# arangesh/Ground-Plane-Polling

Measured on AMD Instinct MI355X. Metric: images/sec end-to-end (resnet50, 1k planes, 1242x375), higher is better.
Workload: dtype f16x3

## Files before the change

### ground-plane-polling_amd/csrc/conv_igemm.hip

```cpp

#include <hip/hip_runtime.h>
#include <stdint.h>
#include <stdlib.h>

#include "conv_igemm_types.h"
#include "conv_tiles.h"
#include "gpp.h"

namespace {

inline bool is_x3(int dtype) { return dtype == GPP_BF16X3 || dtype == GPP_F16X3; }
inline bool f32_storage(int dtype) { return dtype == GPP_F32 || is_x3(dtype); }
inline int elem_size(int dtype) { return f32_storage(dtype) ? 4 : 2; }

int validate(const gpp_conv_desc& d)
{
    if (!d.in || !d.weight || !d.out) return GPP_ERR_BAD_ARG;
    if (d.dtype != GPP_BF16 && d.dtype != GPP_F16 && d.dtype != GPP_F32 && !is_x3(d.dtype)) return GPP_ERR_UNSUPPORTED;
    const int esz = elem_size(d.dtype), ck = 128 / esz, va = 16 / esz;
    if (d.batch <= 0 || d.C_in <= 0 || d.C_out <= 0 || d.KH <= 0 || d.KW <= 0) return GPP_ERR_BAD_ARG;
    constexpr int kMaxDim = 1 << 20;
    if (d.batch > kMaxDim || d.C_in > kMaxDim || d.C_out > kMaxDim || d.in_pitch > kMaxDim || d.out_pitch > kMaxDim || d.res_pitch > kMaxDim ||
        d.weight_rows > kMaxDim || d.weight_rows < 0 || d.in_pitch < 0 || d.out_pitch < 0 || d.res_pitch < 0 || d.partial_bytes < 0)
        return GPP_ERR_UNSUPPORTED;
    if (d.KH > 8 || d.KW > 8) return GPP_ERR_UNSUPPORTED;
    if (d.C_in % ck != 0 || d.C_out % 4 != 0) return GPP_ERR_UNSUPPORTED;
    if (d.stride != 1 && d.stride != 2) return GPP_ERR_UNSUPPORTED;
    if (d.n_groups < 1 || d.n_groups > GPP_MAX_GROUPS) return GPP_ERR_BAD_ARG;
    if (d.split_k < 0) return GPP_ERR_BAD_ARG;
#ifndef GPP_STAMPS
    if (d.reserved != 0) return GPP_ERR_BAD_ARG;
#endif
    if (d.reserved2 != 0 || (d.x3_split & ~(GPP_X3_IN | GPP_X3_OUT | GPP_X3_RES))) return GPP_ERR_BAD_ARG;
    if (d.reserved3 != 0 || (d.gather_rows != nullptr) != (d.gather_counts != nullptr)) return GPP_ERR_BAD_ARG;
    if (((uintptr_t)d.gather_rows | (uintptr_t)d.gather_counts | (uintptr_t)d.guard) & 3) return GPP_ERR_ALIGN;
    if (d.gather_rows && (d.stride != 1 || d.residual || !d.out_f32 || d.split_k > 1)) return GPP_ERR_UNSUPPORTED;
    if (d.x3_split && !is_x3(d.dtype)) return GPP_ERR_BAD_ARG;
    if (d.out_scale && d.dtype != GPP_F16X3) return GPP_ERR_BAD_ARG;
    if ((d.x3_split & GPP_X3_OUT) && (d.out_f32 || d.C_out % 32 != 0 || d.out_pitch % 32 != 0)) return GPP_ERR_UNSUPPORTED;
    if ((d.x3_split & GPP_X3_IN) && d.in_pitch % 32 != 0) return GPP_ERR_UNSUPPORTED;
    if ((d.x3_split & GPP_X3_RES) && (!d.residual || d.res_pitch % 32 != 0)) return GPP_ERR_UNSUPPORTED;
    const int oa = (d.out_f32 || f32_storage(d.dtype)) ? 4 : 8;
    if (d.in_pitch < d.C_in || d.in_pitch % va != 0) return GPP_ERR_ALIGN;
    if (d.out_pitch < d.C_out || d.out_pitch % oa != 0) return GPP_ERR_ALIGN;
    if (d.residual && (d.res_pitch < d.C_out || d.res_pitch % va != 0)) return GPP_ERR_ALIGN;
    if (((uintptr_t)d.in | (uintptr_t)d.weight | (uintptr_t)d.out | (uintptr_t)d.zero_page | (uintptr_t)d.residual |
         (uintptr_t)d.bias | (uintptr_t)d.partial) & 15)
        return GPP_ERR_ALIGN;
    for (int g = 0; g < d.n_groups; ++g) {
        const gpp_conv_group& G = d.groups[g];
        if (G.H_in <= 0 || G.W_in <= 0 || G.H_out <= 0 || G.W_out <= 0) return GPP_ERR_BAD_ARG;
        if (G.H_in > kMaxDim || G.W_in > kMaxDim || G.H_out > kMaxDim || G.W_out > kMaxDim || G.H_res > kMaxDim || G.W_res > kMaxDim) return GPP_ERR_UNSUPPORTED;
        constexpr int64_t kMaxOff = (int64_t)1 << 40;
        if (G.in_off < 0 || G.out_off < 0 || G.res_off < 0 || G.in_bstride < 0 || G.out_bstride < 0 || G.res_bstride < 0 || G.in_off > kMaxOff ||
            G.out_off > kMaxOff || G.res_off > kMaxOff || G.in_bstride > kMaxOff || G.out_bstride > kMaxOff || G.res_bstride > kMaxOff)
            return GPP_ERR_BAD_ARG;
        if ((G.out_off | G.out_bstride) % oa != 0) return GPP_ERR_ALIGN;
        if ((G.in_off | G.in_bstride) % va != 0) return GPP_ERR_ALIGN;
        if (d.residual && ((G.res_off | G.res_bstride) % va != 0 || G.H_res <= 0 || G.W_res <= 0)) return GPP_ERR_ALIGN;
        if ((int64_t)d.batch * G.H_out * G.W_out >= (1LL << 31)) return GPP_ERR_UNSUPPORTED;
        if ((d.x3_split & GPP_X3_OUT) && ((G.out_off | G.out_bstride) % 32 != 0)) return GPP_ERR_ALIGN;
        if ((d.x3_split & GPP_X3_IN) && ((G.in_off | G.in_bstride) % 32 != 0)) return GPP_ERR_ALIGN;
        if ((d.x3_split & GPP_X3_RES) && ((G.res_off | G.res_bstride) % 32 != 0)) return GPP_ERR_ALIGN;
    }
    return GPP_OK;
}

int split_rule(const gpp_conv_desc& d)
{
    if (!d.partial) return 1;
    int64_t pix = 0;
    for (int g = 0; g < d.n_groups; ++g) pix += (int64_t)d.groups[g].H_out * d.groups[g].W_out;
    const int64_t tiles_per_image = ((pix + 127) / 128) * ((d.C_out + 127) / 128);
    const int64_t kdepth = (int64_t)d.KH * d.KW * d.C_in;
    if (tiles_per_image > 24 || kdepth < 3072) return 1;
    int split = (int)((kdepth + 768) / 1536);
    return split < 1 ? 1 : (split > 8 ? 8 : split);
}

int fill_range_counter(gpp_conv_desc& d)
{
    if (d.dtype != GPP_F16X3) return d.range_counter ? GPP_ERR_BAD_ARG : GPP_OK;
    if (!d.range_counter) d.range_counter = (uint64_t*)gpp_x3_range_counter_f16x3();
    if (!d.range_counter) return GPP_ERR_UNSUPPORTED;
    return ((uintptr_t)d.range_counter & 7) ? GPP_ERR_ALIGN : GPP_OK;
}

int dispatch_any(gpp_conv_desc& d, hipStream_t st)
{
    const int rc = fill_range_counter(d);
    if (rc != GPP_OK) return rc;
    if (d.split_k == 0) d.split_k = split_rule(d);
    if (d.gather_rows) {
        if (d.split_k > 1) return GPP_ERR_UNSUPPORTED;
        return gpp_conv_gather_dispatch(d, st);
    }
    switch (d.dtype) {
        case GPP_BF16: return gpp_conv_dispatch_bf16(d, st);
        case GPP_F16: return gpp_conv_dispatch_f16(d, st);
        case GPP_BF16X3: return gpp_conv_dispatch_bf16x3(d, st);
        case GPP_F16X3: return gpp_conv_dispatch_f16x3(d, st);
        default: return gpp_conv_dispatch_f32(d, st);
    }
}

int tail_entry(const gpp_conv_desc* conv3x3, const gpp_conv_desc* conv1x1, int tile_rows, void* stream)
{
    if (!conv3x3 || !conv1x1) return GPP_ERR_BAD_ARG;
    gpp_conv_desc d1 = *conv3x3, d2 = *conv1x1;
    int rc = validate(d1);
    if (rc == GPP_OK) rc = validate(d2);
    if (rc != GPP_OK) return rc;
    if (d1.gather_rows || d2.gather_rows || d1.guard || d2.guard) return GPP_ERR_UNSUPPORTED;
    const gpp_conv_group &G1 = d1.groups[0], &G2 = d2.groups[0];
    if (d1.dtype == GPP_F32) return GPP_ERR_UNSUPPORTED;
    if (is_x3(d1.dtype) && (!(d1.x3_split & GPP_X3_IN) || (d2.x3_split & (GPP_X3_OUT | GPP_X3_RES)) != (GPP_X3_OUT | GPP_X3_RES) || !d2.residual))
        return GPP_ERR_UNSUPPORTED;
    if (d1.dtype != d2.dtype || d1.n_groups != 1 || d2.n_groups != 1 || d1.batch != d2.batch) return GPP_ERR_UNSUPPORTED;
    if (d1.KH != 3 || d1.KW != 3 || d1.stride != 1 || d1.pad_top != 1 || d1.pad_left != 1 || d1.residual || d1.out_f32) return GPP_ERR_UNSUPPORTED;
// ... 71 lines not shown
{
    return gpp_x3_range_snapshot_of(nullptr, device_count, stream);
}

extern "C" int gpp_x3_range_snapshot_of(const uint64_t* counter, uint64_t* device_count, void* stream)
{
    if (!device_count) return GPP_ERR_BAD_ARG;
    if (((uintptr_t)counter | (uintptr_t)device_count) & 7) return GPP_ERR_ALIGN;
    return gpp_x3_range_snapshot_f16x3((const unsigned long long*)counter, (unsigned long long*)device_count, (hipStream_t)stream);
}

extern "C" int gpp_conv2d_flops(const gpp_conv_desc* host_desc, double* flops)
{
    if (!host_desc || !flops) return GPP_ERR_BAD_ARG;
    if (host_desc->n_groups < 1 || host_desc->n_groups > GPP_MAX_GROUPS) return GPP_ERR_BAD_ARG;
    double f = 0.0;
    for (int g = 0; g < host_desc->n_groups; ++g)
        f += 2.0 * host_desc->batch * (double)host_desc->groups[g].H_out * host_desc->groups[g].W_out *
             host_desc->KH * host_desc->KW * (double)host_desc->C_in * host_desc->C_out;
    *flops = f;
    return GPP_OK;
}

extern "C" int gpp_conv2d_split_rule(const gpp_conv_desc* host_desc, int* split_k)
{
    if (!host_desc || !split_k) return GPP_ERR_BAD_ARG;
    gpp_conv_desc d = *host_desc;
    int rc = validate(d);
    if (rc != GPP_OK) return rc;
    *split_k = d.split_k > 0 ? d.split_k : split_rule(d);
    return GPP_OK;
}

extern "C" int gpp_conv2d_workspace_bytes(const gpp_conv_desc* host_desc, size_t* bytes)
{
    if (!host_desc || !bytes) return GPP_ERR_BAD_ARG;
    gpp_conv_desc d = *host_desc;
    char probe[16] __attribute__((aligned(16)));
    if (!d.partial) { d.partial = probe; d.partial_bytes = 0; }
    int rc = validate(d);
    if (rc != GPP_OK) return rc;
    const int split = d.split_k > 0 ? d.split_k : split_rule(d);
    *bytes = 0;
    if (split <= 1) return GPP_OK;
    int64_t rows = 0;
    for (int g = 0; g < d.n_groups; ++g) rows += (int64_t)d.batch * d.groups[g].H_out * d.groups[g].W_out + 256;
    const int64_t npad = (d.C_out + 255) / 256 * 256;
    *bytes = (size_t)(split * rows * npad * 4);
    return GPP_OK;
}

extern "C" int gpp_conv2d_igemm(const gpp_conv_desc* host_desc, void* stream)
{
    if (!host_desc) return GPP_ERR_BAD_ARG;
    gpp_conv_desc d = *host_desc;
    for (int g = 0; g < GPP_MAX_GROUPS; ++g) d.groups[g].row_begin = 0;
    int rc = validate(d);
    if (rc != GPP_OK) return rc;
    return dispatch_any(d, (hipStream_t)stream);
}

static const gpp_tiles::Entry kTiles[] = {{0, gpp_tiles::PLAIN, gpp_tiles::ALL, 0, 128, 0, 0, 0}, GPP_CONV_TILES(GPP_TILE_ENTRY, GPP_TILE_NONE, GPP_TILE_NONE)};

static bool env_is_1(const char* name) { const char* e = getenv(name); return e && e[0] == '1'; }

static bool tile_is_candidate(const gpp_conv_desc* desc, const gpp_tiles::Entry& t)
{
    using namespace gpp_tiles;
    const gpp_conv_desc& d = *desc;
    if ((d.gather_rows != nullptr) != (t.form == GATHER)) return t.code == 0;
    const bool x3_in = is_x3(d.dtype) && (d.x3_split & GPP_X3_IN);
    if (!owner_has(t.owner, f32_storage(d.dtype), is_x3(d.dtype))) return false;
    if (is_x3(d.dtype) && x3_wants_split_input(t.form, t.owner) && !x3_in && t.owner != ALL_X3IN) return false;
    const int nk = d.KH * d.KW * (d.C_in / (128 / elem_size(d.dtype)));
    if (t.form == DUAL && !dual_can_run(d, nk)) return false;
    if (t.form == MIX && !mix_can_run(d, nk)) return false;
    if (t.form == WS && !ws_can_run(d, t.bm, t.bn)) return false;
    static const bool no_deep = env_is_1("GPP_NO_DEEP_TILES"), no_ws = env_is_1("GPP_NO_WS_TILES"), no_mix = env_is_1("GPP_NO_MIX_TILES");
    int64_t rows = 0;
    for (int g = 0; g < d.n_groups; ++g) rows += (int64_t)d.batch * d.groups[g].H_out * d.groups[g].W_out;
    const int bn = t.bn;
    const auto pads_less_than = [&](int other) { return (d.C_out + bn - 1) / bn * bn < (d.C_out + other - 1) / other * other; };
    switch (t.form) {
        case GATHER: return bn != 160 || pads_less_than(64);
        case DEEP: {
            int64_t tiles_m = 0;
            for (int g = 0; g < d.n_groups; ++g) tiles_m += ((int64_t)d.batch * d.groups[g].H_out * d.groups[g].W_out + t.bm - 1) / t.bm;
            const int64_t wgs = tiles_m * ((d.C_out + bn - 1) / bn) * (d.split_k > 1 ? d.split_k : 1);
            return !(bn == 64 && d.C_out > 256) && !no_deep && nk >= 12 && wgs <= 320;
        }
        case WS: return !no_ws && rows >= 256 * 16;
        case MIX: return !no_mix && nk >= 4 && rows * (d.C_out / 256) >= 256 * 256;
        default: break;
    }
    if (t.code == 0) return true;
    if (bn == 64 && d.C_out > 256 && !(d.KH == 1 && d.KW == 1 && d.C_in <= 256)) return false;
    if (bn == 256 && (d.C_out < 192 || rows < 256 * 16)) return false;
    if ((t.form == PIPE || t.form == DUAL) && nk < 4) return false;
    if ((bn == 160 || bn == 96) && !pads_less_than(128)) return false;
    return true;
}

extern "C" int gpp_conv2d_tile_candidates(const gpp_conv_desc* desc, int* tiles, int capacity, int* count)
{
    if (!desc || !count || capacity < 0 || (capacity > 0 && !tiles)) return GPP_ERR_BAD_ARG;
    {
        gpp_conv_desc d = *desc;
        for (int g = 0; g < GPP_MAX_GROUPS; ++g) d.groups[g].row_begin = 0;
        const int rc = validate(d);
        if (rc != GPP_OK) return rc;
    }
    int n = 0;
    for (const gpp_tiles::Entry& t : kTiles) {
        if (!tile_is_candidate(desc, t)) continue;
        if (n < capacity) tiles[n] = t.code;
        ++n;
    }
    *count = n;
    return GPP_OK;
}

extern "C" int gpp_conv2d_autotune(gpp_conv_desc* desc, int iters, void* stream, float* best_us)
{
    if (!desc || iters < 1) return GPP_ERR_BAD_ARG;
    {
        gpp_conv_desc d = *desc;
        for (int g = 0; g < GPP_MAX_GROUPS; ++g) d.groups[g].row_begin = 0;
        const int rc = validate(d);
        if (rc != GPP_OK) return rc;
    }
    hipStream_t st = (hipStream_t)stream;
    hipEvent_t e0, e1;
    hipError_t e = hipEventCreate(&e0);
    if (e != hipSuccess) return (int)e;
    e = hipEventCreate(&e1);
    if (e != hipSuccess) { (void)hipEventDestroy(e0); return (int)e; }
    const int tile_in = desc->tile_hint;
    float best = 1e30f;
    int best_tile = tile_in, rc = GPP_OK;
    auto time_one = [&](int tile, float* us, int reps = 2) -> int {
        desc->tile_hint = tile;
        int r = gpp_conv2d_igemm(desc, stream);
        if (r != GPP_OK) return r;
        float t_best = 1e30f;
        for (int rep = 0; rep < reps; ++rep) {
            (void)hipEventRecord(e0, st);
            for (int i = 0; i < iters; ++i) (void)gpp_conv2d_igemm(desc, stream);
            (void)hipEventRecord(e1, st);
            hipError_t s = hipEventSynchronize(e1);
            if (s != hipSuccess) return (int)s;
            float ms = 0.0f;
            (void)hipEventElapsedTime(&ms, e0, e1);
            t_best = ms < t_best ? ms : t_best;
        }
        *us = t_best * 1000.0f / iters;
        return GPP_OK;
    };
    float second = 1e30f;
    int second_tile = -1;
    for (const gpp_tiles::Entry& t : kTiles) {
        if (!tile_is_candidate(desc, t)) continue;
        const int tile = t.code;
        float us = 0.0f;
        int r = time_one(tile, &us);
        if (r != GPP_OK) { if (tile == 0) { rc = r; break; } continue; }
        if (us < best) { second = best; second_tile = best_tile; best = us; best_tile = tile; }
        else if (us < second) { second = us; second_tile = tile; }
// ... 124 lines not shown
```

### ground-plane-polling_amd/csrc/conv_igemm_impl.h

```cpp
#ifndef GPP_CONV_IGEMM_IMPL_H_
#define GPP_CONV_IGEMM_IMPL_H_

#include <hip/hip_runtime.h>
#include <stdint.h>

#include <atomic>
#include <type_traits>

#include "conv_tiles.h"
#include "gpp.h"

namespace {

typedef __attribute__((ext_vector_type(8))) __bf16 bf16x8;
typedef __attribute__((ext_vector_type(8))) _Float16 f16x8;
typedef __attribute__((ext_vector_type(4))) float f32x4;

struct f32x8 {
    f32x4 lo, hi;
    __device__ __forceinline__ float operator[](int e) const { return e < 4 ? lo[e] : hi[e - 4]; }
};

template <int DT> struct Elem;
template <> struct Elem<GPP_BF16> {
    using scalar = __bf16;
    using vec8 = bf16x8;
    using frag = bf16x8;
    static constexpr int ESZ = 2;
    static __device__ __forceinline__ f32x4 mfma(frag a, frag b, f32x4 c)
    {
        return __builtin_amdgcn_mfma_f32_16x16x32_bf16(a, b, c, 0, 0, 0);
    }
    static __device__ __forceinline__ vec8 pack(const float (&v)[8])
    {
        vec8 o;
#pragma unroll
        for (int e = 0; e < 8; ++e) o[e] = (scalar)v[e];
        return o;
    }
};
template <> struct Elem<GPP_F16> {
    using scalar = _Float16;
    using vec8 = f16x8;
    using frag = f16x8;
    static constexpr int ESZ = 2;
    static __device__ __forceinline__ f32x4 mfma(frag a, frag b, f32x4 c)
    {
        return __builtin_amdgcn_mfma_f32_16x16x32_f16(a, b, c, 0, 0, 0);
    }
    static __device__ __forceinline__ vec8 pack(const float (&v)[8])
    {
        vec8 o;
#pragma unroll
        for (int e = 0; e < 8; ++e) o[e] = (scalar)v[e];
        return o;
    }
};
template <> struct Elem<GPP_F32> {
    using scalar = float;
    using vec8 = f32x8;
    using frag = f32x4;
    static constexpr int ESZ = 4;
    static __device__ __forceinline__ f32x4 mfma(frag a, frag b, f32x4 c)
    {
        c = __builtin_amdgcn_mfma_f32_16x16x4f32(a[0], b[0], c, 0, 0, 0);
        c = __builtin_amdgcn_mfma_f32_16x16x4f32(a[1], b[1], c, 0, 0, 0);
        c = __builtin_amdgcn_mfma_f32_16x16x4f32(a[2], b[2], c, 0, 0, 0);
        c = __builtin_amdgcn_mfma_f32_16x16x4f32(a[3], b[3], c, 0, 0, 0);
        return c;
    }
    static __device__ __forceinline__ vec8 pack(const float (&v)[8])
    {
        vec8 o;
        o.lo = (f32x4){v[0], v[1], v[2], v[3]};
        o.hi = (f32x4){v[4], v[5], v[6], v[7]};
        return o;
    }
};

constexpr int kRowBytes = 128;

__device__ __forceinline__ void glds16(__amdgpu_buffer_rsrc_t rsrc, int voffset, int soffset, void* lds_dst_wave_base)
{
    __builtin_amdgcn_raw_ptr_buffer_load_lds(rsrc, (__attribute__((address_space(3))) void*)lds_dst_wave_base, 16,
                                             voffset, soffset, 0, 0);
}

constexpr int kOutOfRange = (int)0x80000000;

#ifndef GPP_DMA_SPREAD
#define GPP_DMA_SPREAD 1
#endif
#ifndef GPP_X3_PRIO
#define GPP_X3_PRIO 1
#endif
constexpr bool kSpreadDma = GPP_DMA_SPREAD != 0;

#ifndef GPP_X3_SERPENTINE
#define GPP_X3_SERPENTINE 2
#endif
#define GPP_SERP(g, j, n) ((GPP_X3_SERPENTINE && ((g) & 1)) ? (n) - 1 - (j) : (j))
#define GPP_SERP2(g, j, n) ((GPP_X3_SERPENTINE > 1 && ((g) & 1)) ? (n) - 1 - (j) : (j))

#ifdef GPP_STAMPS
#define GPP_STAMP(k)                                                                                          \
    do {                                                                                                      \
        if ((d.reserved & 16) && wave == 0 && lane == 0)                                                      \
            ((unsigned long long*)d.zero_page)[((int64_t)blockIdx.y * gridDim.x + blockIdx.x) * 8 + (k)] = __builtin_amdgcn_s_memrealtime(); \
    } while (0)
#define GPP_STAMP_END()                                                                                       \
    do {                                                                                                      \
        GPP_STAMP(3);                                                                                         \
        asm volatile("s_waitcnt vmcnt(0)" ::: "memory");                                                      \
        GPP_STAMP(4);                                                                                         \
    } while (0)
#define GPP_ABL(flag) if (!(flag))
#else
#define GPP_ABL(flag)
#define GPP_STAMP(k) do { } while (0)
#define GPP_STAMP_END() do { } while (0)
#endif

__device__ __forceinline__ int xcd_remap(int bid, int nwg)
{
    const int xcd = bid & 7, local = bid >> 3;
    const int q = nwg >> 3, r = nwg & 7;
    return (xcd < r ? xcd * (q + 1) : r * (q + 1) + (xcd - r) * q) + local;
}

template <int DT> constexpr bool kX3 = (DT == GPP_BF16X3 || DT == GPP_F16X3);
template <int DT> struct X3Half {
    using half = __bf16;
    using vec = bf16x8;
    static __device__ __forceinline__ f32x4 mfma(vec, vec, f32x4 c) { return c; }
    static __device__ __forceinline__ float clamp(float x) { return x; }
};

template <> struct X3Half<GPP_BF16X3> {
    using half = __bf16;
    using vec = bf16x8;
    static __device__ __forceinline__ f32x4 mfma(vec a, vec b, f32x4 c) { return __builtin_amdgcn_mfma_f32_16x16x32_bf16(a, b, c, 0, 0, 0); }
    static __device__ __forceinline__ float clamp(float x) { return x; }
};
template <> struct X3Half<GPP_F16X3> {
    using half = _Float16;
    using vec = f16x8;
    static __device__ __forceinline__ f32x4 mfma(vec a, vec b, f32x4 c) { return __builtin_amdgcn_mfma_f32_16x16x32_f16(a, b, c, 0, 0, 0); }
    static __device__ __forceinline__ float clamp(float x) { return fminf(fmaxf(x, -65504.0f), 65504.0f); }
};
template <int DT>
__device__ __forceinline__ void x3_range(float (&v)[8], unsigned long long* counter)
{
    if constexpr (DT == GPP_F16X3) {
        float c[8];
        bool changed = false;
#pragma unroll
        for (int e = 0; e < 8; ++e) {
            c[e] = X3Half<DT>::clamp(v[e]);
            changed |= (c[e] != v[e]);
        }
        if (__builtin_expect(changed, 0)) {
            atomicAdd(counter, 1ull);
#pragma unroll
            for (int e = 0; e < 8; ++e) c[e] = (fabsf(v[e]) <= 3.402823466e38f) ? c[e] : v[e];
        }
#pragma unroll
        for (int e = 0; e < 8; ++e) v[e] = c[e];
    }
}
__device__ __forceinline__ const char* x3_addr(const void* buf, int64_t base, int n)
{
    return (const char*)buf + ((base + (n & ~31)) << 2) + ((n & 31) << 1);
}
template <int DT>
__device__ __forceinline__ void x3_unpack(const f32x4 hi_bits, const f32x4 lo_bits, float (&r)[8])
{
    union { f32x4 f; typename X3Half<DT>::vec b; } h, l;
    h.f = hi_bits;
    l.f = lo_bits;
// ... 120 lines not shown
                                            int64_t out_off, int64_t out_bs, int64_t res_off, int64_t res_bs)
{
    const int b = m / HoWo, p = m - b * HoWo;
    int64_t rp = p;
    if (d.residual && (H_res != H_out || W_res != W_out)) {
        const float sy = (float)H_res / (float)H_out, sx = (float)W_res / (float)W_out;
        const int oy = p / W_out, ox = p - oy * W_out;
        const int ry = min((int)floorf((float)oy * sy), H_res - 1);
        const int rx = min((int)floorf((float)ox * sx), W_res - 1);
        rp = (int64_t)ry * W_res + rx;
    }
    RowAddr a;
    a.obase = out_off + (int64_t)b * out_bs + (int64_t)p * d.out_pitch;
    a.rbase = res_off + (int64_t)b * res_bs + rp * d.res_pitch;
    return a;
}

struct PixWalk {
    int b, oy, ox;
    __device__ __forceinline__ void init(int m, int HoWo, int W_out)
    {
        b = m / HoWo;
        const int p = m - b * HoWo;
        oy = p / W_out;
        ox = p - oy * W_out;
    }
    __device__ __forceinline__ void advance(int n, int H_out, int W_out)
    {
        ox += n;
        while (ox >= W_out) { ox -= W_out; ++oy; }
        while (oy >= H_out) { oy -= H_out; ++b; }
    }
};

__device__ __forceinline__ RowAddr row_addr_at(const gpp_conv_desc& d, const PixWalk& w, int W_out, int H_out, int H_res, int W_res,
                                               int64_t out_off, int64_t out_bs, int64_t res_off, int64_t res_bs)
{
    const int p = w.oy * W_out + w.ox;
    int64_t rp = p;
    if (d.residual && (H_res != H_out || W_res != W_out)) {
        const float sy = (float)H_res / (float)H_out, sx = (float)W_res / (float)W_out;
        const int ry = min((int)floorf((float)w.oy * sy), H_res - 1);
        const int rx = min((int)floorf((float)w.ox * sx), W_res - 1);
        rp = (int64_t)ry * W_res + rx;
    }
    RowAddr a;
    a.obase = out_off + (int64_t)w.b * out_bs + (int64_t)p * d.out_pitch;
    a.rbase = res_off + (int64_t)w.b * res_bs + rp * d.res_pitch;
    return a;
}

template <int DT> struct ElemX3 {
    using scalar = float;
    using vec8 = f32x8;
    using frag = f32x4;
    static constexpr int ESZ = 4;
    static __device__ __forceinline__ vec8 pack(const float (&v)[8]) { return Elem<GPP_F32>::pack(v); }
    static __device__ __forceinline__ f32x4 mfma(frag, frag, f32x4 c) { return c; }
    static __device__ __forceinline__ void split(const f32x4 x0, const f32x4 x1, typename X3Half<DT>::vec& hi, typename X3Half<DT>::vec& lo)
    {
        using half = typename X3Half<DT>::half;
#pragma unroll
        for (int e = 0; e < 8; ++e) {
            const float x = X3Half<DT>::clamp(e < 4 ? x0[e] : x1[e - 4]);
            const half h = (half)x;
            hi[e] = h;
            lo[e] = (half)(x - (float)h);
        }
    }
};
template <> struct Elem<GPP_BF16X3> : ElemX3<GPP_BF16X3> {};
template <> struct Elem<GPP_F16X3> : ElemX3<GPP_F16X3> {};

template <int DT> constexpr bool kF32Storage = (DT == GPP_F32 || DT == GPP_BF16X3 || DT == GPP_F16X3);

constexpr int stage_rows(int BM, int NW) { return (BM + 8 * NW - 1) / (8 * NW) * (8 * NW); }

template <int DT, int BM, int BN, int WM, int WN, int STAGES, bool PIPE, bool XIN = false, bool PRE = false, bool GATHER = false>
__device__ __forceinline__ void conv_igemm_body(const gpp_conv_desc& d, const int block_x, const int grid_x, const float* pre_s = nullptr,
                                                const float* pre_t = nullptr)
{
    static_assert(!XIN || kX3<DT>, "pre-split input maps: GPP_BF16X3 / GPP_F16X3");
    static_assert(!PRE || (!PIPE && !XIN && kF32Storage<DT>), "pre-activation: float32-sized input maps, plain loop");
    static_assert(!GATHER || (!PIPE && !PRE), "gathered rows: plain loop");
    if (d.guard != nullptr && *(const volatile int32_t*)d.guard != d.guard_value) return;
    using E = Elem<DT>;
    using vec8 = typename E::vec8;
    using frag = typename E::frag;
    using scalar = typename E::scalar;
    using xh8 = typename X3Half<DT>::vec;
    constexpr int ESZ = E::ESZ, CK = kRowBytes / ESZ;
    constexpr int NW = WM * WN;
    constexpr int MF = BM / WM / 16, NF = BN / WN / 16;
    constexpr int BMS = stage_rows(BM, NW);
    constexpr int A_BYTES = BMS * kRowBytes, B_BYTES = BN * kRowBytes, STAGE = A_BYTES + B_BYTES;
    constexpr int A_IT = BMS / 8 / NW, B_IT = BN / 8 / NW;
    constexpr int PER_STAGE = A_IT + B_IT;
    constexpr int PF = STAGES - 1;
    static_assert(MF >= 1 && NF >= 1 && A_IT >= 1 && B_IT >= 1 && BMS % (8 * NW) == 0 && BN % (8 * NW) == 0 && BM % (16 * WM) == 0, "tile / wave shape");

    extern __shared__ __attribute__((aligned(16))) unsigned char smem[];

    const int tid = threadIdx.x, lane = tid & 63;
    const int wave = __builtin_amdgcn_readfirstlane(tid >> 6);
    const int wm = wave / WN, wn = wave % WN;
    GPP_STAMP(0);

    const int bid = GATHER ? block_x : xcd_remap(block_x, grid_x);
    const int n_tiles = (d.C_out + BN - 1) / BN;
    const int nt = bid % n_tiles, mt = bid / n_tiles;
    int tile_start = 0, row_begin = 0, H_in = 0, W_in = 0, H_out = 0, W_out = 0, H_res = 0, W_res = 0;
    int64_t in_off = 0, in_bs = 0, out_off = 0, out_bs = 0, res_off = 0, res_bs = 0;
    int list_begin = 0, list_next = 0, group = 0;
#pragma unroll
    for (int q = 0; q < GPP_MAX_GROUPS; ++q) {
        if constexpr (GATHER) {
            if (q < d.n_groups && mt >= d.groups[q].tile_start) { list_begin = list_next; group = q; }
            if (q < d.n_groups) list_next += d.batch * d.groups[q].H_out * d.groups[q].W_out;
        }
        if (q < d.n_groups && mt >= d.groups[q].tile_start) {
            tile_start = d.groups[q].tile_start;
            row_begin = d.groups[q].row_begin;
            H_in = d.groups[q].H_in; W_in = d.groups[q].W_in;
            H_out = d.groups[q].H_out; W_out = d.groups[q].W_out;
            H_res = d.groups[q].H_res; W_res = d.groups[q].W_res;
            in_off = d.groups[q].in_off; in_bs = d.groups[q].in_bstride;
            out_off = d.groups[q].out_off; out_bs = d.groups[q].out_bstride;
            res_off = d.groups[q].res_off; res_bs = d.groups[q].res_bstride;
        }
    }
    const int HoWo = H_out * W_out;
    const int Mpix = d.batch * HoWo;
    const int32_t* const glist = GATHER ? d.gather_rows + list_begin : nullptr;
    const int Mg = GATHER ? min(max(d.gather_counts[group], 0), Mpix) : Mpix;
    const int m0 = row_begin + (mt - tile_start) * BM, n0 = nt * BN;
    if constexpr (GATHER) {
        if (m0 >= Mg) return;
    }
    auto pixel_of = [&](int m) { return min(max(glist[m], 0), Mpix - 1); };
    const int Ktot = d.KH * d.KW * d.C_in;
    const int cpt = d.C_in / CK;
    const int nk_total = d.KH * d.KW * cpt;
    const int nsplit = gridDim.y, split = blockIdx.y;
    int ks0 = 0, nk = nk_total;
    if (nsplit > 1) {
        ks0 = (int)((unsigned)(nk_total * split) / (unsigned)nsplit);
        nk = (int)((unsigned)(nk_total * (split + 1)) / (unsigned)nsplit) - ks0;
    }

    const int srow = lane >> 3;
    const int gchunk = (lane & 7) ^ srow;
    const __amdgpu_buffer_rsrc_t in_rsrc = __builtin_amdgcn_make_buffer_rsrc((void*)d.in, 0, d.in_bytes, 0x00020000);
    const __amdgpu_buffer_rsrc_t w_rsrc = __builtin_amdgcn_make_buffer_rsrc((void*)d.weight, 0, d.weight_bytes, 0x00020000);
    constexpr bool VOFF_INLINE = PIPE && A_IT >= 8;
    int a_base[A_IT], a_mask[A_IT], a_voff[VOFF_INLINE ? 1 : A_IT];
    int tap_delta = 0, tap_need = 0;
    const int pitch2 = d.in_pitch * ESZ;
    {
        PixWalk pw;
        if constexpr (!GATHER) pw.init(m0 + wave * A_IT * 8 + srow, HoWo, W_out);
#pragma unroll
        for (int i = 0; i < A_IT; ++i) {
            const int m = m0 + (wave * A_IT + i) * 8 + srow;
            a_mask[i] = 0;
            a_base[i] = 0;
            if (m < Mg) {
                if constexpr (GATHER) pw.init(pixel_of(m), HoWo, W_out);
                const int iy0 = pw.oy * d.stride - d.pad_top, ix0 = pw.ox * d.stride - d.pad_left;
                const int rlo = max(0, -iy0), rhi = min(d.KH, max(0, H_in - iy0));
                const int clo = max(0, -ix0), chi = min(d.KW, max(0, W_in - ix0));
                const int rmask = rhi > rlo ? ((1 << rhi) - 1) & ~((1 << rlo) - 1) : 0;
                const int cmask = chi > clo ? ((1 << chi) - 1) & ~((1 << clo) - 1) : 0;
                a_mask[i] = rmask | (cmask << 8);
                a_base[i] = (int)((in_off + (int64_t)pw.b * in_bs) * ESZ) + gchunk * 16 + (iy0 * W_in + ix0) * pitch2;
            }
            if (!GATHER && i + 1 < A_IT) pw.advance(8, H_out, W_out);
        }
    }
    int w_voff[B_IT];
#pragma unroll
    for (int i = 0; i < B_IT; ++i) w_voff[i] = (n0 + (wave * B_IT + i) * 8 + srow) * Ktot * ESZ + gchunk * 16;

    auto set_tap = [&](int kh, int kw) {
        const int delta = (kh * W_in + kw) * pitch2;
        const int need = (1 << kh) | (1 << (8 + kw));
        if constexpr (VOFF_INLINE) {
            tap_delta = delta; tap_need = need;
        } else {
#pragma unroll
            for (int i = 0; i < A_IT; ++i) a_voff[i] = ((a_mask[i] & need) == need) ? a_base[i] + delta : kOutOfRange;
        }
    };
    auto voff_of = [&](int i) {
        if constexpr (VOFF_INLINE) return ((a_mask[i] & tap_need) == tap_need) ? a_base[i] + tap_delta : kOutOfRange;
        else return a_voff[i];
    };
    auto stage = [&](int buf, int cc, int ks) {
        unsigned char* sa = smem + buf * STAGE + wave * A_IT * 8 * kRowBytes;
        unsigned char* sb = smem + buf * STAGE + A_BYTES + wave * B_IT * 8 * kRowBytes;
#pragma unroll
        for (int i = 0; i < A_IT; ++i) glds16(in_rsrc, voff_of(i), cc * kRowBytes, sa + i * 8 * kRowBytes);
#pragma unroll
        for (int i = 0; i < B_IT; ++i) glds16(w_rsrc, w_voff[i], ks * kRowBytes, sb + i * 8 * kRowBytes);
    };
// ... 456 lines not shown
        }
        if (use_pre) {
#pragma unroll
            for (int i = 0; i < MF; ++i) {
                const int m = m0 + wm * (BM / WM) + i * 16 + frow;
                if (m >= Mg) continue;
#pragma unroll
                for (int jj = 0; jj < NF / 2; ++jj) {
                    const int n = n0 + wn * COLS + jj * 32 + fq * 8;
                    if (n >= d.C_out) continue;
                    float v[8];
#pragma unroll
                    for (int e = 0; e < 4; ++e) {
                        v[e] = comb(acc[i][2 * jj][e], jj, e);
                        v[4 + e] = comb(acc[i][2 * jj + 1][e], jj, 4 + e);
                    }
                    finish8_pre<DT>(d, v, n, ra_pre[i].obase, true, rpre[i][jj]);
                }
            }
            GPP_STAMP_END();
            return;
        }
    }
    if (interior && !res) {
        const int mfirst = m0 + wm * (BM / WM) + frow;
        int b = mfirst / HoWo, p = mfirst - b * HoWo;
#pragma unroll
        for (int i = 0; i < MF; ++i) {
            const int64_t obase = out_off + (int64_t)b * out_bs + (int64_t)p * d.out_pitch;
#pragma unroll
            for (int jj = 0; jj < NF / 2; ++jj) {
                float v[8];
#pragma unroll
                for (int e = 0; e < 4; ++e) {
                    v[e] = comb(acc[i][2 * jj][e], jj, e);
                    v[4 + e] = comb(acc[i][2 * jj + 1][e], jj, 4 + e);
                }
                finish8_pre<DT>(d, v, n0 + wn * COLS + jj * 32 + fq * 8, obase, false, typename E::vec8());
            }
            p += 16;
            while (p >= HoWo) { p -= HoWo; ++b; }
        }
        GPP_STAMP_END();
        return;
    }
    PixWalk pwe;
    if constexpr (!GATHER) pwe.init(m0 + wm * (BM / WM) + frow, HoWo, W_out);
#pragma unroll
    for (int i = 0; i < MF; ++i) {
        const int m = m0 + wm * (BM / WM) + i * 16 + frow;
        if (m >= Mg) break;
        if constexpr (GATHER) pwe.init(pixel_of(m), HoWo, W_out);
        const RowAddr ra = row_addr_at(d, pwe, W_out, H_out, H_res, W_res, out_off, out_bs, res_off, res_bs);
        if constexpr (!GATHER) pwe.advance(16, H_out, W_out);
        const scalar* rrow = res ? res + ra.rbase : nullptr;
#pragma unroll
        for (int jj = 0; jj < NF / 2; ++jj) {
            const int n = n0 + wn * COLS + jj * 32 + fq * 8;
            if (n >= d.C_out) continue;
            float v[8];
#pragma unroll
            for (int e = 0; e < 4; ++e) {
                v[e] = comb(acc[i][2 * jj][e], jj, e);
                v[4 + e] = comb(acc[i][2 * jj + 1][e], jj, 4 + e);
            }
            finish8<DT>(d, v, n, ra.obase, rrow);
        }
    }
    GPP_STAMP_END();
}

template <int DT, int BM, int BN, int WM, int WN, int STAGES, bool PIPE, bool XIN = false>
__global__ __launch_bounds__(64 * WM * WN, 2) void conv_igemm_kernel(const gpp_conv_desc d)
{
    conv_igemm_body<DT, BM, BN, WM, WN, STAGES, PIPE, XIN>(d, blockIdx.x, gridDim.x);
}

template <int DT, int BM, int BN, int WM, int WN, int STAGES, bool XIN>
__global__ __launch_bounds__(64 * WM * WN, 2) void conv_gather_kernel(const gpp_conv_desc d)
{
    conv_igemm_body<DT, BM, BN, WM, WN, STAGES, false, XIN, false, true>(d, blockIdx.x, gridDim.x);
}

template <int DT, int BM, int BN, int WM, int WN>
__global__ __launch_bounds__(64 * WM * WN, 2) void conv_preact_kernel(const gpp_conv_desc d, const float* in_scale, const float* in_shift)
{
    conv_igemm_body<DT, BM, BN, WM, WN, 2, false, false, true>(d, blockIdx.x, gridDim.x, in_scale, in_shift);
}

template <int DT, bool XIN = false>
__global__ __launch_bounds__(512, 2) void conv_igemm_dual_kernel(const gpp_conv_desc d0, const gpp_conv_desc d1, const int n0,
                                                                 const int split0, const int n1)
{
    if ((int)blockIdx.x < split0) {
        if ((int)blockIdx.x < n0) conv_igemm_body<DT, 256, 256, 2, 4, 2, true, XIN>(d0, blockIdx.x, n0);
    } else {
        conv_igemm_body<DT, 512, 128, 4, 2, 2, true, XIN>(d1, (int)blockIdx.x - split0, n1);
    }
}

template <int DT, int BMA, int BMB, int BN, bool XIN>
__global__ __launch_bounds__(512, 2) void conv_igemm_mix_kernel(const gpp_conv_desc da, const gpp_conv_desc db, const int na,
                                                                const int splita, const int nb)
{
    if ((int)blockIdx.x < splita) {
        if ((int)blockIdx.x < na) conv_igemm_body<DT, BMA, BN, 2, 4, 2, true, XIN>(da, blockIdx.x, na);
    } else {
        conv_igemm_body<DT, BMB, BN, 2, 4, 2, true, XIN>(db, (int)blockIdx.x - splita, nb);
    }
}

template <int DT>
__global__ __launch_bounds__(256) void splitk_reduce_kernel(const gpp_conv_desc d, int BM, int npad, int nsplit)
{
    if (d.guard != nullptr && *(const volatile int32_t*)d.guard != d.guard_value) return;
    using scalar = typename Elem<DT>::scalar;
    const int n8 = (d.C_out + 7) / 8;
    const int64_t total = (int64_t)d.partial_rows * n8;
    const int64_t e = (int64_t)blockIdx.x * 256 + threadIdx.x;
    if (e >= total) return;
    const int r = (int)(e / n8), n = (int)(e - (int64_t)r * n8) * 8;
    const int mt = r / BM;
    int tile_start = 0, H_out = 0, W_out = 0, H_res = 0, W_res = 0;
    int64_t out_off = 0, out_bs = 0, res_off = 0, res_bs = 0;
#pragma unroll
    for (int q = 0; q < GPP_MAX_GROUPS; ++q) {
        if (q < d.n_groups && mt >= d.groups[q].tile_start) {
            tile_start = d.groups[q].tile_start;
            H_out = d.groups[q].H_out; W_out = d.groups[q].W_out;
            H_res = d.groups[q].H_res; W_res = d.groups[q].W_res;
            out_off = d.groups[q].out_off; out_bs = d.groups[q].out_bstride;
            res_off = d.groups[q].res_off; res_bs = d.groups[q].res_bstride;
        }
    }
    const int HoWo = H_out * W_out;
    const int m = r - tile_start * BM;
    if (m >= d.batch * HoWo) return;
    float v[8];
#pragma unroll
    for (int k = 0; k < 8; ++k) v[k] = 0.0f;
    const float* src = (const float*)d.partial + (int64_t)r * npad + n;
    for (int s = 0; s < nsplit; ++s) {
        const f32x4 a = *(const f32x4*)(src + (int64_t)s * d.partial_rows * npad);
        const f32x4 b = *(const f32x4*)(src + (int64_t)s * d.partial_rows * npad + 4);
#pragma unroll
        for (int k = 0; k < 4; ++k) { v[k] += a[k]; v[4 + k] += b[k]; }
    }
    if constexpr (DT == GPP_F16X3) {
        if (d.out_scale) {
#pragma unroll
            for (int k = 0; k < 8; ++k) if (n + k < d.C_out) v[k] *= d.out_scale[n + k];
        }
    }
    if (d.bias) {
#pragma unroll
        for (int k = 0; k < 8; ++k) if (n + k < d.C_out) v[k] += d.bias[n + k];
    }
    const RowAddr ra = row_addr(d, m, HoWo, W_out, H_out, H_res, W_res, out_off, out_bs, res_off, res_bs);
    finish8<DT>(d, v, n, ra.obase, d.residual ? (const scalar*)d.residual + ra.rbase : nullptr);
}

template <int DT, int BM, int CMID>
__global__ __launch_bounds__(256, 2) void bottleneck_tail_kernel(const gpp_conv_desc d1, const gpp_conv_desc d2)
{
    using E = Elem<DT>;
    using vec8 = typename E::vec8;
// ... 896 lines not shown
    d1.weight_rows = d.weight_rows - head;
    if (d.bias) d1.bias = d.bias + head;
    if (d.out_scale) d1.out_scale = d.out_scale + head;
    for (int g = 0; g < d.n_groups; ++g) {
        d1.groups[g].out_off += head;
        d1.groups[g].res_off += head;
    }
    const int t0 = prepare<256, 256>(d0), t1 = prepare<512, 128>(d1);
    if (t0 < 0) return t0;
    if (t1 < 0) return t1;
    const int n0 = t0 * (head / 256), n1 = t1;
    const int split0 = (n0 + 7) / 8 * 8;
    kernel<<<dim3((unsigned)(split0 + n1)), dim3(512), lds, st>>>(d0, d1, n0, split0, n1);
    return last_launch_rc();
}

template <int DT, int BMA, int BMB>
int launch_mix(const gpp_conv_desc& d, hipStream_t st)
{
    constexpr int BN = 256, CUS = 256;
    constexpr int ESZ = Elem<DT>::ESZ, CK = kRowBytes / ESZ;
    static_assert(kX3<DT>, "mixed grids exist for the x3 types");
    if (!gpp_tiles::mix_can_run(d, d.KH * d.KW * (d.C_in / CK))) return GPP_ERR_UNSUPPORTED;
    const int n_tiles = d.C_out / BN;
    const int64_t rows0 = (int64_t)d.batch * d.groups[0].H_out * d.groups[0].W_out;
    auto tiles_b = [&](int64_t begin, int bm) {
        int64_t t = (rows0 - begin + bm - 1) / bm;
        for (int g = 1; g < d.n_groups; ++g) t += ((int64_t)d.batch * d.groups[g].H_out * d.groups[g].W_out + bm - 1) / bm;
        return t * n_tiles;
    };
    int64_t best_cost = (tiles_b(0, BMA) + CUS - 1) / CUS * BMA;
    int best_ra = 0;
    for (int ra = 1; ra <= 64; ++ra) {
        if ((ra * CUS) % n_tiles != 0) continue;
        const int64_t ma = (int64_t)ra * CUS / n_tiles;
        if (ma * BMA > rows0) break;
        const int64_t cost = (int64_t)ra * BMA + (tiles_b(ma * BMA, BMB) + CUS - 1) / CUS * BMB;
        if (cost < best_cost) { best_cost = cost; best_ra = ra; }
    }
    if (best_ra == 0) return GPP_ERR_UNSUPPORTED;
    constexpr int lds = 2 * (stage_rows(BMA > BMB ? BMA : BMB, 8) + BN) * kRowBytes;
    constexpr auto kernel = conv_igemm_mix_kernel<DT, BMA, BMB, BN, true>;
    const int rc = allow_lds<kernel>(lds);
    if (rc != GPP_OK) return rc;
    const int ma = best_ra * CUS / n_tiles;
    gpp_conv_desc da = d, db = d;
    da.n_groups = 1;
    const int ta = prepare<BMA, BN>(da);
    if (ta < 0) return ta;
    db.groups[0].row_begin = ma * BMA;
    const int tb = prepare<BMB, BN>(db);
    if (tb < 0) return tb;
    da.in_bytes = db.in_bytes;
    const int na = ma * n_tiles, nb = tb * n_tiles;
    const int splita = (na + 7) / 8 * 8;
    kernel<<<dim3((unsigned)(splita + nb)), dim3(512), lds, st>>>(da, db, na, splita, nb);
    return last_launch_rc();
}

template <int DT, int BM, int BN>
int launch_ws(gpp_conv_desc& d, hipStream_t st)
{
    constexpr int R = 4;
    static_assert(kX3<DT>, "weight-stationary 1 x 1: x3 types");
    if (!gpp_tiles::ws_can_run(d, BM, BN)) return GPP_ERR_UNSUPPORTED;
    const gpp_conv_group& G = d.groups[0];
    const int lds = (d.C_in / 32) * BN * kRowBytes + R * BM * kRowBytes;
    const int tiles = prepare<BM, BN>(d);
    if (tiles < 0) return tiles;
    const int n_mtiles = (int)(((int64_t)d.batch * G.H_out * G.W_out + BM - 1) / BM);
    const auto go = [&](auto has_res) {
        constexpr auto kernel = conv1x1_ws_kernel<DT, BM, BN, decltype(has_res)::value>;
        const int rc = allow_lds<kernel>(160 * 1024);
        if (rc != GPP_OK) return rc;
        kernel<<<dim3(256), dim3(512), lds, st>>>(d, n_mtiles);
        return last_launch_rc();
    };
    return d.residual ? go(std::true_type()) : go(std::false_type());
}

template <int DT, int BM, int BN, int WM, int WN, int STAGES, bool XIN = false>
int launch_gather(gpp_conv_desc& d, hipStream_t st)
{
    if constexpr (kX3<DT> && !XIN) {
        if (d.x3_split & GPP_X3_IN) return launch_gather<DT, BM, BN, WM, WN, STAGES, true>(d, st);
    }
    constexpr int BMS = stage_rows(BM, WM * WN);
    constexpr int lds = STAGES * (BMS + BN) * kRowBytes;
    constexpr auto kernel = conv_gather_kernel<DT, BM, BN, WM, WN, STAGES, XIN>;
    const int rc = allow_lds<kernel>(lds);
    if (rc != GPP_OK) return rc;
    const int tiles = prepare<BM, BN>(d);
    if (tiles < 0) return tiles;
    const int n_tiles = (d.C_out + BN - 1) / BN;
    kernel<<<dim3((unsigned)(tiles * n_tiles)), dim3(64 * WM * WN), lds, st>>>(d);
    return last_launch_rc();
}

template <int DT, int FORM, int OWNER, int BM, int BN, int WM, int WN, int STAGES>
int run_tile(gpp_conv_desc& d, hipStream_t st)
{
    if constexpr (FORM == gpp_tiles::GATHER) {
        return GPP_ERR_BAD_ARG;
    } else if constexpr (!gpp_tiles::owner_has(OWNER, kF32Storage<DT>, kX3<DT>)) {
        return kF32Storage<DT> ? GPP_ERR_UNSUPPORTED : GPP_ERR_BAD_ARG;
    } else {
        constexpr bool XIN = kX3<DT> && gpp_tiles::x3_wants_split_input(FORM, OWNER);
        if (XIN && !(d.x3_split & GPP_X3_IN)) return GPP_ERR_UNSUPPORTED;
        if constexpr (FORM == gpp_tiles::DUAL) return launch_dual<DT>(d, st);
        else if constexpr (FORM == gpp_tiles::MIX) return launch_mix<DT, BM, BN>(d, st);
        else if constexpr (FORM == gpp_tiles::WS) return d.guard ? GPP_ERR_UNSUPPORTED : launch_ws<DT, BM, BN>(d, st);
        else return launch<DT, BM, BN, WM, WN, STAGES, gpp_tiles::tile_pipelined(FORM, BM, BN, kF32Storage<DT>), XIN>(d, st);
    }
}

#define GPP_RUN_TILE(code, form, owner, bm, bn, wm, wn, stages) \
    case code: return run_tile<DT, gpp_tiles::form, gpp_tiles::owner, bm, bn, wm, wn, stages>(d, st);
#define GPP_RUN_GATHER(code, form, owner, bm, bn, wm, wn, stages) \
    case code: if constexpr (gpp_tiles::form == gpp_tiles::GATHER) return launch_gather<DT, bm, bn, wm, wn, stages>(d, st); else break;
#define GPP_RUN_PREACT(code, form, owner, bm, bn, wm, wn, stages) \
    case code: return launch_preact<DT, bm, bn, wm, wn>(d, in_scale, in_shift, st);

template <int DT>
int dispatch_preact(gpp_conv_desc& d, const float* in_scale, const float* in_shift, hipStream_t st)
{
    switch (d.tile_hint) {
        case 0: return d.C_out <= 64 ? launch_preact<DT, 128, 64, 2, 2>(d, in_scale, in_shift, st)
                                     : launch_preact<DT, 128, 128, 2, 2>(d, in_scale, in_shift, st);
        GPP_CONV_TILES(GPP_TILE_NONE, GPP_TILE_NONE, GPP_RUN_PREACT)
        default: return GPP_ERR_BAD_ARG;
    }
}

template <int DT>
int dispatch_gather(gpp_conv_desc& d, hipStream_t st)
{
    switch (d.tile_hint) {
        case 0: return launch_gather<DT, 64, 64, 2, 2, 2>(d, st);
        GPP_CONV_TILES(GPP_RUN_GATHER, GPP_RUN_GATHER, GPP_TILE_NONE)
        default: break;
    }
    return GPP_ERR_BAD_ARG;
}

template <int DT>
int dispatch(gpp_conv_desc& d, hipStream_t st)
{
#ifdef GPP_STAMPS
    if constexpr (!kF32Storage<DT>) {
        if ((d.reserved & 4) && (d.tile_hint == 128 || d.tile_hint == 128128)) return launch<DT, 128, 128, 2, 2, 2, true>(d, st);
        if ((d.reserved & 8) && (d.tile_hint == 512 || d.tile_hint == 256256)) return launch<DT, 256, 256, 2, 4, 2, false>(d, st);
    }
#endif
    switch (d.tile_hint) {
        GPP_CONV_TILES(GPP_RUN_TILE, GPP_RUN_TILE, GPP_TILE_NONE)
        case 0: break;
        default: return GPP_ERR_BAD_ARG;
    }
    if (d.C_out <= 64 || (d.C_out % 128 != 0 && d.C_out % 128 <= 64)) return launch<DT, 128, 64, 2, 2, 2, false>(d, st);
    if constexpr (!kF32Storage<DT>) {
        int64_t rows = 0;
        for (int g = 0; g < d.n_groups; ++g) rows += (int64_t)d.batch * d.groups[g].H_out * d.groups[g].W_out;
        const int nk = d.KH * d.KW * (d.C_in / 64);
        const int n256 = (d.C_out + 255) / 256;
        const int64_t big_blocks = ((rows + 255) / 256) * n256;
        const bool n_fits = d.C_out >= 256 && n256 * 256 * 7 <= d.C_out * 8;
        if (n_fits && big_blocks >= 512 && nk >= 8 && d.split_k <= 1) return launch<DT, 256, 256, 2, 4, 2, true>(d, st);
    }
    return launch<DT, 128, 128, 2, 2, 2, false>(d, st);
}

template <auto KERNEL, int BM, int CMID, int ESZ, int LDS>
int launch_tail_as(gpp_conv_desc& d1, gpp_conv_desc& d2, hipStream_t st)
{
    int rc = allow_lds<KERNEL>(LDS);
    if (rc == GPP_OK) rc = set_input_extent(d1, ESZ);
    if (rc == GPP_OK) rc = set_weight_extent(d1, 9 * CMID, ESZ);
    if (rc == GPP_OK) rc = set_weight_extent(d2, CMID, ESZ);
    if (rc != GPP_OK) return rc;
    const gpp_conv_group& G = d1.groups[0];
    const int64_t rows = (int64_t)d1.batch * G.H_out * G.W_out;
    KERNEL<<<dim3((unsigned)((rows + BM - 1) / BM)), dim3(256), LDS, st>>>(d1, d2);
    return last_launch_rc();
}

template <int DT, int BM, int CMID>
int launch_tail(gpp_conv_desc& d1, gpp_conv_desc& d2, hipStream_t st)
{
    return launch_tail_as<bottleneck_tail_kernel<DT, BM, CMID>, BM, CMID, 2, 2 * (BM + CMID) * kRowBytes>(d1, d2, st);
}

template <int DT, int BM, int CMID>
int launch_tail_x3(gpp_conv_desc& d1, gpp_conv_desc& d2, hipStream_t st)
{
    constexpr int KC = CMID / 32;
    constexpr int ring = 2 * (BM + CMID) * kRowBytes, phase2 = KC * BM * kRowBytes + KC * 128 * kRowBytes;
    return launch_tail_as<bottleneck_tail_x3_kernel<DT, BM, CMID>, BM, CMID, 4, (ring > phase2 ? ring : phase2)>(d1, d2, st);
}

template <int DT>
int dispatch_tail_x3(gpp_conv_desc& d1, gpp_conv_desc& d2, int tile_rows, hipStream_t st)
{
    if (d1.C_in != 64) return GPP_ERR_UNSUPPORTED;
    switch (tile_rows) {
        case 64: return launch_tail_x3<DT, 64, 64>(d1, d2, st);
        case 96: return launch_tail_x3<DT, 96, 64>(d1, d2, st);
        case 0:
        case 128: return launch_tail_x3<DT, 128, 64>(d1, d2, st);
        case 160: return launch_tail_x3<DT, 160, 64>(d1, d2, st);
        default: return GPP_ERR_BAD_ARG;
    }
}

template <int DT>
int dispatch_tail(gpp_conv_desc& d1, gpp_conv_desc& d2, int tile_rows, hipStream_t st)
{
    const bool c64 = d1.C_in == 64;
    switch (tile_rows) {
        case 96: return c64 ? launch_tail<DT, 96, 64>(d1, d2, st) : launch_tail<DT, 96, 128>(d1, d2, st);
        case 0:
        case 128: return c64 ? launch_tail<DT, 128, 64>(d1, d2, st) : launch_tail<DT, 128, 128>(d1, d2, st);
// ... 9 lines not shown
```

### ground-plane-polling_amd/csrc/conv_tiles.h

```cpp
#ifndef GPP_CONV_TILES_H_
#define GPP_CONV_TILES_H_

#include <stdint.h>

#include "gpp.h"

namespace gpp_tiles {

enum Form {
    PLAIN,
    PIPE,
    DUAL,
    MIX,
    WS,
    DEEP,
    GATHER,
    PREACT,
};

enum Owner {
    ALL,
    ALL_X3IN,
    B16,
    NOT_F32,
    X3,
    X3IN,
};

struct Entry {
    int code, form, owner;
    int bm, bn;
    int wm, wn, stages;
};

#define GPP_CONV_TILES(T, X, P)                                                                                                          \
    T(64064, PLAIN, ALL, 64, 64, 2, 2, 2)                                                                                                \
    T(96064, PLAIN, ALL, 96, 64, 2, 2, 2)                                                                                                \
    T(128064, PLAIN, ALL, 128, 64, 2, 2, 2)                                                                                              \
    T(160064, PLAIN, ALL, 160, 64, 2, 2, 2)                                                                                              \
    T(192064, PLAIN, ALL, 192, 64, 2, 2, 2)                                                                                              \
    T(64128, PLAIN, ALL, 64, 128, 2, 2, 2)                                                                                               \
    T(96128, PLAIN, ALL, 96, 128, 2, 2, 2)                                                                                               \
    T(128128, PLAIN, ALL, 128, 128, 2, 2, 2)                                                                                             \
    T(160128, PLAIN, ALL, 160, 128, 2, 2, 2)                                                                                             \
    T(192128, PLAIN, ALL, 192, 128, 2, 2, 2)                                                                                             \
    T(224128, PLAIN, ALL, 224, 128, 2, 2, 2)                                                                                             \
    T(1128128, PIPE, NOT_F32, 128, 128, 2, 2, 2)                                                                                         \
    T(1192128, PIPE, NOT_F32, 192, 128, 2, 2, 2)                                                                                         \
    T(1128256, PIPE, NOT_F32, 128, 256, 2, 4, 2)                                                                                         \
    T(1160256, PIPE, X3IN, 160, 256, 2, 4, 2)                                 \
    T(1192256, PIPE, NOT_F32, 192, 256, 2, 4, 2)                                                                                         \
    T(1224256, PIPE, X3IN, 224, 256, 2, 4, 2)                                                                                            \
                                \
    T(256256, PLAIN, NOT_F32, 256, 256, 2, 4, 2)                                                                                         \
    T(1256256, PIPE, X3IN, 256, 256, 2, 4, 2)                                                                                            \
                     \
    T(128160, PLAIN, ALL, 128, 160, 4, 1, 2)                                                                                             \
    T(192160, PLAIN, ALL_X3IN, 192, 160, 4, 1, 2)                  \
    T(1192160, PIPE, B16, 192, 160, 4, 1, 2)                                                                                             \
    T(1128160, PIPE, NOT_F32, 128, 160, 4, 1, 2)                                                                                         \
    T(2256256, DUAL, NOT_F32, 256, 256, 2, 4, 2)                                                                                         \
    T(1192096, PIPE, NOT_F32, 192, 96, 4, 1, 2)                                                                                          \
    T(3256224, MIX, X3IN, 256, 224, 2, 4, 2)                                                                                             \
    T(3192160, MIX, X3IN, 192, 160, 2, 4, 2)                                                                                             \
    T(4128064, WS, X3IN, 128, 64, 2, 4, 4)                                                                                               \
    T(4064064, WS, X3IN, 64, 64, 2, 4, 4)                                                                                                \
    T(4128128, WS, X3IN, 128, 128, 2, 4, 4)                                                                                              \
    T(4064128, WS, X3IN, 64, 128, 2, 4, 4)                                                                                               \
              \
    T(5064064, DEEP, X3IN, 64, 64, 2, 2, 4)                                                                                              \
    T(5096064, DEEP, X3IN, 96, 64, 2, 2, 4)                                                                                              \
    T(5064128, DEEP, X3IN, 64, 128, 2, 2, 4)                                                                                             \
    T(5096128, DEEP, X3IN, 96, 128, 2, 2, 4)                                                                                             \
    T(5128128, DEEP, X3IN, 128, 128, 2, 2, 4)                                                                                            \
                                                 \
    T(128256, PLAIN, X3, 128, 256, 2, 4, 2)                                                                                              \
    T(192256, PLAIN, X3, 192, 256, 2, 4, 2)                                                                                              \
           \
    T(6064064, GATHER, ALL, 64, 64, 2, 2, 2)                                                                                             \
    T(6032064, GATHER, ALL, 32, 64, 2, 2, 2)                                                                                             \
    T(6064160, GATHER, ALL, 64, 160, 4, 1, 2)                                                                                            \
    T(7064064, GATHER, ALL, 64, 64, 2, 2, 4)                                                                                             \
    T(7032064, GATHER, ALL, 32, 64, 2, 2, 4)                                                                                             \
    T(7064160, GATHER, ALL, 64, 160, 4, 1, 4)                                                                                            \
    X(64, PLAIN, ALL, 128, 64, 2, 2, 2)                                                                                                  \
    X(128, PLAIN, ALL, 128, 128, 2, 2, 2)                                                                                                \
    X(256, PLAIN, B16, 256, 128, 4, 2, 3)                                                             \
    X(512, PLAIN, B16, 256, 256, 2, 4, 2)                                                                                                \
    P(64064, PREACT, ALL, 64, 64, 2, 2, 2)                                                                                               \
    P(128064, PREACT, ALL, 128, 64, 2, 2, 2)                                                                                             \
    P(64128, PREACT, ALL, 64, 128, 2, 2, 2)                                                                                              \
    P(128128, PREACT, ALL, 128, 128, 2, 2, 2)                                                                                            \
    P(192128, PREACT, ALL, 192, 128, 2, 2, 2)

#define GPP_TILE_ENTRY(code, form, owner, bm, bn, wm, wn, stages) {code, gpp_tiles::form, gpp_tiles::owner, bm, bn, wm, wn, stages},
#define GPP_TILE_NONE(...)

constexpr bool owner_has(int owner, bool f32_storage, bool x3)
{
    return owner == ALL || owner == ALL_X3IN || (owner == B16 && !f32_storage) || (owner == NOT_F32 && (!f32_storage || x3)) ||
           ((owner == X3 || owner == X3IN) && x3);
}

constexpr bool x3_wants_split_input(int form, int owner)
{
    return owner == X3IN || owner == ALL_X3IN || (form != PLAIN && form != GATHER && form != PREACT);
}

constexpr bool tile_pipelined(int form, int bm, int bn, bool f32_storage) { return form == PIPE || (!f32_storage && form == PLAIN && bm == 256 && bn == 256); }


inline bool dual_can_run(const gpp_conv_desc& d, int nk) { return d.C_out >= 384 && d.C_out % 256 == 128 && nk >= 2 && d.split_k <= 1; }

inline bool mix_can_run(const gpp_conv_desc& d, int nk) { return d.C_out % 256 == 0 && nk >= 2 && d.split_k <= 1; }

inline bool ws_can_run(const gpp_conv_desc& d, int bm, int bn)
{
    const gpp_conv_group& G = d.groups[0];
    return (d.x3_split & GPP_X3_IN) && d.KH == 1 && d.KW == 1 && d.stride == 1 && d.pad_top == 0 && d.pad_left == 0 && d.n_groups == 1 && d.split_k <= 1 &&
           d.C_out % bn == 0 && 32 % (d.C_out / bn) == 0 && d.C_in % 32 == 0 && G.H_in == G.H_out && G.W_in == G.W_out &&
           (!d.residual || ((d.x3_split & GPP_X3_RES) && G.H_res == G.H_out && G.W_res == G.W_out)) &&
           (d.C_in / 32) * bn * 128 + 4 * bm * 128 <= 160 * 1024;
}

}

#endif
```

### ground-plane-polling_amd/csrc/decode.hip

```cpp

#include <hip/hip_runtime.h>
#include <stdint.h>
#include <limits.h>

#include <atomic>

#include "gpp.h"

namespace {

constexpr int kCounterStride = 4096;
constexpr int kHeaderBytes = 64 * kCounterStride;
constexpr int kKeptCountWord = 1;
constexpr int kKeptKeysOffset = 1024;

__device__ __forceinline__ float cephes_expf(float x)
{
    x = fminf(fmaxf(x, -88.3762626647949f), 88.3762626647949f);
    float fx = floorf(x * 1.44269504088896341f + 0.5f);
    x = (x - fx * 0.693359375f) - fx * -2.12194440e-4f;
    const float z = x * x;
    float y = 1.9875691500e-4f;
    y = y * x + 1.3981999507e-3f;
    y = y * x + 8.3334519073e-3f;
// ... 567 lines not shown
    if (stages & GPP_DETECT_CANDIDATES) {
        clear_counters_kernel<<<1, 64, 0, st>>>(cnt, lists);
        const dim3 grid((unsigned)((n_anchors + 255) / 256), (unsigned)B);
        if (osf) candidates_osf_kernel<<<grid, 256, 0, st>>>(cls_logits, n_anchors, kstride, score_thr, keys, cnt);
        else candidates_kernel<<<grid, 256, 0, st>>>(cls_logits, n_anchors, kstride, score_thr, keys, cnt);
    }
    if (stages & GPP_DETECT_SELECT) {
        static std::atomic<uint64_t> configured{0};
        int dev = 0;
        e = hipGetDevice(&dev);
        if (e != hipSuccess) return (int)e;
        if (!(configured.load(std::memory_order_acquire) & (1ull << (dev & 63)))) {
            e = hipFuncSetAttribute((const void*)nms_kernel, hipFuncAttributeMaxDynamicSharedMemorySize, kLdsKeys * 16 + kHistBins * 4);
            if (e != hipSuccess) return (int)e;
            configured.fetch_or(1ull << (dev & 63), std::memory_order_release);
        }
        nms_kernel<<<dim3((unsigned)lists), kNmsThreads, kLdsKeys * 16 + kHistBins * 4, st>>>(
            keys, cnt, kstride, cls_logits, regression, regression_dim, (const float4*)anchors, n_anchors, L, iou_thr, max_det,
            counts, wboxes, alive, ws, lists_per_image);
    }
    if (stages & GPP_DETECT_EMIT) {
        if (osf)
            emit_osf_kernel<<<dim3((unsigned)B), 512, 0, st>>>(ws, cls_logits, regression, regression_dim, (const float4*)anchors,
                                                               n_anchors, L, max_det, boxes, dims, scores, labels, orientations,
                                                               anchor_index, counts);
        else
            emit_kernel<<<dim3((unsigned)B), 128, 0, st>>>(ws, cls_logits, regression, regression_dim, (const float4*)anchors,
                                                           n_anchors, L, max_det, boxes, dims, scores, labels, orientations, anchor_index);
    }
    e = hipGetLastError();
    return e == hipSuccess ? GPP_OK : (int)e;
}

}

namespace {

__global__ __launch_bounds__(256) void pack_kernel(const float* __restrict__ boxes, const float* __restrict__ dims,
                                                   const float* __restrict__ scores, const int32_t* __restrict__ labels,
                                                   const int32_t* __restrict__ orient, const float* __restrict__ keypoints,
                                                   const float* __restrict__ keyplanes, const float* __restrict__ residuals,
                                                   float* __restrict__ out, int64_t rows)
{
    const int64_t e = (int64_t)blockIdx.x * 256 + threadIdx.x;
    if (e >= rows * 35) return;
    const int64_t r = e / 35;
    const int c = (int)(e - r * 35);
    float v;
    if (c < 12) v = boxes[r * 12 + c];
    else if (c < 15) v = dims[r * 3 + (c - 12)];
    else if (c == 15) v = scores[r];
    else if (c == 16) v = (float)labels[r];
    else if (c == 17) v = (float)orient[r];
    else if (c < 30) v = keypoints[r * 12 + (c - 18)];
    else if (c < 34) v = keyplanes[r * 4 + (c - 30)];
    else v = residuals[r];
    out[e] = v;
}

}

extern "C" int gpp_pack_detections(const float* boxes, const float* dims, const float* scores, const int32_t* labels,
                                   const int32_t* orientations, const float* keypoints, const float* keyplanes,
                                   const float* residuals, int B, int D, float* packed, void* stream)
{
    if (B < 0 || D < 0) return GPP_ERR_BAD_ARG;
    if (B == 0 || D == 0) return GPP_OK;
    if (!boxes || !dims || !scores || !labels || !orientations || !keypoints || !keyplanes || !residuals || !packed) return GPP_ERR_BAD_ARG;
    const int64_t rows = (int64_t)B * D;
    pack_kernel<<<dim3((unsigned)((rows * 35 + 255) / 256)), 256, 0, (hipStream_t)stream>>>(
        boxes, dims, scores, labels, orientations, keypoints, keyplanes, residuals, packed, rows);
    hipError_t e = hipGetLastError();
    return e == hipSuccess ? GPP_OK : (int)e;
}

namespace {

struct LevelTable {
    int n_levels;
    int pix[GPP_MAX_GROUPS];
    int pix_begin[GPP_MAX_GROUPS];
    int word_begin[GPP_MAX_GROUPS];
    int list_begin[GPP_MAX_GROUPS];
};

__global__ __launch_bounds__(256) void mark_pixels_kernel(const unsigned long long* __restrict__ keys, const int32_t* __restrict__ cnt,
                                                          int64_t key_stride, int64_t n_anchors, int nba, int lists_per_image,
                                                          const LevelTable T, uint32_t* __restrict__ bitmap)
{
    const int list = blockIdx.y, b = list / lists_per_image;
    const int64_t n = min((int64_t)max(cnt[list * (kCounterStride / 4)], 0), n_anchors);
    for (int64_t i = (int64_t)blockIdx.x * 256 + threadIdx.x; i < n; i += (int64_t)gridDim.x * 256) {
        const uint32_t a = 0xFFFFFFFFu - (uint32_t)keys[(int64_t)list * key_stride + i];
        if ((int64_t)a >= n_anchors) continue;
        const int pixel = (int)(a / (uint32_t)nba);
        int l = 0;
        for (int q = 1; q < T.n_levels; ++q) l = pixel >= T.pix_begin[q] ? q : l;
        const int bit = b * T.pix[l] + (pixel - T.pix_begin[l]);
        atomicOr(&bitmap[T.word_begin[l] + (bit >> 5)], 1u << (bit & 31));
    }
}

constexpr int kCompactThreads = 1024;
__global__ __launch_bounds__(kCompactThreads) void compact_pixels_kernel(uint32_t* __restrict__ bitmap, const LevelTable T, int B, int max_rows,
                                                                         int32_t* __restrict__ rows, int32_t* __restrict__ counts,
                                                                         int32_t* __restrict__ flag)
{
    __shared__ int wave_sum[kCompactThreads / 64];
    const int tid = threadIdx.x, lane = tid & 63, wave = tid >> 6;
    int total = 0;
    for (int l = 0; l < GPP_MAX_GROUPS; ++l) {
        int running = 0;
        if (l < T.n_levels) {
            const int n_words = (B * T.pix[l] + 31) >> 5;
            for (int w0 = 0; w0 < n_words; w0 += kCompactThreads) {
                const int w = w0 + tid;
                uint32_t word = 0;
                if (w < n_words) {
                    word = bitmap[T.word_begin[l] + w];
                    if (word) bitmap[T.word_begin[l] + w] = 0;
                }
                const int c = __popc(word);
                int incl = c;
#pragma unroll
                for (int s = 1; s < 64; s <<= 1) {
                    const int up = __shfl_up(incl, s, 64);
                    if (lane >= s) incl += up;
                }
                if (lane == 63) wave_sum[wave] = incl;
                __syncthreads();
                int before = 0, all = 0;
#pragma unroll
                for (int q = 0; q < kCompactThreads / 64; ++q) {
                    const int v = wave_sum[q];
                    before += q < wave ? v : 0;
                    all += v;
                }
                __syncthreads();
                int pos = running + before + incl - c;
                while (word) {
                    const int bit = __ffs((int)word) - 1;
                    word &= word - 1;
                    rows[T.list_begin[l] + pos++] = w * 32 + bit;
                }
                running += all;
            }
        }
        if (tid == 0) counts[l] = running;
        total += running;
    }
    if (tid == 0) {
        counts[GPP_MAX_GROUPS] = total;
        flag[0] = total > max_rows ? 1 : 0;
    }
}

}

extern "C" int gpp_detect_pixel_lists(const gpp_pixel_list_desc* host_desc, void* stream)
{
    if (!host_desc) return GPP_ERR_BAD_ARG;
    const gpp_pixel_list_desc& d = *host_desc;
    if (d.B < 0 || d.B > kMaxBatch || d.n_anchors <= 0 || d.n_anchors > kMaxAnchors || d.num_base_anchors <= 0 || d.max_rows < 0 ||
        d.n_levels < 1 || d.n_levels > GPP_MAX_GROUPS || (d.lists_per_image != 1 && d.lists_per_image != 4) || d.reserved != 0 || d.reserved2 != 0)
        return GPP_ERR_BAD_ARG;
    if (d.B == 0) return GPP_OK;
    if (!d.workspace || !d.bitmap || !d.rows || !d.counts || !d.flag) return GPP_ERR_BAD_ARG;
    if (((uintptr_t)d.workspace & 15) || (((uintptr_t)d.bitmap | (uintptr_t)d.rows | (uintptr_t)d.counts | (uintptr_t)d.flag) & 3)) return GPP_ERR_ALIGN;
    const int lists = d.B * d.lists_per_image;
    if (lists > 64) return GPP_ERR_UNSUPPORTED;
    LevelTable T;
    T.n_levels = d.n_levels;
    int64_t pixels = 0, words = 0;
    for (int l = 0; l < GPP_MAX_GROUPS; ++l) {
        const int pix = l < d.n_levels ? d.level_pixels[l] : 0;
        if (l < d.n_levels && pix <= 0) return GPP_ERR_BAD_ARG;
        if ((int64_t)d.B * (pixels + pix) >= (1LL << 31)) return GPP_ERR_UNSUPPORTED;
        T.pix[l] = pix;
        T.pix_begin[l] = (int)pixels;
        T.word_begin[l] = (int)words;
        T.list_begin[l] = (int)((int64_t)d.B * pixels);
        pixels += pix;
        words += ((int64_t)d.B * pix + 31) / 32;
    }
    if (pixels * d.num_base_anchors != d.n_anchors) return GPP_ERR_BAD_ARG;
    hipStream_t st = (hipStream_t)stream;
    const unsigned char* ws = (const unsigned char*)d.workspace;
    const int32_t* cnt = (const int32_t*)ws;
    const unsigned long long* keys = (const unsigned long long*)(ws + kHeaderBytes);
    mark_pixels_kernel<<<dim3(16, (unsigned)lists), 256, 0, st>>>(keys, cnt, pow2_ceil(d.n_anchors), d.n_anchors, d.num_base_anchors,
                                                                   d.lists_per_image, T, d.bitmap);
    compact_pixels_kernel<<<1, kCompactThreads, 0, st>>>(d.bitmap, T, d.B, d.max_rows, d.rows, d.counts, d.flag);
    const hipError_t e = hipGetLastError();
    return e == hipSuccess ? GPP_OK : (int)e;
}

extern "C" int gpp_detect_workspace_bytes(int B, int64_t n_anchors, size_t* bytes)
{
    if (!bytes || B < 0 || B > kMaxBatch || n_anchors <= 0 || n_anchors > kMaxAnchors) return GPP_ERR_BAD_ARG;
    *bytes = detect_bytes(B, n_anchors, 1);
    return GPP_OK;
}

extern "C" int gpp_detect_osf_workspace_bytes(int B, int64_t n_anchors, size_t* bytes)
{
    if (!bytes || B < 0 || B > kMaxBatch || n_anchors <= 0 || n_anchors > kMaxAnchors) return GPP_ERR_BAD_ARG;
    *bytes = detect_bytes(B, n_anchors, 4);
    return GPP_OK;
}

extern "C" int gpp_detect_stages_f32(int stages, const float* cls_logits, const float* regression,
                                     const float* regression_dim, const float* anchors, int B, int64_t n_anchors,
                                     int num_base_anchors, int fused_layout, float score_thr, float iou_thr, int max_det,
                                     float* boxes, float* dims, float* scores, int32_t* labels, int32_t* orientations,
                                     int32_t* anchor_index, int32_t* counts,
                                     void* workspace, size_t workspace_bytes, void* stream)
{
    return detect_impl(stages, 1, cls_logits, regression, regression_dim, anchors, B, n_anchors, num_base_anchors, fused_layout, score_thr,
                       iou_thr, max_det, boxes, dims, scores, labels, orientations, anchor_index, counts, workspace, workspace_bytes, stream);
}

extern "C" int gpp_detect_osf_f32(const float* cls_logits, const float* regression, const float* regression_dim,
                                  const float* anchors, int B, int64_t n_anchors, int num_base_anchors, int fused_layout,
                                  float score_thr, float iou_thr, int max_det,
                                  float* boxes, float* dims, float* scores, int32_t* labels, int32_t* orientations,
                                  int32_t* anchor_index, int32_t* counts,
                                  void* workspace, size_t workspace_bytes, void* stream)
{
    return detect_impl(GPP_DETECT_CANDIDATES | GPP_DETECT_SELECT | GPP_DETECT_EMIT, 4, cls_logits, regression, regression_dim, anchors, B,
                       n_anchors, num_base_anchors, fused_layout, score_thr, iou_thr, max_det, boxes, dims, scores, labels, orientations,
                       anchor_index, counts, workspace, workspace_bytes, stream);
}

extern "C" int gpp_detect_f32(const float* cls_logits, const float* regression, const float* regression_dim,
                              const float* anchors, int B, int64_t n_anchors, int num_base_anchors, int fused_layout,
                              float score_thr, float iou_thr, int max_det,
                              float* boxes, float* dims, float* scores, int32_t* labels, int32_t* orientations,
                              int32_t* anchor_index, int32_t* counts,
                              void* workspace, size_t workspace_bytes, void* stream)
{
    return gpp_detect_stages_f32(GPP_DETECT_CANDIDATES | GPP_DETECT_SELECT | GPP_DETECT_EMIT, cls_logits, regression, regression_dim,
                                 anchors, B, n_anchors, num_base_anchors, fused_layout, score_thr, iou_thr, max_det, boxes, dims,
                                 scores, labels, orientations, anchor_index, counts, workspace, workspace_bytes, stream);
}
```

### ground-plane-polling_amd/csrc/stem.hip

```cpp

#include <hip/hip_runtime.h>
#include <stdlib.h>
#include <stdint.h>

#include <atomic>

#include "gpp.h"
#include "conv_igemm_types.h"

namespace {

typedef __attribute__((ext_vector_type(8))) __bf16 bf16x8;
typedef __attribute__((ext_vector_type(8))) _Float16 f16x8;
typedef __attribute__((ext_vector_type(8))) float f32x8_natural;
typedef f32x8_natural f32x8 __attribute__((aligned(16)));

constexpr int TW = 64, TH = 4;
constexpr int PW = TW * 2 + 5, PH = TH * 2 + 5;
constexpr int PPITCH = PW * 3 + 1;

__device__ __forceinline__ int ragged_height(const int* __restrict__ heights, int b, int H)
{
    const int h = __builtin_amdgcn_readfirstlane(heights[b]);
    return h < 1 ? 1 : (h > H ? H : h);
// ... 291 lines not shown
        else stem_pool_mfma_ragged_kernel<_Float16, f16x8, 4><<<grid, 256, lds, st>>>(in, wp, bias, (_Float16*)out, B, H, W, Ho, Wo, Hp, Wp, pt, pl, heights);
        return result();
    }
    if (which == 0) stem_pool_mfma_kernel<__bf16, bf16x8, 8><<<grid, 512, lds, st>>>(in, wp, bias, (__bf16*)out, B, H, W, Ho, Wo, Hp, Wp, pt, pl);
    else if (which == 1) stem_pool_mfma_kernel<_Float16, f16x8, 8><<<grid, 512, lds, st>>>(in, wp, bias, (_Float16*)out, B, H, W, Ho, Wo, Hp, Wp, pt, pl);
    else if (which == 2) stem_pool_mfma_kernel<__bf16, bf16x8, 4><<<grid, 256, lds, st>>>(in, wp, bias, (__bf16*)out, B, H, W, Ho, Wo, Hp, Wp, pt, pl);
    else stem_pool_mfma_kernel<_Float16, f16x8, 4><<<grid, 256, lds, st>>>(in, wp, bias, (_Float16*)out, B, H, W, Ho, Wo, Hp, Wp, pt, pl);
    return result();
}

extern "C" int gpp_stem_pool_fused_mfma(const float* in, const void* packed_weight_f16, const float* bias, void* out,
                                        int dtype, int B, int H, int W, void* stream)
{
    return stem_pool_mfma_run(in, packed_weight_f16, bias, out, dtype, B, H, W, nullptr, stream);
}

extern "C" int gpp_stem_pool_fused_mfma_ragged(const float* in, const void* packed_weight_f16, const float* bias, void* out,
                                               int dtype, int B, int H, int W, int Hp, const int32_t* heights, void* stream)
{
    const int rc = ragged_check(heights, H, Hp, 4);
    return rc != GPP_OK ? rc : stem_pool_mfma_run(in, packed_weight_f16, bias, out, dtype, B, H, W, heights, stream);
}

static int stem_pool_x3_run(const float* in, const void* packed_weight_x3, const float* bias, float* out,
                            int B, int H, int W, uint64_t* range_counter, const int32_t* heights, void* stream)
{
    if (!in || !packed_weight_x3 || !bias || !out || B <= 0 || H <= 0 || W <= 0) return GPP_ERR_BAD_ARG;
    if ((uintptr_t)range_counter & 7) return GPP_ERR_ALIGN;
    if (((uintptr_t)out | (uintptr_t)packed_weight_x3) & 15) return GPP_ERR_ALIGN;
    const int Ho = (H + 6 - 7) / 2 + 1, Wo = (W + 6 - 7) / 2 + 1;
    const int Hp = (Ho + 1) / 2, Wp = (Wo + 1) / 2;
    const int pt = ((Hp - 1) * 2 + 3 - Ho > 0 ? (Hp - 1) * 2 + 3 - Ho : 0) / 2;
    const int pl = ((Wp - 1) * 2 + 3 - Wo > 0 ? (Wp - 1) * 2 + 3 - Wo : 0) / 2;
    static const int env_rows = [] { const char* e = getenv("GPP_STEM_POOL_X3_ROWS"); return (e && atoi(e) == 4) ? 4 : 6; }();
    const int rows = heights ? 4 : env_rows;
    const int pr = rows / 2;
    const int64_t total = (int64_t)B * ((Wp + FP_PCOLS - 1) / FP_PCOLS) * ((Hp + pr - 1) / pr);
    if (total >= (1LL << 30)) return GPP_ERR_UNSUPPORTED;
    int dev = 0, cus = 0;
    if (hipGetDevice(&dev) != hipSuccess || hipDeviceGetAttribute(&cus, hipDeviceAttributeMultiprocessorCount, dev) != hipSuccess || cus <= 0)
        return GPP_ERR_UNSUPPORTED;
    const unsigned grid = (unsigned)(total < cus ? total : cus);
    hipStream_t st = (hipStream_t)stream;
    static std::atomic<uint64_t> done[4];
    const int which = rows == 6 ? 0 : 1;
    const void* fns[4] = {(const void*)stem_pool_mfma_x3_kernel<6>, (const void*)stem_pool_mfma_x3_kernel<4>,
                          nullptr, (const void*)stem_pool_mfma_x3_ragged_kernel<4>};
    const int lds = xp_lds(rows);
    const int fn = which + (heights ? 2 : 0);
    if (!(done[fn].load(std::memory_order_acquire) & (1ull << (dev & 63)))) {
        const hipError_t e = hipFuncSetAttribute(fns[fn], hipFuncAttributeMaxDynamicSharedMemorySize, lds);
        if (e != hipSuccess) return (int)e;
        done[fn].fetch_or(1ull << (dev & 63), std::memory_order_release);
    }
    unsigned long long* counter = range_counter ? (unsigned long long*)range_counter : gpp_x3_range_counter_f16x3();
    if (!counter) return GPP_ERR_UNSUPPORTED;
    const _Float16* wp = (const _Float16*)packed_weight_x3;
    if (heights) stem_pool_mfma_x3_ragged_kernel<4><<<grid, 256, lds, st>>>(in, wp, bias, out, B, H, W, Ho, Wo, Hp, Wp, pt, pl, counter, heights);
    else if (which == 0) stem_pool_mfma_x3_kernel<6><<<grid, 384, lds, st>>>(in, wp, bias, out, B, H, W, Ho, Wo, Hp, Wp, pt, pl, counter);
    else stem_pool_mfma_x3_kernel<4><<<grid, 256, lds, st>>>(in, wp, bias, out, B, H, W, Ho, Wo, Hp, Wp, pt, pl, counter);
    return result();
}

extern "C" int gpp_stem_pool_fused_x3(const float* in, const void* packed_weight_x3, const float* bias, float* out,
                                      int B, int H, int W, uint64_t* range_counter, void* stream)
{
    return stem_pool_x3_run(in, packed_weight_x3, bias, out, B, H, W, range_counter, nullptr, stream);
}

extern "C" int gpp_stem_pool_fused_x3_ragged(const float* in, const void* packed_weight_x3, const float* bias, float* out,
                                             int B, int H, int W, int Hp, const int32_t* heights, uint64_t* range_counter, void* stream)
{
    const int rc = ragged_check(heights, H, Hp, 4);
    return rc != GPP_OK ? rc : stem_pool_x3_run(in, packed_weight_x3, bias, out, B, H, W, range_counter, heights, stream);
}

static int maxpool_run(const void* in, void* out, int dtype, int B, int H, int W, int C, const int32_t* heights, void* stream)
{
    if (!in || !out || B <= 0 || H <= 0 || W <= 0 || C <= 0 || C % 8 != 0) return GPP_ERR_BAD_ARG;
    if (((uintptr_t)in | (uintptr_t)out) & 15) return GPP_ERR_ALIGN;
    const int Ho = (H + 1) / 2, Wo = (W + 1) / 2;
    const int pt = ((Ho - 1) * 2 + 3 - H > 0 ? (Ho - 1) * 2 + 3 - H : 0) / 2;
    const int pl = ((Wo - 1) * 2 + 3 - W > 0 ? (Wo - 1) * 2 + 3 - W : 0) / 2;
    const int64_t total = (int64_t)B * Ho * Wo * (C / 8);
    const unsigned blocks = (unsigned)((total + 255) / 256 < 8192 ? (total + 255) / 256 : 8192);
    hipStream_t st = (hipStream_t)stream;
    if (dtype != GPP_BF16 && dtype != GPP_F16 && dtype != GPP_F32) return GPP_ERR_UNSUPPORTED;
    if (heights) {
        if (dtype == GPP_BF16)
            maxpool_ragged_kernel<__bf16, bf16x8><<<blocks, 256, 0, st>>>((const __bf16*)in, (__bf16*)out, B, H, W, C, Ho, Wo, pt, pl, heights);
        else if (dtype == GPP_F16)
            maxpool_ragged_kernel<_Float16, f16x8><<<blocks, 256, 0, st>>>((const _Float16*)in, (_Float16*)out, B, H, W, C, Ho, Wo, pt, pl, heights);
        else
            maxpool_ragged_kernel<float, f32x8><<<blocks, 256, 0, st>>>((const float*)in, (float*)out, B, H, W, C, Ho, Wo, pt, pl, heights);
        return result();
    }
    if (dtype == GPP_BF16)
        maxpool_kernel<__bf16, bf16x8><<<blocks, 256, 0, st>>>((const __bf16*)in, (__bf16*)out, B, H, W, C, Ho, Wo, pt, pl);
    else if (dtype == GPP_F16)
        maxpool_kernel<_Float16, f16x8><<<blocks, 256, 0, st>>>((const _Float16*)in, (_Float16*)out, B, H, W, C, Ho, Wo, pt, pl);
    else if (dtype == GPP_F32)
        maxpool_kernel<float, f32x8><<<blocks, 256, 0, st>>>((const float*)in, (float*)out, B, H, W, C, Ho, Wo, pt, pl);
    else
        return GPP_ERR_UNSUPPORTED;
    return result();
}

extern "C" int gpp_maxpool3x3s2_same(const void* in, void* out, int dtype, int B, int H, int W, int C, void* stream)
{
    return maxpool_run(in, out, dtype, B, H, W, C, nullptr, stream);
}

extern "C" int gpp_maxpool3x3s2_same_ragged(const void* in, void* out, int dtype, int B, int H, int W, int C, int Hp,
                                            const int32_t* heights, void* stream)
{
    const int rc = ragged_check(heights, H, Hp, 2);
    return rc != GPP_OK ? rc : maxpool_run(in, out, dtype, B, H, W, C, heights, stream);
}

extern "C" int gpp_relu_strided(const void* in, int64_t in_bstride, void* out, int64_t out_bstride, int dtype, int B,
                                int64_t count, void* stream)
{
    if (!in || !out || B <= 0 || count <= 0 || count % 8 != 0 || in_bstride % 8 != 0 || out_bstride % 8 != 0)
        return GPP_ERR_BAD_ARG;
    if (((uintptr_t)in | (uintptr_t)out) & 15) return GPP_ERR_ALIGN;
    const int64_t n8 = count / 8;
    const dim3 grid((unsigned)((n8 + 255) / 256 < 4096 ? (n8 + 255) / 256 : 4096), (unsigned)B);
    hipStream_t st = (hipStream_t)stream;
    if (dtype == GPP_BF16X3 || dtype == GPP_F16X3) {
        if (count % 32 != 0 || in_bstride % 32 != 0 || out_bstride % 32 != 0) return GPP_ERR_BAD_ARG;
        relu_x3_kernel<<<grid, 256, 0, st>>>((const char*)in, in_bstride * 4, (char*)out, out_bstride * 4, count / 8);
        return result();
    }
    if (dtype == GPP_BF16)
        relu_kernel<__bf16, bf16x8><<<grid, 256, 0, st>>>((const __bf16*)in, in_bstride, (__bf16*)out, out_bstride, n8);
    else if (dtype == GPP_F16)
        relu_kernel<_Float16, f16x8><<<grid, 256, 0, st>>>((const _Float16*)in, in_bstride, (_Float16*)out, out_bstride, n8);
    else if (dtype == GPP_F32)
        relu_kernel<float, f32x8><<<grid, 256, 0, st>>>((const float*)in, in_bstride, (float*)out, out_bstride, n8);
    else
        return GPP_ERR_UNSUPPORTED;
    return result();
}

extern "C" int gpp_relu(const void* in, void* out, int dtype, int64_t count, void* stream)
{
    return gpp_relu_strided(in, 0, out, 0, dtype, 1, count, stream);
}
```

### ground-plane-polling_amd/keras_retinanet_3D/backend/hip.py

```python

import ctypes
import os

_LIB = None
_HERE = os.path.dirname(os.path.abspath(__file__))
LIB_PATH = os.environ.get('GPP_LIB') or os.path.normpath(os.path.join(_HERE, '..', '..', 'lib', 'libgpp_hip.so'))
CSRC_DIR = os.path.normpath(os.path.join(_HERE, '..', '..', 'csrc'))

GPP_OK = 0
_ERRORS = {
    -1: 'GPP_ERR_BAD_ARG',
    -2: 'GPP_ERR_WORKSPACE',
    -3: 'GPP_ERR_ALIGN',
    -4: 'GPP_ERR_UNSUPPORTED',
}

c_void_p = ctypes.c_void_p
c_int = ctypes.c_int
c_float = ctypes.c_float
c_size_t = ctypes.c_size_t
c_int64 = ctypes.c_int64


GPP_BF16 = 1
GPP_F16 = 2
GPP_F32 = 3
GPP_BF16X3 = 4
GPP_F16X3 = 5
GPP_MAX_GROUPS = 5
GPP_DRAW_PRIM_WORDS = 16
GPP_DRAW_PRIMS_PER_DET = 26
GPP_DRAW_COUNT_WORDS = 4
GPP_POSE_COLS = 36
GPP_EVAL_MAX_DETECTIONS, GPP_EVAL_MAX_ANNOTATIONS = 1024, 1024
GPP_EVAL_ANN_COLS, GPP_EVAL_ERR_COLS = 17, 11
GPP_KITTI_MAX_DETECTIONS, GPP_KITTI_MAX_LABELS = 128, 128
GPP_KITTI_MAX_THRESHOLDS, GPP_KITTI_LABEL_COLS = 41, 16
GPP_LABEL_MOD_COLS = 20
GPP_ABSMAX_F32, GPP_ABSMAX_SPLIT_F16, GPP_ABSMAX_SPLIT_BF16 = 1, 2, 3


class GppError(RuntimeError):
    pass


class ConvGroup(ctypes.Structure):
    _fields_ = [('in_off', c_int64), ('in_bstride', c_int64), ('out_off', c_int64), ('out_bstride', c_int64),
                ('res_off', c_int64), ('res_bstride', c_int64),
                ('H_in', ctypes.c_int32), ('W_in', ctypes.c_int32), ('H_out', ctypes.c_int32), ('W_out', ctypes.c_int32),
                ('H_res', ctypes.c_int32), ('W_res', ctypes.c_int32), ('tile_start', ctypes.c_int32),
                ('row_begin', ctypes.c_int32)]


class ConvDesc(ctypes.Structure):
    _fields_ = [('inp', c_void_p), ('weight', c_void_p), ('bias', c_void_p), ('residual', c_void_p),
                ('out', c_void_p), ('zero_page', c_void_p),
                ('dtype', ctypes.c_int32), ('out_f32', ctypes.c_int32),
                ('batch', ctypes.c_int32), ('C_in', ctypes.c_int32), ('C_out', ctypes.c_int32),
                ('KH', ctypes.c_int32), ('KW', ctypes.c_int32), ('stride', ctypes.c_int32),
                ('pad_top', ctypes.c_int32), ('pad_left', ctypes.c_int32),
                ('in_pitch', ctypes.c_int32), ('out_pitch', ctypes.c_int32), ('res_pitch', ctypes.c_int32),
                ('weight_rows', ctypes.c_int32), ('relu', ctypes.c_int32), ('n_groups', ctypes.c_int32),
                ('tile_hint', ctypes.c_int32), ('reserved', ctypes.c_int32),
                ('in_bytes', ctypes.c_int32), ('weight_bytes', ctypes.c_int32),
                ('partial', c_void_p), ('partial_bytes', c_int64), ('split_k', ctypes.c_int32), ('partial_rows', ctypes.c_int32),
                ('groups', ConvGroup * GPP_MAX_GROUPS),
                ('x3_split', ctypes.c_int32), ('reserved2', ctypes.c_int32), ('out_scale', c_void_p), ('range_counter', c_void_p),
                ('gather_rows', c_void_p), ('gather_counts', c_void_p), ('guard', c_void_p),
                ('guard_value', ctypes.c_int32), ('reserved3', ctypes.c_int32)]


class PixelListDesc(ctypes.Structure):
    _fields_ = [('workspace', c_void_p), ('bitmap', c_void_p), ('rows', c_void_p), ('counts', c_void_p), ('flag', c_void_p),
                ('n_anchors', c_int64)] + \
               [(n, ctypes.c_int32) for n in ('B', 'num_base_anchors', 'lists_per_image', 'n_levels', 'max_rows', 'reserved')] + \
               [('level_pixels', ctypes.c_int32 * GPP_MAX_GROUPS), ('reserved2', ctypes.c_int32)]


class MobileNetBlockDesc(ctypes.Structure):
    _fields_ = [('inp', c_void_p), ('dw_weight', c_void_p), ('dw_bias', c_void_p), ('pw_weight', c_void_p), ('pw_bias', c_void_p),
                ('out_scale', c_void_p), ('out', c_void_p)] + \
               [(n, ctypes.c_int32) for n in ('dtype', 'B', 'H', 'W', 'C_in', 'C_out', 'stride', 'in_pitch', 'out_pitch', 'weight_rows',
                                              'tile_hint', 'reserved')]


class MobileNetStemDesc(ctypes.Structure):
    _fields_ = [('inp', c_void_p), ('weight', c_void_p), ('bias', c_void_p), ('out', c_void_p)] + \
               [(n, ctypes.c_int32) for n in ('B', 'H', 'W', 'C_out', 'out_pitch', 'reserved')]


class AbsmaxDesc(ctypes.Structure):
    _fields_ = [('inp', c_void_p), ('out', c_void_p), ('M', c_int64), ('pitch', c_int64)] + \
               [(n, ctypes.c_int32) for n in ('C', 'c_off', 'layout', 'reserved')]


class AbsmaxClearDesc(ctypes.Structure):
    _fields_ = [('table', c_void_p), ('n', c_int64)]


def _declare(lib):
    lib.gpp_version.restype = ctypes.c_char_p
    lib.gpp_version.argtypes = []
    lib.gpp_poll_workspace_bytes.restype = c_int
    lib.gpp_poll_workspace_bytes.argtypes = [c_int, c_int, c_int, ctypes.POINTER(c_size_t)]
    lib.gpp_poll_f32.restype = c_int
    lib.gpp_poll_f32.argtypes = [c_void_p] * 5 + [c_int, c_int, c_int, c_int, c_float] + [c_void_p] * 4 + \
        [c_void_p, c_size_t, c_void_p]
    lib.gpp_pose_f32.restype = c_int
    lib.gpp_pose_f32.argtypes = [c_void_p] * 8 + [c_int, c_int, c_float] + [c_void_p] * 3
    if hasattr(lib, 'gpp_draw_build'):
        lib.gpp_draw_workspace_bytes.restype = c_int
        lib.gpp_draw_workspace_bytes.argtypes = [c_int, c_int, ctypes.POINTER(c_size_t), ctypes.POINTER(c_size_t)]
        lib.gpp_draw_build.restype = c_int
        lib.gpp_draw_build.argtypes = [c_void_p, c_void_p, c_int, c_int, c_float, c_void_p, c_void_p, c_void_p]
        lib.gpp_draw_raster.restype = c_int
        lib.gpp_draw_raster.argtypes = [c_void_p, c_void_p, c_int, c_int, c_void_p, c_void_p, c_int, c_void_p, c_void_p, c_void_p]
    if hasattr(lib, 'gpp_eval_match_f32'):
        lib.gpp_eval_match_f32.restype = c_int
        lib.gpp_eval_match_f32.argtypes = [c_void_p] * 8 + [c_int] * 4 + [c_float, c_int, ctypes.c_double] + [c_void_p] * 4
    if hasattr(lib, 'gpp_kitti_overlaps_f64'):
        lib.gpp_kitti_overlaps_f64.restype = c_int
        lib.gpp_kitti_overlaps_f64.argtypes = [c_void_p] * 3 + [c_int] * 3 + [c_void_p] * 2
        lib.gpp_kitti_stats_f64.restype = c_int
        lib.gpp_kitti_stats_f64.argtypes = [c_void_p] * 4 + [ctypes.POINTER(ctypes.c_double)] + [c_void_p] * 2 + [c_int] * 4 + [c_void_p] * 5
    if hasattr(lib, 'gpp_label_prep_f64'):
        lib.gpp_label_prep_f64.restype = c_int
        lib.gpp_label_prep_f64.argtypes = [c_void_p] * 4 + [c_int, c_int, ctypes.c_uint, c_int] + [c_void_p] * 7
    if hasattr(lib, 'gpp_detect_pixel_lists'):
        lib.gpp_detect_pixel_lists.restype = c_int
        lib.gpp_detect_pixel_lists.argtypes = [ctypes.POINTER(PixelListDesc), c_void_p]
    lib.gpp_conv2d_igemm.restype = c_int
    lib.gpp_conv2d_igemm.argtypes = [ctypes.POINTER(ConvDesc), c_void_p]
    lib.gpp_stem_conv7x7_bn_relu.restype = c_int
    lib.gpp_stem_conv7x7_bn_relu.argtypes = [c_void_p, c_void_p, c_void_p, c_void_p, c_int, c_int, c_int, c_int, c_void_p]
    lib.gpp_stem_conv7x7_bn_relu_mfma.restype = c_int
    lib.gpp_stem_conv7x7_bn_relu_mfma.argtypes = [c_void_p, c_void_p, c_void_p, c_void_p, c_int, c_int, c_int, c_int, c_void_p]
    lib.gpp_stem_pack_weights_f16.restype = c_int
    lib.gpp_stem_pack_weights_f16.argtypes = [c_void_p, c_void_p, c_size_t]
    lib.gpp_stem_pack_weights_f16x3.restype = c_int
    lib.gpp_stem_pack_weights_f16x3.argtypes = [c_void_p, c_void_p, c_size_t]
    lib.gpp_stem_conv7x7_bn_relu_x3.restype = c_int
    lib.gpp_stem_conv7x7_bn_relu_x3.argtypes = [c_void_p, c_void_p, c_void_p, c_void_p, c_int, c_int, c_int, c_void_p]
    lib.gpp_stem_pool_fused_mfma.restype = c_int
    lib.gpp_stem_pool_fused_mfma.argtypes = [c_void_p, c_void_p, c_void_p, c_void_p, c_int, c_int, c_int, c_int, c_void_p]
    lib.gpp_maxpool3x3s2_same.restype = c_int
    lib.gpp_maxpool3x3s2_same.argtypes = [c_void_p, c_void_p, c_int, c_int, c_int, c_int, c_int, c_void_p]
    lib.gpp_conv2d_preact.restype = c_int
    lib.gpp_conv2d_preact.argtypes = [ctypes.POINTER(ConvDesc), c_void_p, c_void_p, c_void_p]
    lib.gpp_conv2d_preact_tile_candidates.restype = c_int
    lib.gpp_conv2d_preact_tile_candidates.argtypes = [ctypes.POINTER(ConvDesc), ctypes.POINTER(c_int), c_int, ctypes.POINTER(c_int)]
    lib.gpp_conv2d_preact_autotune.restype = c_int
    lib.gpp_conv2d_preact_autotune.argtypes = [ctypes.POINTER(ConvDesc), c_void_p, c_void_p, c_int, c_void_p, ctypes.POINTER(c_float)]
    lib.gpp_maxpool3x3s2_pad_f32.restype = c_int
    lib.gpp_maxpool3x3s2_pad_f32.argtypes = [c_void_p, c_void_p, c_int, c_int, c_int, c_int, c_int, c_int, c_void_p]
    lib.gpp_avgpool2x2_f32.restype = c_int
    lib.gpp_avgpool2x2_f32.argtypes = [c_void_p, c_void_p, c_int, c_int, c_int, c_int, c_int, c_void_p]
    lib.gpp_mobilenet_block.restype = c_int
    lib.gpp_mobilenet_block.argtypes = [ctypes.POINTER(MobileNetBlockDesc), c_void_p]
    lib.gpp_mobilenet_block_tile_candidates.restype = c_int
# ... 261 lines not shown
```

### ground-plane-polling_amd/keras_retinanet_3D/models/plan.py

```python

import collections
import ctypes

import numpy as np

from ..backend import hip
from ..layers import conv as C


class StemDesc(ctypes.Structure):
    _fields_ = [('inp', ctypes.c_void_p), ('weight', ctypes.c_void_p), ('bias', ctypes.c_void_p), ('out', ctypes.c_void_p),
                ('dtype', ctypes.c_int32), ('B', ctypes.c_int32), ('H', ctypes.c_int32), ('W', ctypes.c_int32), ('range_counter', ctypes.c_void_p)]


class PoolDesc(ctypes.Structure):
    _fields_ = [('inp', ctypes.c_void_p), ('out', ctypes.c_void_p), ('dtype', ctypes.c_int32), ('B', ctypes.c_int32),
                ('H', ctypes.c_int32), ('W', ctypes.c_int32), ('C', ctypes.c_int32), ('reserved', ctypes.c_int32)]


class RaggedStemDesc(ctypes.Structure):
    _fields_ = [('stem', StemDesc), ('heights', ctypes.c_void_p), ('Hp', ctypes.c_int32), ('reserved', ctypes.c_int32)]


class RaggedPoolDesc(ctypes.Structure):
    _fields_ = [('pool', PoolDesc), ('heights', ctypes.c_void_p), ('Hp', ctypes.c_int32), ('reserved', ctypes.c_int32)]


class ReluDesc(ctypes.Structure):
    _fields_ = [('inp', ctypes.c_void_p), ('out', ctypes.c_void_p), ('in_bstride', ctypes.c_int64),
                ('out_bstride', ctypes.c_int64), ('count', ctypes.c_int64), ('dtype', ctypes.c_int32), ('B', ctypes.c_int32)]


class DetectDesc(ctypes.Structure):
    _fields_ = [(n, ctypes.c_void_p) for n in ('cls_logits', 'regression', 'regression_dim', 'anchors', 'boxes', 'dims',
                                               'scores', 'labels', 'orientations', 'anchor_index', 'counts', 'workspace')] + \
               [('workspace_bytes', ctypes.c_size_t), ('n_anchors', ctypes.c_int64),
                ('B', ctypes.c_int32), ('num_base_anchors', ctypes.c_int32), ('fused_layout', ctypes.c_int32),
                ('max_det', ctypes.c_int32), ('score_thr', ctypes.c_float), ('iou_thr', ctypes.c_float)]


class CandidatePixelsDesc(ctypes.Structure):
    _fields_ = [('detect', ctypes.c_void_p), ('lists', hip.PixelListDesc)]


class PollDesc(ctypes.Structure):
    _fields_ = [(n, ctypes.c_void_p) for n in ('boxes', 'dims', 'orient', 'P_inv', 'planes', 'keypoints', 'keyplanes',
                                               'residuals', 'best_idx', 'workspace')] + \
               [('workspace_bytes', ctypes.c_size_t), ('B', ctypes.c_int32), ('D', ctypes.c_int32), ('N', ctypes.c_int32),
                ('planes_batched', ctypes.c_int32), ('thr', ctypes.c_float), ('reserved', ctypes.c_int32)]


class PoseDesc(ctypes.Structure):
    _fields_ = [(n, ctypes.c_void_p) for n in ('boxes', 'dims', 'scores', 'labels', 'orientations', 'keypoints', 'residuals',
                                               'frame_info', 'rows', 'counts')] + \
               [('B', ctypes.c_int32), ('D', ctypes.c_int32), ('score_thr', ctypes.c_float), ('reserved', ctypes.c_int32)]


class PreactDesc(ctypes.Structure):
    _fields_ = [('conv', ctypes.c_void_p), ('in_scale', ctypes.c_void_p), ('in_shift', ctypes.c_void_p)]


class DensePoolDesc(ctypes.Structure):
    _fields_ = [('inp', ctypes.c_void_p), ('out', ctypes.c_void_p), ('B', ctypes.c_int32), ('H', ctypes.c_int32), ('W', ctypes.c_int32),
                ('C', ctypes.c_int32), ('pad', ctypes.c_int32), ('out_pitch', ctypes.c_int32)]


class PlanOp(ctypes.Structure):
    _fields_ = [('kind', ctypes.c_int32), ('tag', ctypes.c_int32), ('desc', ctypes.c_void_p)]


class TailDesc(ctypes.Structure):
    _fields_ = [('conv3x3', ctypes.c_void_p), ('conv1x1', ctypes.c_void_p), ('tile_rows', ctypes.c_int32), ('reserved', ctypes.c_int32)]


class BlockDesc(ctypes.Structure):
    _fields_ = [('conv1x1_a', ctypes.c_void_p), ('conv3x3_b', ctypes.c_void_p), ('conv1x1_c', ctypes.c_void_p), ('tile', ctypes.c_int32), ('reserved', ctypes.c_int32)]


OP_STEM, OP_MAXPOOL, OP_CONV, OP_RELU, OP_DETECT, OP_POLL, OP_TAIL = 1, 2, 3, 4, 5, 6, 7
OP_BLOCK = 16
OP_DETECT_CANDIDATES, OP_DETECT_SELECT, OP_DETECT_EMIT = 8, 9, 10
OP_DETECT_OSF = 12
OP_STEM_POOL = 13
OP_MAXPOOL_PAD, OP_AVGPOOL, OP_CONV_PREACT = 17, 18, 32
OP_MOBILENET_STEM, OP_MOBILENET_BLOCK = 33, 34
OP_POSE = 19
OP_ABSMAX, OP_ABSMAX_CLEAR = 35, 36
OP_STEM_RAGGED, OP_STEM_POOL_RAGGED, OP_MAXPOOL_RAGGED = 37, 38, 39
OP_DETECT_CANDIDATE_PIXELS = 40
DETECT_OPS = (OP_DETECT, OP_DETECT_CANDIDATES, OP_DETECT_SELECT, OP_DETECT_EMIT, 12, OP_DETECT_CANDIDATE_PIXELS)
OP_JOIN, OP_SYNC = 0x10000, 0x20000


PlanOptions = collections.namedtuple('PlanOptions', 'x3_level fuse_stem_pool stage_chunks half_stages fuse_tail fuse_block fuse_block_proj '
                                                    'br1_lane fpn_lanes p4_lane head_lanes decode_overlap cls_lane autotune tune_key sparse_heads')


def block_form(opts, width, projection, split_input, halves, join):
    if width in opts.fuse_block and (not projection or opts.fuse_block_proj) and split_input:
        launch = 'block'
    else:
        launch = 'tail' if width in opts.fuse_tail else 'convs'
    if not projection:
        return launch, 'identity'
    return launch, 'side' if opts.br1_lane and not halves and not join else 'inline'


def part_of(fm, c0, nb):
    return C.FMap(fm.buf, nb, fm.H, fm.W, fm.C, off=fm.off + c0 * fm.bstride, bstride=fm.bstride, pitch=fm.pitch, split=fm.split, half=fm.half)


TOWER_SLICES = {('pyramid_towers_0', 0): 'pyramid_regression_0', ('pyramid_towers_0', 512): 'pyramid_classification_0',
                ('pyramid_towers_0', 768): 'pyramid_regression_dim_0'}
RANGE_AUDIT_THRESHOLD = 2.0 ** -9
X3_QUANTUM = 2.0 ** -24
SPARSE_HEADS_MAX_SHARE = '0.5'


def audit_report(maps, table, threshold=RANGE_AUDIT_THRESHOLD):
    table = np.ascontiguousarray(table).view(np.uint32).reshape(-1)
    out = []
    for m in maps:
        first, n = m['row']
        bits = table[first:first + n]
        vals = bits.view(np.float32).astype(np.float64)
        live = vals[bits != 0]
        finite = live[~np.isnan(live)]
        absmax = float('nan') if len(finite) < len(live) else float(finite.max()) if len(finite) else 0.0
        rec = {k: m[k] for k in ('name', 'consumers', 'channels') if k in m}
        rec.update({'live': int(len(live)), 'absmax': absmax,
                    'absmax_min_live': float(finite.min()) if len(finite) else None,
                    'absmax_median_live': float(np.median(finite)) if len(finite) else None,
                    'small_channels': int((finite < threshold).sum()),
                    'bits': None if not absmax > 0 else int(min(22, max(0, np.floor(np.log2(absmax / X3_QUANTUM))))) if np.isfinite(absmax) else 22,
                    'flagged': bool(0 < absmax < threshold)})
        out.append(rec)
    return out


class SparseHeads(object):

    def __init__(self, torch, device, B, level_pixels, max_share):
        i32 = torch.int32
        self.B, self.level_pixels = B, [int(p) for p in level_pixels]
        total = B * sum(self.level_pixels)
        self.max_rows = max(0, min(total, int(max_share * total)))
        self.bitmap = torch.zeros((sum((B * p + 31) // 32 for p in self.level_pixels),), dtype=i32, device=device)
        self.rows = torch.zeros((total,), dtype=i32, device=device)
        self.counts = torch.zeros((hip.GPP_MAX_GROUPS + 1,), dtype=i32, device=device)
        self.flag = torch.ones((1,), dtype=i32, device=device)
        self.dense, self.gathered = [], []
        self.lists_joined = False

    def tensors(self):
        return [self.bitmap, self.rows, self.counts, self.flag]

    def put_every_nth(self, torch, n=8):
        begin, counts = 0, []
        for p in self.level_pixels:
            idx = torch.arange(0, self.B * p, n, dtype=torch.int32, device=self.rows.device)
            self.rows[begin:begin + idx.numel()] = idx
            counts.append(int(idx.numel()))
            begin += self.B * p
        counts += [0] * (hip.GPP_MAX_GROUPS - len(counts)) + [sum(counts)]
        self.counts.copy_(torch.as_tensor(counts, dtype=torch.int32))

    def reset(self, torch):
        self.counts.zero_()
        self.flag.fill_(1)


class Plan(object):

    def __init__(self):
        self.keep = []
        self.io = {}
        self.io_parts = {}
        self.tuning_parts = {}
        self.ops = []
        self.oracle_names = {}
        self.lanes = []
        self.access = []
        self.atomic = []
        self.wrote = []
        self.op_io = []
        self.audit_table = None
        self.audit_maps = []
        self.audit_unobserved = []
        self.inner = {}
        self.open_lanes = set()
        self.conv_descs = []
        self.ws_need = {}
        self.array = None
        self.flops = 0.0
        self.ragged = False
        self.heights = None
        self.sparse = None
        self.heads_stale = False

    @property
    def regression(self):
        self.complete_heads()
        return self._regression

    @regression.setter
    def regression(self, tensor):
        self._regression = tensor

    @property
    def regression_dim(self):
        self.complete_heads()
        return self._regression_dim

    @regression_dim.setter
    def regression_dim(self, tensor):
        self._regression_dim = tensor

    def complete_heads(self):
        if self.sparse is None or not self.heads_stale:
            return
        self.heads_stale = False
        for guarded in self.sparse.dense:
            d = type(guarded).from_buffer_copy(guarded)
            d.guard, d.guard_value = None, 0
            hip.check(hip.lib().gpp_conv2d_igemm(ctypes.byref(d), hip.stream_ptr()), 'gpp_conv2d_igemm (head tensors completed)')

    def emit(self, kind, desc, name, reads=(), writes=(), tag=0, flops=0.0, lane=0, join=False, sync=False, io=None, inner=(), atomic=()):
        self.keep += list(inner) + [desc]
        if inner:
            self.inner[id(desc)] = tuple(inner)
        self.ops.append((kind, tag, desc, name, flops))
        self.lanes.append((int(lane) << 8) | (OP_JOIN if join else 0) | (OP_SYNC if sync else 0))
        self.access.append((self.spans(reads), self.spans(writes)))
        self.atomic.append(self.spans(atomic))
        self.wrote.append([x for x in writes if isinstance(x, C.FMap)])
        self.op_io.append(io)
        self.flops += flops
        if lane:
            self.open_lanes.add(lane)
        elif join:
            self.open_lanes.clear()
        if io is not None:
            self.io[name] = io
            self.io_parts.setdefault(name, []).append(io)

    @staticmethod
    def span(fm):
        e = fm.buf.element_size()
        base = fm.buf.data_ptr() + fm.off * e
        size = ((fm.H * fm.W - 1) * fm.pitch + fm.C) * e
        return [(base + b * fm.bstride * e, base + b * fm.bstride * e + size) for b in range(fm.B)]

    @staticmethod
    def span_of(tensor):
        return [(tensor.data_ptr(), tensor.data_ptr() + tensor.numel() * tensor.element_size())]

    @staticmethod
    def spans(items):
        return [iv for x in items for iv in (Plan.span(x) if isinstance(x, C.FMap) else Plan.span_of(x))]

    def insert_behind(self, extra):
        old = (self.ops, self.lanes, self.access, self.atomic, self.wrote, self.op_io)
        self.ops, self.lanes, self.access, self.atomic, self.wrote, self.op_io = [], [], [], [], [], []
        for pos, row in enumerate(zip(*old)):
            for dst, item in zip((self.ops, self.lanes, self.access, self.atomic, self.wrote, self.op_io), row):
                dst.append(item)
            for kind, desc, name, reads, atomic in extra.get(pos, ()):
                self.keep.append(desc)
                self.ops.append((kind, 0, desc, name, 0.0))
                self.lanes.append(row[1] & 0xff00)
                self.access.append((self.spans(reads), []))
                self.atomic.append(self.spans(atomic))
                self.wrote.append([])
                self.op_io.append(None)

    def check_stream_ordering(self):
        def overlap(a, b):
            return any(x0 < y1 and y0 < x1 for x0, x1 in a for y0, y1 in b)
        bad, seen = [], []
        active = {}
        forks, joins = {}, []
        for pos, (kind, _, desc, name, _) in enumerate(self.ops):
            flags = self.lanes[pos]
            lane, join, sync = (flags >> 8) & 0xff, bool(flags & OP_JOIN), bool(flags & OP_SYNC)
            if lane > 0:
                if not active.get(lane) or sync:
                    forks.setdefault(lane, []).append(pos)
                    active[lane] = True
            elif join:
                joins.append(pos)
                active = {}
            reads, writes = self.access[pos]
            atomic = self.atomic[pos]
            for p0, l0, n0, r0, w0, a0 in seen:
                if l0 == lane or not (overlap(w0, reads) or overlap(w0, writes) or overlap(r0, writes) or overlap(a0, reads) or
                                      overlap(a0, writes) or overlap(w0, atomic) or overlap(r0, atomic)):
                    continue
                j = [q for q in joins if p0 < q <= pos]
                if l0 == 0:
                    ok = any(p0 < f <= pos for f in forks.get(lane, []))
                elif lane == 0:
                    ok = bool(j)
                else:
                    ok = bool(j) and any(min(j) <= f <= pos for f in forks.get(lane, []))
                if not ok:
                    bad.append((n0, name))
            seen.append((pos, lane, name, reads, writes, atomic))
# ... 26 lines not shown
```

### ground-plane-polling_amd/keras_retinanet_3D/models/retinanet.py

```python

import ctypes
import json
import os

import numpy as np

from ..backend import hip
from ..layers import conv as C
from ..layers import mobilenet as M
from ..layers.filter_detections import MAX_DETECTIONS, NMS_THRESHOLD, SCORE_THRESHOLD
from ..utils import anchors as anchor_utils
from ..utils.gpp_utils import POLL_THRESHOLD, POSE_SCORE_THRESHOLD
from . import weights as W
from .plan import (BlockDesc, CandidatePixelsDesc, DensePoolDesc, DetectDesc, PlanOp, PollDesc, PoolDesc, PoseDesc,
                   PreactDesc, RaggedPoolDesc, RaggedStemDesc, ReluDesc, StemDesc, TailDesc,
                   OP_STEM, OP_MAXPOOL, OP_CONV, OP_RELU, OP_DETECT, OP_POLL, OP_TAIL, OP_BLOCK,
                   OP_DETECT_CANDIDATES, OP_DETECT_SELECT, OP_DETECT_EMIT, OP_DETECT_OSF, OP_STEM_POOL,
                   OP_MAXPOOL_PAD, OP_AVGPOOL, OP_CONV_PREACT, OP_MOBILENET_STEM, OP_MOBILENET_BLOCK, OP_POSE,
                   OP_ABSMAX, OP_ABSMAX_CLEAR, OP_STEM_RAGGED, OP_STEM_POOL_RAGGED, OP_MAXPOOL_RAGGED,
                   OP_DETECT_CANDIDATE_PIXELS, DETECT_OPS, OP_JOIN, OP_SYNC,
                   PlanOptions, block_form, part_of, TOWER_SLICES, RANGE_AUDIT_THRESHOLD, X3_QUANTUM,
                   SPARSE_HEADS_MAX_SHARE, audit_report, SparseHeads, Plan)


class RetinaNet3D(object):

    def __init__(self, weights, backbone_name='resnet50', dtype='f16x3', nms=True, class_specific_filter=True,
                 orientation_specific_filter=False, name='retinanet-bbox', on_range_event=None, plan=None, pose=False, range_audit=False):
        import torch
        self.audit = bool(range_audit)
        if self.audit and dtype != 'f16x3':
            raise ValueError("range_audit=True watches the lower range of dtype='f16x3', got dtype={!r}: the IEEE-half pair is a fixed-point "
                             "number with a quantum of 2^-24 below 2^-14; bf16 halves keep float32's exponent and have no such regime, "
                             "and the other types store no split halves".format(dtype))
        self.small_magnitude_events = 0
        self.last_range_audit = None
        self._last_plan = None
        self.pose = bool(pose)
        self.plan_mode = plan or os.environ.get('GPP_PLAN', 'throughput')
        if self.plan_mode not in ('throughput', 'latency'):
            raise ValueError("plan must be 'throughput' or 'latency', got {!r}".format(self.plan_mode))
        self.on_range_event = on_range_event or os.environ.get('GPP_ON_RANGE_EVENT', 'f32')
        if self.on_range_event not in ('f32', 'raise', 'ignore'):
            raise ValueError("on_range_event must be 'f32', 'raise' or 'ignore', got {!r}".format(self.on_range_event))
        self.range_fallbacks = 0
        self._twin = None
        self._weights = weights if (dtype == 'f16x3' and self.on_range_event == 'f32') else None
        self.class_specific_filter = class_specific_filter
        self.osf = bool(orientation_specific_filter)
        self.nms = bool(nms)
        self.name = name
        self.mobilenet = W.is_mobilenet(backbone_name)
        self.backbone_name = backbone_name if self.mobilenet else backbone_name.split('_')[0]
        self.densenet = W.is_densenet(self.backbone_name)
        if self.backbone_name not in W.BLOCKS and not self.densenet and not self.mobilenet:
            raise ValueError('Backbone (\'{}\') not in allowed backbones ({}).'.format(
                backbone_name, sorted(W.BLOCKS) + sorted(W.DENSENET_BLOCKS) + ['{}_<{}>'.format(r, '|'.join(str(a) for a in W.MOBILENET_ALPHAS))
                                                                              for r in W.MOBILENET_ROWS]))
        if dtype not in ('bf16', 'f16', 'f32', 'bf16x3', 'f16x3'):
            raise ValueError("dtype must be 'bf16', 'f16', 'f32', 'bf16x3' or 'f16x3', got {!r}".format(dtype))
        if self.densenet and dtype not in ('f32', 'f16x3', 'bf16x3'):
            raise ValueError("a DenseNet backbone runs with dtype 'f32', 'f16x3' or 'bf16x3', got {!r}".format(dtype))
        if self.mobilenet and dtype not in ('f32', 'f16x3', 'bf16x3'):
            raise ValueError("a MobileNet backbone runs with dtype 'f32', 'f16x3' or 'bf16x3', got {!r}".format(dtype))
        self.dtype = dtype
        self.esz = C.elem_size(dtype)
        self.tdtype = C.torch_dtype(dtype)
        self.device = hip.require_device()
        hip.lib()
        self.torch = torch
        self._plans = {}
        self._anchors = {}
        self._taps, self._ragged_taps = {}, {}
        self._tuned = {}
        self.stem_x3 = False
        self._load_tune_cache()
        self._upload(weights)
        self.tag_names = []

    def _upload(self, weights):
        torch, dev = self.torch, self.device
        W.validate_weights(weights, self.backbone_name)
        self.conv_w = {}
        self.conv_scale = {}

        def put(name, kernel, bias):
            self.conv_w[name] = (C.pack_weight(kernel, self.dtype, dev), torch.as_tensor(bias).to(dev).contiguous(),
                                 kernel.shape)
            if self.dtype == 'f16x3':
                self.conv_scale[name] = C.out_scale_of(kernel, dev)

        if self.densenet:
            self._upload_densenet(weights, put)
        if self.mobilenet:
            self._upload_mobilenet(weights)
        for conv, bn, kh, kw, cin, cout, _ in (() if self.densenet or self.mobilenet else W.backbone_layers(self.backbone_name)):
            k, b = W.folded_conv(weights, conv, bn)
            if k.shape != (kh, kw, cin, cout):
                raise ValueError('weight {} has shape {}, expected {}'.format(conv, k.shape, (kh, kw, cin, cout)))
            if conv == 'conv1':
                if self.dtype in C.X3_TYPES and os.environ.get('GPP_X3_STEM', 'mfma') != 'valu':
                    self.stem_w = hip.pack_stem_weights_x3(k.reshape(147, 64), dev)
                    self.stem_x3 = True
                elif self.esz == 4:
                    self.stem_w = torch.as_tensor(np.ascontiguousarray(k.reshape(147, 64), dtype=np.float32)).to(dev).contiguous()
# ... 227 lines not shown
            d = M.block_desc(x, y, dw_w, dw_b, pw_w, pw_b, scale, stride, self.dtype)
            plan.emit(OP_MOBILENET_BLOCK, d, 'conv_pw_{}'.format(i), [x], [y], flops=M.block_flops(d), io=([x], [y], None))
            x = y
            if i in W.MOBILENET_TAPS:
                feats.append(x)
        return feats

    def _pyramid(self, plan, opts, B, H, Wd, C3, C4, C5):
        got = [(C3.H, C3.W), (C4.H, C4.W), (C5.H, C5.W)]
        shapes = anchor_utils.pyramid_shapes_of_features(got) if self.densenet else anchor_utils.pyramid_shapes((H, Wd))
        if got != [tuple(s) for s in shapes[:3]]:
            raise RuntimeError('backbone / pyramid shape mismatch: {} vs {}'.format(got, shapes))
        pix = [h * w for h, w in shapes]
        total = sum(pix)
        plan.n_anchors = total * anchor_utils.NUM_BASE_ANCHORS
        x3s = opts.x3_level >= 1

        def pyramid(c, dtype=None):
            buf = self.torch.empty((B, total, c), dtype=dtype or self.tdtype, device=self.device)
            plan.keep.append(buf)
            sp = x3s and dtype is None
            return buf, [C.FMap(buf, B, h, w, c, off=sum(pix[:i]) * c, bstride=total * c, split=sp, half=self.dtype if sp else 'bf16x3')
                         for i, (h, w) in enumerate(shapes)]
        return shapes, pyramid

    def _fpn(self, plan, opts, C3, C4, C5, pyramid, smap):
        _, P = pyramid(512)
        l_p5, l_p6 = (1, 2) if opts.fpn_lanes else (0, 0)
        T5 = smap(C5.H, C5.W, 512)
        self._conv(plan, 'C5_reduced', [C5], [T5], 1, join=bool(plan.open_lanes))
        self._conv(plan, 'P5', [T5], [P[2]], 3, pad=(1, 1), lane=l_p5)
        self._conv(plan, 'P6', [C5], [P[3]], 3, stride=2, pad=(C.same_pad(C5.H, 3, 2)[1], C.same_pad(C5.W, 3, 2)[1]), lane=l_p6)
        R6 = smap(P[3].H, P[3].W, 512)
        relu_d = ReluDesc(P[3].buf.data_ptr() + P[3].off * self.esz, R6.buf.data_ptr(), P[3].bstride, R6.bstride, P[3].H * P[3].W * 512,
                          C.gpp_dtype(self.dtype) if opts.x3_level >= 1 else C.gpp_storage_dtype(self.dtype), P[3].B)
        plan.emit(OP_RELU, relu_d, 'C6_relu', [P[3]], [R6], lane=l_p6)
        plan.relu_io = (P[3], R6)
        self._conv(plan, 'P7', [R6], [P[4]], 3, stride=2, pad=(C.same_pad(P[3].H, 3, 2)[1], C.same_pad(P[3].W, 3, 2)[1]), lane=l_p6)
        T4 = smap(C4.H, C4.W, 512)
        self._conv(plan, 'C4_reduced', [C4], [T4], 1, residuals=[T5])
        self._conv(plan, 'P4', [T4], [P[1]], 3, pad=(1, 1), lane=opts.p4_lane, sync=bool(opts.p4_lane))
        T3 = smap(C3.H, C3.W, 512)
        self._conv(plan, 'C3_reduced', [C3], [T3], 1, residuals=[T4])
        self._conv(plan, 'P3', [T3], [P[0]], 3, pad=(1, 1))
        return P

    def _detect(self, plan, B, anchors, pyramid):
        torch, dev, D = self.torch, self.device, MAX_DETECTIONS
        f32, i32 = torch.float32, torch.int32
        plan.cls_logits, cls_o = pyramid(96, f32)
        plan.regression, reg_o = pyramid(144, f32)
        plan.regression_dim, dim_o = pyramid(36, f32)
        plan.boxes = torch.empty((B, D, 12), dtype=f32, device=dev)
        plan.dimensions = torch.empty((B, D, 3), dtype=f32, device=dev)
        plan.scores = torch.empty((B, D), dtype=f32, device=dev)
        plan.labels = torch.empty((B, D), dtype=i32, device=dev)
        plan.orientations = torch.empty((B, D), dtype=i32, device=dev)
        plan.anchor_index = torch.empty((B, D), dtype=i32, device=dev)
        plan.counts = torch.zeros((B,), dtype=i32, device=dev)
        need = hip.c_size_t(0)
        if self.osf and B > 16:
            raise ValueError('orientation_specific_filter=True handles at most 16 images per batch')
        size_fn = hip.lib().gpp_detect_osf_workspace_bytes if self.osf else hip.lib().gpp_detect_workspace_bytes
        hip.check(size_fn(B, plan.n_anchors, need), 'gpp_detect_workspace_bytes')
        plan.detect_ws = ws = torch.empty((int(need.value),), dtype=torch.uint8, device=dev)
        plan.anchors = anchors
        dd = DetectDesc(plan.cls_logits.data_ptr(), plan.regression.data_ptr(), plan.regression_dim.data_ptr(),
                        anchors.data_ptr(), plan.boxes.data_ptr(), plan.dimensions.data_ptr(), plan.scores.data_ptr(),
                        plan.labels.data_ptr(), plan.orientations.data_ptr(), plan.anchor_index.data_ptr(),
                        plan.counts.data_ptr(), ws.data_ptr(), ws.numel(), plan.n_anchors,
                        B, anchor_utils.NUM_BASE_ANCHORS, 1, D, SCORE_THRESHOLD, NMS_THRESHOLD if self.nms else 2.0)
        heads = [plan.cls_logits, plan.regression, plan.regression_dim]
        dets = [plan.boxes, plan.dimensions, plan.scores, plan.labels, plan.orientations, plan.anchor_index]
        access = {OP_DETECT_CANDIDATES: ([plan.cls_logits], [ws, plan.counts]), OP_DETECT_SELECT: ([ws, plan.regression], [ws]),
                  OP_DETECT_EMIT: (heads + [ws], dets)}

        def decode(kind, name='filtered_detections', **flags):
            reads, writes = access.get(kind, (heads, dets + [ws, plan.counts]))
            if kind == OP_DETECT_CANDIDATE_PIXELS:
                sp = plan.sparse
                lists = hip.PixelListDesc(ws.data_ptr(), sp.bitmap.data_ptr(), sp.rows.data_ptr(), sp.counts.data_ptr(), sp.flag.data_ptr(),
                                          plan.n_anchors, B, anchor_utils.NUM_BASE_ANCHORS, 4 if self.osf else 1, len(sp.level_pixels),
                                          sp.max_rows, 0, (ctypes.c_int32 * hip.GPP_MAX_GROUPS)(*sp.level_pixels), 0)
                reads, writes = access[OP_DETECT_CANDIDATES]
                plan.emit(kind, CandidatePixelsDesc(ctypes.addressof(dd), lists), name, reads, writes + sp.tensors(), inner=(dd,), **flags)
                return
            plan.emit(kind, dd, name, reads, writes, **flags)
        return (cls_o, reg_o, dim_o), decode

    def _heads(self, plan, opts, P, pyramid, outs, decode):
        cls_o, reg_o, dim_o = outs
        _, wide = pyramid(896)
        self._conv(plan, 'pyramid_towers_0', P, wide, 3, pad=(1, 1), relu=True, join=True)

        def tower(prefix, width, c0, out_name, out, tag=0, lane=0, join=False):
            src = [C.FMap(m.buf, m.B, m.H, m.W, width, off=m.off + c0, bstride=m.bstride, pitch=m.pitch, split=m.split, half=m.half)
                   for m in wide]
            for i in range(1, 4):
                _, dst = pyramid(width)
                self._conv(plan, '{}_{}'.format(prefix, i), src, dst, 3, pad=(1, 1), relu=True, tag=tag, lane=lane)
                src = dst
            out_layer(out_name, src, out, lane, join)

        def out_layer(name, src, out, lane, join):
            sp = plan.sparse
            kh, kw, cin, cout = self.conv_w[name][2]
            pixels = sum(f.H * f.W for f in out)
            split = (C.latency_split if self.plan_mode == 'latency' else C.default_split)(kh, kw, cin, cout, pixels)
            if sp is None or name == 'pyramid_classification' or lane or split > 1:
                self._conv(plan, name, src, out, 3, pad=(1, 1), out_f32=True, lane=lane, join=join)
                if sp is not None and join and not lane:
                    sp.lists_joined = True
                return
            dense = self._desc(plan, name, src, out, 3, pad=(1, 1), out_f32=True, lane=lane)
            dense.guard, dense.guard_value = sp.flag.data_ptr(), 1
            plan.emit(OP_CONV, dense, name, list(src) + [sp.flag], out, flops=C.conv_flops(dense), lane=lane, join=join or not sp.lists_joined,
                      io=(src, out, None))
            sp.lists_joined = True
            rows = self._desc(plan, name, src, out, 3, pad=(1, 1), out_f32=True, lane=lane)
            rows.gather_rows, rows.gather_counts, rows.split_k = sp.rows.data_ptr(), sp.counts.data_ptr(), 1
            rows.guard, rows.guard_value = sp.flag.data_ptr(), 0
            plan.emit(OP_CONV, rows, name, list(src) + [sp.rows, sp.counts, sp.flag], out, lane=lane, io=(src, out, None))
            sp.dense.append(dense)
            sp.gathered.append(rows)

        l_dim, l_cls = (1, 2) if opts.head_lanes else (0, 0)
        towers = {'cls': ('pyramid_classification', 256, 512, 'pyramid_classification', cls_o, 0, l_cls or opts.cls_lane),
                  'reg': ('pyramid_regression', 512, 0, 'pyramid_regression_ops', reg_o, 1, 0, bool(opts.cls_lane)),
                  'dim': ('pyramid_regression_dim', 128, 768, 'pyramid_regression_dim', dim_o, 0, l_dim)}
        if opts.sparse_heads:
            plan.sparse = SparseHeads(self.torch, self.device, P[0].B, [m.H * m.W for m in P], opts.sparse_heads)
            plan.keep += plan.sparse.tensors()
        if opts.decode_overlap:
            tower(*towers['cls'])
            decode(OP_DETECT_CANDIDATE_PIXELS if plan.sparse else OP_DETECT_CANDIDATES, 'filtered_detections/candidates',
                   lane=opts.cls_lane or 1)
            tower(*towers['reg'])
            decode(OP_DETECT_SELECT, 'filtered_detections/select', lane=1, sync=True)
            tower(*towers['dim'])
            decode(OP_DETECT_EMIT, join=True)
        else:
            for t in ('dim', 'cls', 'reg'):
                tower(*towers[t])
            decode(OP_DETECT_OSF if self.osf else OP_DETECT, join=True)

    def _poll(self, plan, B, n_planes, planes_batched):
        torch, dev, D = self.torch, self.device, MAX_DETECTIONS
        plan.keypoints = torch.empty((B, D, 4, 3), dtype=torch.float32, device=dev)
        plan.keyplanes = torch.empty((B, D, 1, 4), dtype=torch.float32, device=dev)
        plan.residuals = torch.empty((B, D), dtype=torch.float32, device=dev)
        plan.best_index = torch.empty((B, D), dtype=torch.int32, device=dev)
        need = hip.c_size_t(0)
        hip.check(hip.lib().gpp_poll_workspace_bytes(B, n_planes, int(planes_batched), need), 'gpp_poll_workspace_bytes')
        plan.poll_ws = torch.empty((max(int(need.value), 16),), dtype=torch.uint8, device=dev)
        pd = PollDesc(plan.boxes.data_ptr(), plan.dimensions.data_ptr(), plan.orientations.data_ptr(), plan.P_inv.data_ptr(),
                      plan.planes.data_ptr(), plan.keypoints.data_ptr(), plan.keyplanes.data_ptr(), plan.residuals.data_ptr(),
                      plan.best_index.data_ptr(), plan.poll_ws.data_ptr(), plan.poll_ws.numel(), B, D, n_planes,
                      int(planes_batched), POLL_THRESHOLD, 0)
        plan.emit(OP_POLL, pd, 'fit_road_planes', [plan.boxes, plan.dimensions, plan.orientations, plan.P_inv, plan.planes],
                  [plan.keypoints, plan.keyplanes, plan.residuals, plan.best_index, plan.poll_ws], tag=2,
                  flops=162.0 * B * D * n_planes)

    def _pose(self, plan, B):
        torch, dev, D = self.torch, self.device, MAX_DETECTIONS
        n = B * D * hip.GPP_POSE_COLS
        plan.pose_out = torch.zeros((n + 2 + B,), dtype=torch.float32, device=dev)
        plan.pose_rows = plan.pose_out[:n].view(B, D, hip.GPP_POSE_COLS)
        plan.pose_counts = plan.pose_out[n + 2:].view(torch.int32)
        plan.frame_info = torch.tensor([[1.0, plan.shape[1], plan.shape[2]]] * B, dtype=torch.float32, device=dev)
        pd = PoseDesc(plan.boxes.data_ptr(), plan.dimensions.data_ptr(), plan.scores.data_ptr(), plan.labels.data_ptr(),
                      plan.orientations.data_ptr(), plan.keypoints.data_ptr(), plan.residuals.data_ptr(), plan.frame_info.data_ptr(),
                      plan.pose_rows.data_ptr(), plan.pose_counts.data_ptr(), B, D, POSE_SCORE_THRESHOLD, 0)
        plan.emit(OP_POSE, pd, 'recover_pose', [plan.boxes, plan.dimensions, plan.scores, plan.labels, plan.orientations, plan.keypoints,
                                                plan.residuals, plan.frame_info], [plan.pose_rows, plan.pose_counts])

    def _audit(self, plan):
        torch, esz = self.torch, self.esz
        views, order = {}, []

        def key_of(f):
            return (f.buf.data_ptr(), f.pitch, f.off % f.pitch, f.C)

        for pos, (kind, _, desc, name, _) in enumerate(plan.ops):
            io = plan.op_io[pos]
            if kind == OP_CONV_PREACT:
                lo, hi = min(a for a, _ in Plan.spans(io[0])), max(b for _, b in Plan.spans(io[0]))
                plan.audit_unobserved.append({'name': name + '/operand', 'consumers': [name], 'extent': (lo, hi),
                                              'reason': 'max(x * scale + shift, 0) is formed after the load (gpp_conv2d_preact)'})
            elif kind == OP_MOBILENET_BLOCK:
                plan.audit_unobserved.append({'name': name.replace('conv_pw_', 'conv_dw_'), 'consumers': [name], 'extent': None,
                                              'reason': 'the depthwise result lives in LDS (gpp_mobilenet_block); bounded by ReLU6'})
            elif kind == OP_CONV:
                for f in list(io[0]) + list(io[2] or []):
                    k = key_of(f)
                    if k not in views:
                        views[k] = {'consumers': [], 'producers': [], 'channels': f.C, 'spans': [], 'fmaps': [], 'split': f.split,
                                    'layout': 'split_f16' if f.split else 'f32'}
                        order.append(k)
                    if name not in views[k]['consumers']:
                        views[k]['consumers'].append(name)
                    views[k]['spans'] += Plan.span(f)
                    if not any((g.off, g.B, g.H, g.W) == (f.off, f.B, f.H, f.W) for g in views[k]['fmaps']):
                        views[k]['fmaps'].append(f)
        offset = 0
        for k in order:
            views[k]['row'] = (offset, k[3])
            offset += k[3]
        plan.audit_table = table = torch.zeros((max(offset, 1),), dtype=torch.int32, device=self.device)
        extra = {}
        for pos, (kind, _, desc, name, _) in enumerate(plan.ops):
            for k in order:
                ptr, pitch, c0, c = k
                outs = [o for o in plan.wrote[pos] if o.buf.data_ptr() == ptr and o.pitch == pitch]
                if not outs:
                    continue
                oc0, oc = outs[0].off % pitch, outs[0].C
                lo, hi = max(c0, oc0), min(c0 + c, oc0 + oc)
                if lo >= hi:
                    continue
                v = views[k]
                if name not in v['producers']:
                    v['producers'].append(name)
                runs = []
                for start, n in sorted(((o.off - oc0 + b * o.bstride) // pitch, o.H * o.W) for o in outs for b in range(o.B)):
                    if runs and runs[-1][0] + runs[-1][1] == start:
                        runs[-1][1] += n
                    else:
                        runs.append([start, n])
                row = table[v['row'][0] + lo - c0:v['row'][0] + hi - c0]
                for start, n in runs:
                    d = hip.AbsmaxDesc(ptr + start * pitch * esz, row.data_ptr(), n, pitch, hi - lo, lo,
                                       hip.GPP_ABSMAX_SPLIT_F16 if v['split'] else hip.GPP_ABSMAX_F32, 0)
                    extra.setdefault(pos, []).append((OP_ABSMAX, d, 'absmax:' + name, outs, [row]))
        plan.insert_behind(extra)
        plan.keep.append(table)
        clear = hip.AbsmaxClearDesc(table.data_ptr(), table.numel())
        plan.emit(OP_ABSMAX_CLEAR, clear, 'absmax:clear', [], [table])
        for lst in (plan.ops, plan.lanes, plan.access, plan.atomic, plan.wrote, plan.op_io):
            lst.insert(0, lst.pop())
        for k in order:
            v = views[k]
            names = v['producers']
            if not names:
                raise RuntimeError('range audit: no launch of the plan writes the operand of {}'.format(v['consumers']))
            name = TOWER_SLICES.get((names[0], k[2]), names[0]) if len(names) == 1 else \
                '+'.join(sorted(names)) if len(names) <= 5 else '{}..{}'.format(names[0], names[-1])
            plan.audit_maps.append({'name': name, 'producers': names, 'consumers': v['consumers'], 'channels': v['channels'],
                                    'layout': v['layout'], 'row': v['row'], 'fmaps': v['fmaps'],
                                    'extent': (min(a for a, _ in v['spans']), max(b for _, b in v['spans']))})

    def _bind_workspaces(self, plan):
        plan.workspaces = {lane: self.torch.empty((max(need, 16),), dtype=self.torch.uint8, device=self.device)
                           for lane, need in plan.ws_need.items()}
        for d, lane in plan.conv_descs:
            d.partial = plan.workspaces[lane].data_ptr()
            d.partial_bytes = plan.workspaces[lane].numel()

    def _plan_options(self, B):
        env = os.environ.get
        x3 = self.dtype in C.X3_TYPES
        x3_level = int(env('GPP_X3_SPLIT', '2')) if x3 else 0
        chunks = env('GPP_STAGE_CHUNKS')
        fuse_tail = [int(v) for v in env('GPP_FUSE_TAIL', '64,128').split(',') if v.strip() and int(v) > 0]
        if x3:
            fuse_tail = [v for v in fuse_tail if v == 64] if x3_level >= 2 else []
        elif self.esz == 4:
            fuse_tail = []
        fuse_block = [int(v) for v in env('GPP_FUSE_BLOCK', '64,128').split(',') if v.strip()] if (x3 and x3_level >= 2) else []
        if self.audit:
            fuse_tail, fuse_block = [], []
        head_lanes = env('GPP_HEAD_LANES', '0') != '0'
        fpn_lanes = head_lanes or env('GPP_FPN_LANES', '1') != '0'
        overlap = env('GPP_DECODE_OVERLAP', '1') != '0' and not head_lanes and not self.osf
        return PlanOptions(
            x3_level=x3_level,
            fuse_stem_pool=not self.densenet and not self.mobilenet and (self.esz == 2 or self.stem_x3) and env('GPP_FUSE_STEM_POOL', '1') != '0',
            stage_chunks=tuple(max(1, min(B, int(v))) for v in chunks.split(',')) if chunks else (B,) * 4,
            half_stages=frozenset(int(v) for v in env('GPP_HALF_LANES', '0,1,2,3').split(',') if v.strip()) if B >= 2 else frozenset(),
            fuse_tail=tuple(v for v in fuse_tail if v in (64, 128)),
            fuse_block=tuple(v for v in fuse_block if v in (64, 128)),
            fuse_block_proj=env('GPP_FUSE_BLOCK_PROJ', '0') != '0',
            br1_lane=env('GPP_BR1_LANE', '1') != '0',
            fpn_lanes=fpn_lanes,
            p4_lane=1 if (fpn_lanes and env('GPP_P4_LANE', '1') != '0') else 0,
            head_lanes=head_lanes,
            decode_overlap=overlap,
            cls_lane=2 if (overlap and env('GPP_CLS_LANE', '1' if B <= 2 else '0') != '0') else 0,
            autotune=env('GPP_AUTOTUNE', '1') != '0',
            sparse_heads=(max(1e-9, float(env('GPP_SPARSE_HEADS_MAX_SHARE', SPARSE_HEADS_MAX_SHARE)))
                          if (overlap and not self.audit and env('GPP_SPARSE_HEADS', '1') != '0') else 0.0),
            tune_key='x3split={};fuse={}/{};plan={}{}'.format(env('GPP_X3_SPLIT', '2'), env('GPP_FUSE_TAIL', '64,128'), env('GPP_FUSE_BLOCK', '64,128'),
                                                              self.plan_mode, C.latency_split_config() if self.plan_mode == 'latency' else '') +
                     (';audit' if self.audit else ''))

    def _build(self, B, H, Wd, n_planes, planes_batched, ragged=False):
        torch, dev = self.torch, self.device
        if ragged:
            if self.mobilenet or self.densenet:
                raise ValueError('{} has no ragged form: {}; run its images grouped by shape'.format(
                    self.backbone_name, 'its first block runs at conv1\'s resolution, which differs inside a height class' if self.mobilenet
                    else 'its zero-padded pool1 (gpp_maxpool3x3s2_pad_f32) has no per-image form'))
            if self.audit:
                raise ValueError('range_audit=True has no ragged form: the audit of the conv1 map reads rows that a shorter image does not have')
            if H % 4:
                raise ValueError('the canvas of a ragged plan has 4 Hp rows, got {}'.format(H))
        opts = self._plan_options(B)
        plan = Plan()
        plan.shape = (B, H, Wd, n_planes, planes_batched)
        plan.ragged = bool(ragged)
        if ragged:
            plan.heights = torch.full((B,), H, dtype=torch.int32, device=dev)
            plan.heights_host = [H] * B
        plan.side_lanes = {'fpn': opts.fpn_lanes, 'branch1': opts.br1_lane, 'p4': bool(opts.p4_lane),
                           'half_batch_stages': sorted(opts.half_stages), 'cls_tower': bool(opts.cls_lane)}
        plan.decode_overlap = opts.decode_overlap
        plan.range_slot = torch.zeros((1,), dtype=torch.int64, device=dev)
        plan.range_seen = 0
        plan.images = torch.empty((B, H, Wd, 3), dtype=torch.float32, device=dev)
        plan.P_inv = torch.empty((B, 4, 3), dtype=torch.float32, device=dev)
        plan.planes = torch.empty((B, n_planes, 4) if planes_batched else (n_planes, 4), dtype=torch.float32, device=dev)

        def fmap(h, w, c, split=False):
            f = C.FMap.empty(B, h, w, c, self.tdtype, dev, half=self.dtype if self.dtype in C.X3_TYPES else 'bf16x3')
            plan.keep.append(f.buf)
            return f.mark_split() if split else f

        backbone = self._densenet_backbone if self.densenet else self._mobilenet_backbone if self.mobilenet else self._resnet_backbone
        C2, C3, C4, C5 = backbone(plan, opts, B, H, Wd, fmap, lambda h, w, c: fmap(h, w, c, opts.x3_level >= 2))
        plan.features = {'stem': plan.stem_out, 'C2': C2, 'C3': C3, 'C4': C4, 'C5': C5}
        shapes, pyramid = self._pyramid(plan, opts, B, H, Wd, C3, C4, C5)
        P = self._fpn(plan, opts, C3, C4, C5, pyramid, lambda h, w, c: fmap(h, w, c, opts.x3_level >= 1))
        plan.features.update({'P{}'.format(i + 3): P[i] for i in range(5)})
        outs, decode = self._detect(plan, B, self._anchor_table((H, Wd), shapes if self.densenet else None), pyramid)
        self._heads(plan, opts, P, pyramid, outs, decode)
        self._poll(plan, B, n_planes, planes_batched)
        if self.pose:
            self._pose(plan, B)
        if self.audit:
            self._audit(plan)
        self._bind_workspaces(plan)
        plan.finalize()
        plan.tagged = [name for _, tag, _, name, _ in plan.ops if tag]
        if opts.autotune:
            self._autotune(plan)
        return plan

    def _tune_cache_path(self):
        return os.environ.get('GPP_TUNE_CACHE')

    def _tune_config(self):
        ver = hip.lib().gpp_version().decode().split('src:')[-1]
        return 'v2;{};{}'.format(ver, self._plan_options(1).tune_key)

    def _load_tune_cache(self):
        path = self._tune_cache_path()
        if path and os.path.exists(path):
            with open(path) as f:
                for key, val in json.load(f).items():
                    parts = key.split('|')
                    if len(parts) != 7:
                        continue
                    cfg, bb, dt, name, b, h, w = parts
                    if cfg == self._tune_config() and bb == self.backbone_name and dt == self.dtype:
                        self._tuned[(name, int(b), int(h), int(w))] = (int(val[0]), float(val[-1]))

    def _save_tune_cache(self):
        path = self._tune_cache_path()
        if not path or int(os.environ.get('RANK', '0')) != 0:
            return
        data = {}
        if os.path.exists(path):
            try:
                with open(path) as f:
                    data = json.load(f)
            except ValueError:
                data = {}
        for (name, b, h, w), val in self._tuned.items():
            data['|'.join([self._tune_config(), self.backbone_name, self.dtype, name, str(b), str(h), str(w)])] = list(val)
        tmp = '{}.tmp.{}'.format(path, os.getpid())
        with open(tmp, 'w') as f:
            json.dump(data, f, indent=0, sort_keys=True)
        os.replace(tmp, path)

    def _autotune(self, plan):
        self._require_hip()
        H, Wd = plan.shape[1:3]
        plan.images.uniform_(-120.0, 130.0)
        fresh = False
        plan.tuning = {}
        rnd = None
        if os.environ.get('GPP_TUNE_RANDOM'):
            import random
            rnd = random.Random(int(os.environ['GPP_TUNE_RANDOM']) * 1000003 + int(os.environ.get('RANK', '0')))
        for index, (kind, _, desc, name, flops) in enumerate(plan.ops):
            if kind in DETECT_OPS or kind == OP_POLL:
                continue
            gathered = kind == OP_CONV and bool(desc.gather_rows)
            if kind == OP_CONV and desc.guard:
                plan.sparse.flag.fill_(0 if gathered else 1)
                if gathered:
                    plan.sparse.put_every_nth(self.torch)
                    name = name + '@rows'
            self.run_op(plan, index)
            if kind not in (OP_CONV, OP_TAIL, OP_CONV_PREACT, OP_MOBILENET_BLOCK):
                continue
            target = plan.inner[id(desc)][0] if kind == OP_CONV_PREACT else desc
            field = 'tile_rows' if kind == OP_TAIL else 'tile_hint'
            if rnd is not None:
                setattr(target, field, rnd.choice(self._tile_choices(plan, index, kind, target)))
                plan.tuning[name] = (int(getattr(target, field)), 0.0)
                self.run_op(plan, index)
                continue
            key = (name, target.B if kind == OP_MOBILENET_BLOCK else (plan.inner[id(desc)][0] if kind == OP_TAIL else target).batch, H, Wd)
            if kind == OP_CONV and key in self._tuned and not self._tile_is_listed(desc, self._tuned[key][0]):
                del self._tuned[key]
            if key not in self._tuned:
                self._tuned[key] = self._time_tiles(plan, index, kind, desc, target, flops)
                fresh = True
            setattr(target, field, self._tuned[key][0])
            plan.tuning[name] = self._tuned[key]
            plan.tuning_parts.setdefault(name, []).append(self._tuned[key])
        if plan.sparse is not None:
            plan.sparse.reset(self.torch)
        self.torch.cuda.synchronize()
        if fresh:
            self._save_tune_cache()

    def _tile_choices(self, plan, index, kind, target):
        if kind == OP_TAIL:
            return (64, 96, 128, 160) if self.dtype in C.X3_TYPES else (96, 128, 160)
        lib, tiles, count = hip.lib(), (ctypes.c_int * 32)(), ctypes.c_int(0)
        if kind == OP_MOBILENET_BLOCK:
            hip.check(lib.gpp_mobilenet_block_tile_candidates(ctypes.byref(target), tiles, 16, ctypes.byref(count)),
                      'gpp_mobilenet_block_tile_candidates')
            return list(tiles[:min(count.value, 16)])
        if kind == OP_CONV_PREACT:
            hip.check(lib.gpp_conv2d_preact_tile_candidates(ctypes.byref(target), tiles, 16, ctypes.byref(count)),
                      'gpp_conv2d_preact_tile_candidates')
            return list(tiles[:min(count.value, 16)])
        hip.check(lib.gpp_conv2d_tile_candidates(ctypes.byref(target), tiles, 32, ctypes.byref(count)), 'gpp_conv2d_tile_candidates')
        ok = []
        for tile in tiles[:count.value]:
            target.tile_hint = tile
            if lib.gpp_plan_run(ctypes.byref(plan.array, index * ctypes.sizeof(PlanOp)), 1, hip.stream_ptr(), None, 0) == 0:
                ok.append(tile)
        return ok

    def _time_tiles(self, plan, index, kind, desc, target, flops):
        if kind == OP_TAIL:
            times = {}
            for rows in self._tile_choices(plan, index, kind, target):
                if rows == 64 and os.environ.get('GPP_TAIL64', '1') == '0':
                    continue
                desc.tile_rows = rows
                e0, e1 = self.torch.cuda.Event(enable_timing=True), self.torch.cuda.Event(enable_timing=True)
                self.run_op(plan, index)
                e0.record()
                for _ in range(16):
                    self.run_op(plan, index)
                e1.record()
                e1.synchronize()
                times[rows] = e0.elapsed_time(e1) * 1000.0 / 16
            rows = min(times, key=times.get)
            return rows, round(times[rows], 2)
        slow = self.dtype == 'f32'
        iters = (2 if slow else 6) if flops > 5e10 else (4 if slow else 16)
        best = ctypes.c_float(0.0)
        if kind == OP_MOBILENET_BLOCK:
            hip.check(hip.lib().gpp_mobilenet_block_autotune(ctypes.byref(target), iters, hip.stream_ptr(), ctypes.byref(best)),
                      'gpp_mobilenet_block_autotune')
        elif kind == OP_CONV_PREACT:
            hip.check(hip.lib().gpp_conv2d_preact_autotune(ctypes.byref(target), desc.in_scale, desc.in_shift, iters, hip.stream_ptr(),
                                                           ctypes.byref(best)), 'gpp_conv2d_preact_autotune')
        else:
            hip.check(hip.lib().gpp_conv2d_autotune(ctypes.byref(target), iters, hip.stream_ptr(), ctypes.byref(best)), 'gpp_conv2d_autotune')
        return int(target.tile_hint), round(float(best.value), 2)

    @staticmethod
    def _tile_is_listed(desc, tile):
        tiles, count = (ctypes.c_int * 64)(), ctypes.c_int(0)
        hip.check(hip.lib().gpp_conv2d_tile_candidates(ctypes.byref(desc), tiles, 64, ctypes.byref(count)), 'gpp_conv2d_tile_candidates')
        return int(tile) in list(tiles[:min(count.value, 64)])

    def x3_range_events(self, reset=False):
        if self.dtype != 'f16x3':
# ... 466 lines not shown
```

### include/gpp.h

```cpp
#ifndef GPP_H_
#define GPP_H_

#include <stddef.h>
#include <stdint.h>

#ifdef __cplusplus
extern "C" {
#endif

#define GPP_OK 0
#define GPP_ERR_BAD_ARG (-1)
#define GPP_ERR_WORKSPACE (-2)
#define GPP_ERR_ALIGN (-3)
#define GPP_ERR_UNSUPPORTED (-4)

const char* gpp_version(void);

int gpp_poll_workspace_bytes(int B, int N, int planes_batched, size_t* bytes);

int gpp_poll_f32(const float* boxes, const float* dims, const int32_t* orient, const float* P_inv,
                 const float* planes, int B, int D, int N, int planes_batched, float thr,
                 float* keypoints, float* keyplanes, float* residuals, int32_t* best_idx,
                 void* workspace, size_t workspace_bytes, void* stream);

// ... 75 lines not shown

int gpp_conv2d_preact(const gpp_conv_desc* host_desc, const float* in_scale, const float* in_shift, void* stream);
int gpp_conv2d_preact_tile_candidates(const gpp_conv_desc* host_desc, int* tiles, int capacity, int* count);
int gpp_conv2d_preact_autotune(gpp_conv_desc* desc, const float* in_scale, const float* in_shift, int iters, void* stream, float* best_us);
int gpp_maxpool3x3s2_pad_f32(const float* in, float* out, int B, int H, int W, int C, int pad, int out_pitch, void* stream);
int gpp_avgpool2x2_f32(const float* in, float* out, int B, int H, int W, int C, int out_pitch, void* stream);

typedef struct gpp_mobilenet_block_desc {
    const float* in; const float* dw_weight; const float* dw_bias; const void* pw_weight; const float* pw_bias; const float* out_scale;
    float* out;
    int32_t dtype, B, H, W, C_in, C_out, stride, in_pitch, out_pitch, weight_rows, tile_hint, reserved;
} gpp_mobilenet_block_desc;
typedef struct gpp_mobilenet_stem_desc { const float* in; const float* weight; const float* bias; float* out; int32_t B, H, W, C_out, out_pitch, reserved; } gpp_mobilenet_stem_desc;
int gpp_mobilenet_block(const gpp_mobilenet_block_desc* host_desc, void* stream);
int gpp_mobilenet_block_tile_candidates(const gpp_mobilenet_block_desc* host_desc, int* tiles, int capacity, int* count);
int gpp_mobilenet_block_autotune(gpp_mobilenet_block_desc* desc, int iters, void* stream, float* best_us);
int gpp_mobilenet_stem(const float* in, const float* weight, const float* bias, float* out, int B, int H, int W, int C_out, int out_pitch,
                       void* stream);
int gpp_mobilenet_depthwise(const float* in, const float* weight, const float* bias, float* out, int B, int H, int W, int C, int stride,
                            int in_pitch, int out_pitch, void* stream);

int gpp_stem_conv7x7_bn_relu(const float* in, const float* weight, const float* bias, void* out, int dtype,
                             int B, int H, int W, void* stream);
int gpp_stem_pack_weights_f16(const float* host_weight_147x64, void* host_packed, size_t packed_bytes);
int gpp_stem_conv7x7_bn_relu_mfma(const float* in, const void* packed_weight_f16, const float* bias, void* out,
                                  int dtype, int B, int H, int W, void* stream);
int gpp_maxpool3x3s2_same(const void* in, void* out, int dtype, int B, int H, int W, int C, void* stream);
int gpp_stem_pool_fused_mfma(const float* in, const void* packed_weight_f16, const float* bias, void* out,
                             int dtype, int B, int H, int W, void* stream);
int gpp_stem_pack_weights_f16x3(const float* host_weight_147x64, void* host_packed, size_t packed_bytes);
int gpp_stem_conv7x7_bn_relu_x3(const float* in, const void* packed_weight_x3, const float* bias, float* out,
                                int B, int H, int W, void* stream);
int gpp_stem_conv7x7_bn_relu_x3_rc(const float* in, const void* packed_weight_x3, const float* bias, float* out,
                                   int B, int H, int W, uint64_t* range_counter, void* stream);
int gpp_stem_pool_fused_x3(const float* in, const void* packed_weight_x3, const float* bias, float* out,
                           int B, int H, int W, uint64_t* range_counter, void* stream);
int gpp_stem_conv7x7_bn_relu_ragged(const float* in, const float* weight, const float* bias, void* out, int dtype,
                                    int B, int H, int W, int Hp, const int32_t* heights, void* stream);
int gpp_stem_conv7x7_bn_relu_mfma_ragged(const float* in, const void* packed_weight_f16, const float* bias, void* out,
                                         int dtype, int B, int H, int W, int Hp, const int32_t* heights, void* stream);
int gpp_stem_conv7x7_bn_relu_x3_rc_ragged(const float* in, const void* packed_weight_x3, const float* bias, float* out,
                                          int B, int H, int W, int Hp, const int32_t* heights, uint64_t* range_counter, void* stream);
int gpp_maxpool3x3s2_same_ragged(const void* in, void* out, int dtype, int B, int H, int W, int C, int Hp,
                                 const int32_t* heights, void* stream);
int gpp_stem_pool_fused_mfma_ragged(const float* in, const void* packed_weight_f16, const float* bias, void* out,
                                    int dtype, int B, int H, int W, int Hp, const int32_t* heights, void* stream);
int gpp_stem_pool_fused_x3_ragged(const float* in, const void* packed_weight_x3, const float* bias, float* out,
                                  int B, int H, int W, int Hp, const int32_t* heights, uint64_t* range_counter, void* stream);
int gpp_relu(const void* in, void* out, int dtype, int64_t count, void* stream);
int gpp_relu_strided(const void* in, int64_t in_bstride, void* out, int64_t out_bstride, int dtype, int B,
                     int64_t count, void* stream);

int gpp_preprocess_u8_bgr(const uint8_t* frames, float* out, const int32_t* y0, const int32_t* y1, const float* wy,
                          const int32_t* x0, const int32_t* x1, const float* wx, int B, int H, int W, int Ho, int Wo,
                          float mean_b, float mean_g, float mean_r, void* stream);
int gpp_preprocess_u8_bgr_ragged(const uint8_t* frames, float* out, const int32_t* raw_hw, const int32_t* heights,
                                 const int32_t* y0, const int32_t* y1, const float* wy, const int32_t* x0, const int32_t* x1, const float* wx,
                                 int B, int H, int W, int Hp, int Ho, int Wo, float mean_b, float mean_g, float mean_r, void* stream);

int gpp_detect_workspace_bytes(int B, int64_t n_anchors, size_t* bytes);

int gpp_detect_f32(const float* cls_logits, const float* regression, const float* regression_dim,
                   const float* anchors, int B, int64_t n_anchors, int num_base_anchors, int fused_layout,
                   float score_thr, float iou_thr, int max_det,
                   float* boxes, float* dims, float* scores, int32_t* labels, int32_t* orientations,
                   int32_t* anchor_index, int32_t* counts,
                   void* workspace, size_t workspace_bytes, void* stream);

#define GPP_DETECT_CANDIDATES 1
#define GPP_DETECT_SELECT 2
#define GPP_DETECT_EMIT 4
int gpp_detect_stages_f32(int stages, const float* cls_logits, const float* regression, const float* regression_dim,
                          const float* anchors, int B, int64_t n_anchors, int num_base_anchors, int fused_layout,
                          float score_thr, float iou_thr, int max_det,
                          float* boxes, float* dims, float* scores, int32_t* labels, int32_t* orientations,
                          int32_t* anchor_index, int32_t* counts,
                          void* workspace, size_t workspace_bytes, void* stream);

typedef struct gpp_pixel_list_desc {
    const void* workspace; uint32_t* bitmap; int32_t* rows; int32_t* counts; int32_t* flag;
    int64_t n_anchors;
    int32_t B, num_base_anchors, lists_per_image, n_levels, max_rows, reserved;
    int32_t level_pixels[GPP_MAX_GROUPS]; int32_t reserved2;
} gpp_pixel_list_desc;
int gpp_detect_pixel_lists(const gpp_pixel_list_desc* host_desc, void* stream);

int gpp_detect_osf_workspace_bytes(int B, int64_t n_anchors, size_t* bytes);
int gpp_detect_osf_f32(const float* cls_logits, const float* regression, const float* regression_dim,
                       const float* anchors, int B, int64_t n_anchors, int num_base_anchors, int fused_layout,
                       float score_thr, float iou_thr, int max_det,
                       float* boxes, float* dims, float* scores, int32_t* labels, int32_t* orientations,
                       int32_t* anchor_index, int32_t* counts,
                       void* workspace, size_t workspace_bytes, void* stream);

int gpp_pack_detections(const float* boxes, const float* dims, const float* scores, const int32_t* labels,
                        const int32_t* orientations, const float* keypoints, const float* keyplanes,
                        const float* residuals, int B, int D, float* packed, void* stream);

#define GPP_POSE_COLS 36
int gpp_pose_f32(const float* boxes, const float* dims, const float* scores, const int32_t* labels,
                 const int32_t* orientations, const float* keypoints, const float* residuals,
                 const float* frame_info, int B, int D, float score_thr,
                 float* rows, int32_t* counts, void* stream);

#define GPP_EVAL_MAX_DETECTIONS 1024
#define GPP_EVAL_MAX_ANNOTATIONS 1024
#define GPP_EVAL_ANN_COLS 17
#define GPP_EVAL_ERR_COLS 11
int gpp_eval_match_f32(const float* boxes, const float* dims, const float* scores, const int32_t* labels,
                       const int32_t* orientations, const float* scales, const double* annotations,
                       const int32_t* ann_counts, int B, int D, int A, int num_classes, float score_thr,
                       int max_detections, double iou_thr, int32_t* table, double* errors, int32_t* counts, void* stream);

#define GPP_KITTI_MAX_DETECTIONS 128
#define GPP_KITTI_MAX_LABELS 128
#define GPP_KITTI_MAX_THRESHOLDS 41
#define GPP_KITTI_LABEL_COLS 16
int gpp_kitti_overlaps_f64(const float* rows, const double* labels, const int32_t* label_counts, int B, int D, int A,
                           double* overlaps, void* stream);
int gpp_kitti_stats_f64(const float* rows, const double* labels, const int32_t* label_counts, const double* overlaps,
                        const double* min_overlap, const float* thresholds, const int32_t* n_thresholds, int B, int D, int A, int T,
                        float* tp_scores, int32_t* n_gt, int32_t* stats, double* similarity, void* stream);

#define GPP_LABEL_MOD_COLS 20
int gpp_label_prep_f64(const double* labels, const int32_t* label_counts, const double* P, const double* trig, int B, int A,
                       unsigned det_types, int own_box, double* mod,
                       float* boxes, float* dims, float* scores, int32_t* det_labels, int32_t* orientations, void* stream);

#define GPP_DRAW_PRIM_WORDS 16
#define GPP_DRAW_PRIMS_PER_DET 26
#define GPP_DRAW_COUNT_WORDS 4
#define GPP_DRAW_CAPTION_MAX 20
#define GPP_DRAW_NONE 0
#define GPP_DRAW_LINE 1
#define GPP_DRAW_DASHED 2
#define GPP_DRAW_RECT 3
#define GPP_DRAW_CIRCLE 4
#define GPP_DRAW_CAPTION 5
int gpp_draw_workspace_bytes(int B, int D, size_t* prims_bytes, size_t* workspace_bytes);
int gpp_draw_build(const float* rows, const double* P, int B, int D, float score_thr, void* prims, int32_t* counts, void* stream);
int gpp_draw_raster(const uint8_t* frames_u8, const int32_t* raw_hw, int Hr, int Wr, const void* prims, const int32_t* counts,
                    int B, uint8_t* out_u8, void* workspace, void* stream);

#define GPP_ABSMAX_F32 1
#define GPP_ABSMAX_SPLIT_F16 2
#define GPP_ABSMAX_SPLIT_BF16 3
typedef struct gpp_absmax_desc {
    const void* in; uint32_t* out;
    int64_t M, pitch;
    int32_t C, c_off, layout, reserved;
} gpp_absmax_desc;
typedef struct gpp_absmax_clear_desc { uint32_t* table; int64_t n; } gpp_absmax_clear_desc;
int gpp_channel_absmax(const gpp_absmax_desc* desc, void* stream);
int gpp_absmax_clear(uint32_t* table, int64_t n, void* stream);

#define GPP_OP_STEM 1
#define GPP_OP_MAXPOOL 2
#define GPP_OP_CONV 3
#define GPP_OP_RELU 4
#define GPP_OP_DETECT 5
#define GPP_OP_POLL 6
#define GPP_OP_BOTTLENECK_TAIL 7
#define GPP_OP_DETECT_CANDIDATES 8
#define GPP_OP_DETECT_SELECT 9
#define GPP_OP_DETECT_EMIT 10
#define GPP_OP_DETECT_OSF 12
// ... 80 lines not shown
```

Measured before the change: 837.6.

## Run last regression tower conv sparsely on dilated candidate pixel rows

Extends the sparse-heads path so the third regression tower conv only computes output rows in a 3x3-dilated neighbourhood of candidate pixels. It does this with a new pipelined gather kernel on pre-split x3 maps, with device-side choice of tile height. The mark-pixels step builds a dilated bitmap and the compact kernel now emits two row lists. A dense fallback is guarded by an overflow flag. This avoids dense conv work on pixels that feed no detections, at the cost of extra marking atomics, several guarded launches (one per candidate height), and more plan complexity.

```diff
diff --git a/ground-plane-polling_amd/csrc/conv_igemm.hip b/ground-plane-polling_amd/csrc/conv_igemm.hip
--- a/ground-plane-polling_amd/csrc/conv_igemm.hip
+++ b/ground-plane-polling_amd/csrc/conv_igemm.hip
@@ -34,7 +34,10 @@
     if (d.reserved2 != 0 || (d.x3_split & ~(GPP_X3_IN | GPP_X3_OUT | GPP_X3_RES))) return GPP_ERR_BAD_ARG;
     if (d.reserved3 != 0 || (d.gather_rows != nullptr) != (d.gather_counts != nullptr)) return GPP_ERR_BAD_ARG;
     if (((uintptr_t)d.gather_rows | (uintptr_t)d.gather_counts | (uintptr_t)d.guard) & 3) return GPP_ERR_ALIGN;
-    if (d.gather_rows && (d.stride != 1 || d.residual || !d.out_f32 || d.split_k > 1)) return GPP_ERR_UNSUPPORTED;
+    if (d.gather_rows) {
+        const bool presplit = is_x3(d.dtype) && (d.x3_split & (GPP_X3_IN | GPP_X3_OUT)) == (GPP_X3_IN | GPP_X3_OUT);
+        if (d.stride != 1 || d.residual || d.split_k > 1 || !(d.out_f32 || presplit)) return GPP_ERR_UNSUPPORTED;
+    }
     if (d.x3_split && !is_x3(d.dtype)) return GPP_ERR_BAD_ARG;
     if (d.out_scale && d.dtype != GPP_F16X3) return GPP_ERR_BAD_ARG;
     if ((d.x3_split & GPP_X3_OUT) && (d.out_f32 || d.C_out % 32 != 0 || d.out_pitch % 32 != 0)) return GPP_ERR_UNSUPPORTED;
@@ -272,7 +275,9 @@
     const int bn = t.bn;
     const auto pads_less_than = [&](int other) { return (d.C_out + bn - 1) / bn * bn < (d.C_out + other - 1) / other * other; };
     switch (t.form) {
-        case GATHER: return bn != 160 || pads_less_than(64);
+        case GATHER:
+            if (t.owner == X3IN || (d.x3_split & GPP_X3_OUT)) return t.owner == X3IN && (d.x3_split & GPP_X3_OUT);
+            return bn != 160 || pads_less_than(64);
         case DEEP: {
             int64_t tiles_m = 0;
             for (int g = 0; g < d.n_groups; ++g) tiles_m += ((int64_t)d.batch * d.groups[g].H_out * d.groups[g].W_out + t.bm - 1) / t.bm;
diff --git a/ground-plane-polling_amd/csrc/conv_igemm_impl.h b/ground-plane-polling_amd/csrc/conv_igemm_impl.h
--- a/ground-plane-polling_amd/csrc/conv_igemm_impl.h
+++ b/ground-plane-polling_amd/csrc/conv_igemm_impl.h
@@ -95,6 +95,10 @@
 #define GPP_X3_PRIO 1
 #endif
 constexpr bool kSpreadDma = GPP_DMA_SPREAD != 0;
+#ifndef GPP_GATHER_PIPE_REMAP
+#define GPP_GATHER_PIPE_REMAP 0
+#endif
+constexpr bool kGatherPipeRemap = GPP_GATHER_PIPE_REMAP != 0;
 
 #ifndef GPP_X3_SERPENTINE
 #define GPP_X3_SERPENTINE 2
@@ -381,7 +385,8 @@
 {
     static_assert(!XIN || kX3<DT>, "pre-split input maps: GPP_BF16X3 / GPP_F16X3");
     static_assert(!PRE || (!PIPE && !XIN && kF32Storage<DT>), "pre-activation: float32-sized input maps, plain loop");
-    static_assert(!GATHER || (!PIPE && !PRE), "gathered rows: plain loop");
+    static_assert(!GATHER || !PRE, "gathered rows: no pre-activation form");
+    static_assert(!(GATHER && PIPE) || (XIN && kX3<DT>), "gathered rows on a pipelined loop: the x3 types' three-phase loop on pre-split maps");
     if (d.guard != nullptr && *(const volatile int32_t*)d.guard != d.guard_value) return;
     using E = Elem<DT>;
     using vec8 = typename E::vec8;
@@ -405,20 +410,37 @@
     const int wm = wave / WN, wn = wave % WN;
     GPP_STAMP(0);
 
-    const int bid = GATHER ? block_x : xcd_remap(block_x, grid_x);
     const int n_tiles = (d.C_out + BN - 1) / BN;
+    constexpr bool COUNTED = GATHER && PIPE;
+    auto list_rows = [&](int q) { return min(max(d.gather_counts[q], 0), d.batch * d.groups[q].H_out * d.groups[q].W_out); };
+    int live = grid_x;
+    if constexpr (COUNTED) {
+        int t = 0;
+#pragma unroll
+        for (int q = 0; q < GPP_MAX_GROUPS; ++q)
+            if (q < d.n_groups) t += (list_rows(q) + BM - 1) / BM;
+        live = t * n_tiles;
+        if (block_x >= live) return;
+    }
+    const int bid = GATHER ? ((COUNTED && kGatherPipeRemap) ? xcd_remap(block_x, live) : block_x) : xcd_remap(block_x, grid_x);
     const int nt = bid % n_tiles, mt = bid / n_tiles;
     int tile_start = 0, row_begin = 0, H_in = 0, W_in = 0, H_out = 0, W_out = 0, H_res = 0, W_res = 0;
     int64_t in_off = 0, in_bs = 0, out_off = 0, out_bs = 0, res_off = 0, res_bs = 0;
     int list_begin = 0, list_next = 0, group = 0;
+    int counted_next = 0;
 #pragma unroll
     for (int q = 0; q < GPP_MAX_GROUPS; ++q) {
+        int first_tile = d.groups[q].tile_start;
+        if constexpr (COUNTED) {
+            first_tile = counted_next;
+            if (q < d.n_groups) counted_next += (list_rows(q) + BM - 1) / BM;
+        }
         if constexpr (GATHER) {
-            if (q < d.n_groups && mt >= d.groups[q].tile_start) { list_begin = list_next; group = q; }
+            if (q < d.n_groups && mt >= first_tile) { list_begin = list_next; group = q; }
             if (q < d.n_groups) list_next += d.batch * d.groups[q].H_out * d.groups[q].W_out;
         }
-        if (q < d.n_groups && mt >= d.groups[q].tile_start) {
-            tile_start = d.groups[q].tile_start;
+        if (q < d.n_groups && mt >= first_tile) {
+            tile_start = first_tile;
             row_begin = d.groups[q].row_begin;
             H_in = d.groups[q].H_in; W_in = d.groups[q].W_in;
             H_out = d.groups[q].H_out; W_out = d.groups[q].W_out;
@@ -1041,6 +1063,34 @@
     conv_igemm_body<DT, BM, BN, WM, WN, STAGES, false, XIN, false, true>(d, blockIdx.x, gridDim.x);
 }
 
+__device__ __forceinline__ int gather_pipe_height(const gpp_conv_desc& d)
+{
+    constexpr int CUS = 256;
+    const int n_tiles = (d.C_out + 255) / 256;
+    int rows[GPP_MAX_GROUPS];
+#pragma unroll
+    for (int q = 0; q < GPP_MAX_GROUPS; ++q)
+        rows[q] = q < d.n_groups ? min(max(d.gather_counts[q], 0), d.batch * d.groups[q].H_out * d.groups[q].W_out) : 0;
+    int best_h = 256, best_cost = 0x7fffffff;
+#pragma unroll
+    for (int h = 256; h >= 128; h -= 32) {
+        int t = 0;
+#pragma unroll
+        for (int q = 0; q < GPP_MAX_GROUPS; ++q) t += (rows[q] + h - 1) / h;
+        const int cost = (t * n_tiles + CUS - 1) / CUS * h;
+        if (cost < best_cost) { best_cost = cost; best_h = h; }
+    }
+    return best_h;
+}
+
+template <int DT, int BM>
+__global__ __launch_bounds__(512, 2) void conv_gather_pipe_kernel(const gpp_conv_desc d, const int only_if_picked)
+{
+    if (d.guard != nullptr && *(const volatile int32_t*)d.guard != d.guard_value) return;
+    if (only_if_picked && gather_pipe_height(d) != BM) return;
+    conv_igemm_body<DT, BM, 256, 2, 4, 2, true, true, false, true>(d, blockIdx.x, gridDim.x);
+}
+
 template <int DT, int BM, int BN, int WM, int WN>
 __global__ __launch_bounds__(64 * WM * WN, 2) void conv_preact_kernel(const gpp_conv_desc d, const float* in_scale, const float* in_shift)
 {
@@ -2103,6 +2153,7 @@
 template <int DT, int BM, int BN, int WM, int WN, int STAGES, bool XIN = false>
 int launch_gather(gpp_conv_desc& d, hipStream_t st)
 {
+    if (d.x3_split & GPP_X3_OUT) return GPP_ERR_UNSUPPORTED;
     if constexpr (kX3<DT> && !XIN) {
         if (d.x3_split & GPP_X3_IN) return launch_gather<DT, BM, BN, WM, WN, STAGES, true>(d, st);
     }
@@ -2116,6 +2167,26 @@
     const int n_tiles = (d.C_out + BN - 1) / BN;
     kernel<<<dim3((unsigned)(tiles * n_tiles)), dim3(64 * WM * WN), lds, st>>>(d);
     return last_launch_rc();
+}
+
+template <int DT, int BM, bool PICKED>
+int launch_gather_pipe(gpp_conv_desc& d, hipStream_t st)
+{
+    if constexpr (!kX3<DT>) {
+        return kF32Storage<DT> ? GPP_ERR_UNSUPPORTED : GPP_ERR_BAD_ARG;
+    } else {
+        if ((d.x3_split & (GPP_X3_IN | GPP_X3_OUT)) != (GPP_X3_IN | GPP_X3_OUT)) return GPP_ERR_UNSUPPORTED;
+        constexpr int BN = 256;
+        constexpr int lds = 2 * (stage_rows(BM, 8) + BN) * kRowBytes;
+        constexpr auto kernel = conv_gather_pipe_kernel<DT, BM>;
+        const int rc = allow_lds<kernel>(lds);
+        if (rc != GPP_OK) return rc;
+        const int tiles = prepare<BM, BN>(d);
+        if (tiles < 0) return tiles;
+        const int n_tiles = (d.C_out + BN - 1) / BN;
+        kernel<<<dim3((unsigned)(tiles * n_tiles)), dim3(512), lds, st>>>(d, PICKED ? 1 : 0);
+        return last_launch_rc();
+    }
 }
 
 template <int DT, int FORM, int OWNER, int BM, int BN, int WM, int WN, int STAGES>
@@ -2138,7 +2209,11 @@
 #define GPP_RUN_TILE(code, form, owner, bm, bn, wm, wn, stages) \
     case code: return run_tile<DT, gpp_tiles::form, gpp_tiles::owner, bm, bn, wm, wn, stages>(d, st);
 #define GPP_RUN_GATHER(code, form, owner, bm, bn, wm, wn, stages) \
-    case code: if constexpr (gpp_tiles::form == gpp_tiles::GATHER) return launch_gather<DT, bm, bn, wm, wn, stages>(d, st); else break;
+    case code:                                                                                                                  \
+        if constexpr (gpp_tiles::form == gpp_tiles::GATHER && gpp_tiles::owner == gpp_tiles::X3IN)                              \
+            return launch_gather_pipe<DT, bm, (code >= 9000000)>(d, st);                                                        \
+        else if constexpr (gpp_tiles::form == gpp_tiles::GATHER) return launch_gather<DT, bm, bn, wm, wn, stages>(d, st);       \
+        else break;
 #define GPP_RUN_PREACT(code, form, owner, bm, bn, wm, wn, stages) \
     case code: return launch_preact<DT, bm, bn, wm, wn>(d, in_scale, in_shift, st);
 
@@ -2157,7 +2232,7 @@
 int dispatch_gather(gpp_conv_desc& d, hipStream_t st)
 {
     switch (d.tile_hint) {
-        case 0: return launch_gather<DT, 64, 64, 2, 2, 2>(d, st);
+        case 0: return (d.x3_split & GPP_X3_OUT) ? launch_gather_pipe<DT, 256, false>(d, st) : launch_gather<DT, 64, 64, 2, 2, 2>(d, st);
         GPP_CONV_TILES(GPP_RUN_GATHER, GPP_RUN_GATHER, GPP_TILE_NONE)
         default: break;
     }
diff --git a/ground-plane-polling_amd/csrc/conv_tiles.h b/ground-plane-polling_amd/csrc/conv_tiles.h
--- a/ground-plane-polling_amd/csrc/conv_tiles.h
+++ b/ground-plane-polling_amd/csrc/conv_tiles.h
@@ -83,6 +83,17 @@
     T(7064064, GATHER, ALL, 64, 64, 2, 2, 4)                                                                                             \
     T(7032064, GATHER, ALL, 32, 64, 2, 2, 4)                                                                                             \
     T(7064160, GATHER, ALL, 64, 160, 4, 1, 4)                                                                                            \
+                                                                                                                           \
+    T(8256256, GATHER, X3IN, 256, 256, 2, 4, 2)                                                                                          \
+    T(8224256, GATHER, X3IN, 224, 256, 2, 4, 2)                                                                                          \
+    T(8192256, GATHER, X3IN, 192, 256, 2, 4, 2)                                                                                          \
+    T(8160256, GATHER, X3IN, 160, 256, 2, 4, 2)                                                                                          \
+    T(8128256, GATHER, X3IN, 128, 256, 2, 4, 2)                                                                                          \
+    X(9256256, GATHER, X3IN, 256, 256, 2, 4, 2)                                                                                          \
+    X(9224256, GATHER, X3IN, 224, 256, 2, 4, 2)                                                                                          \
+    X(9192256, GATHER, X3IN, 192, 256, 2, 4, 2)                                                                                          \
+    X(9160256, GATHER, X3IN, 160, 256, 2, 4, 2)                                                                                          \
+    X(9128256, GATHER, X3IN, 128, 256, 2, 4, 2)                                                                                          \
     X(64, PLAIN, ALL, 128, 64, 2, 2, 2)                                                                                                  \
     X(128, PLAIN, ALL, 128, 128, 2, 2, 2)                                                                                                \
     X(256, PLAIN, B16, 256, 128, 4, 2, 3)                                                             \
diff --git a/ground-plane-polling_amd/csrc/decode.hip b/ground-plane-polling_amd/csrc/decode.hip
--- a/ground-plane-polling_amd/csrc/decode.hip
+++ b/ground-plane-polling_amd/csrc/decode.hip
@@ -673,11 +673,12 @@
     int pix_begin[GPP_MAX_GROUPS];
     int word_begin[GPP_MAX_GROUPS];
     int list_begin[GPP_MAX_GROUPS];
+    int width[GPP_MAX_GROUPS];
 };
 
 __global__ __launch_bounds__(256) void mark_pixels_kernel(const unsigned long long* __restrict__ keys, const int32_t* __restrict__ cnt,
                                                           int64_t key_stride, int64_t n_anchors, int nba, int lists_per_image,
-                                                          const LevelTable T, uint32_t* __restrict__ bitmap)
+                                                          const LevelTable T, uint32_t* __restrict__ bitmap, uint32_t* __restrict__ dilated)
 {
     const int list = blockIdx.y, b = list / lists_per_image;
     const int64_t n = min((int64_t)max(cnt[list * (kCounterStride / 4)], 0), n_anchors);
@@ -689,14 +690,28 @@
         for (int q = 1; q < T.n_levels; ++q) l = pixel >= T.pix_begin[q] ? q : l;
         const int bit = b * T.pix[l] + (pixel - T.pix_begin[l]);
         atomicOr(&bitmap[T.word_begin[l] + (bit >> 5)], 1u << (bit & 31));
+        if (dilated != nullptr) {
+            const int W = T.width[l], H = T.pix[l] / W;
+            const int p = pixel - T.pix_begin[l], y = p / W, x = p - y * W;
+            for (int yy = max(y - 1, 0); yy <= min(y + 1, H - 1); ++yy)
+                for (int xx = max(x - 1, 0); xx <= min(x + 1, W - 1); ++xx) {
+                    const int nb = b * T.pix[l] + yy * W + xx;
+                    atomicOr(&dilated[T.word_begin[l] + (nb >> 5)], 1u << (nb & 31));
+                }
+        }
     }
 }
 
 constexpr int kCompactThreads = 1024;
-__global__ __launch_bounds__(kCompactThreads) void compact_pixels_kernel(uint32_t* __restrict__ bitmap, const LevelTable T, int B, int max_rows,
-                                                                         int32_t* __restrict__ rows, int32_t* __restrict__ counts,
-                                                                         int32_t* __restrict__ flag)
-{
+struct PlaneOut { uint32_t* bitmap; int32_t* rows; int32_t* counts; int32_t* flag; int max_rows; };
+__global__ __launch_bounds__(kCompactThreads) void compact_pixels_kernel(const PlaneOut first, const PlaneOut second, const LevelTable T, int B)
+{
+    const bool one = blockIdx.x == 0;
+    uint32_t* __restrict__ bitmap = one ? first.bitmap : second.bitmap;
+    int32_t* __restrict__ rows = one ? first.rows : second.rows;
+    int32_t* __restrict__ counts = one ? first.counts : second.counts;
+    int32_t* __restrict__ flag = one ? first.flag : second.flag;
+    const int max_rows = one ? first.max_rows : second.max_rows;
     __shared__ int wave_sum[kCompactThreads / 64];
     const int tid = threadIdx.x, lane = tid & 63, wave = tid >> 6;
     int total = 0;
@@ -755,9 +770,17 @@
     if (d.B < 0 || d.B > kMaxBatch || d.n_anchors <= 0 || d.n_anchors > kMaxAnchors || d.num_base_anchors <= 0 || d.max_rows < 0 ||
         d.n_levels < 1 || d.n_levels > GPP_MAX_GROUPS || (d.lists_per_image != 1 && d.lists_per_image != 4) || d.reserved != 0 || d.reserved2 != 0)
         return GPP_ERR_BAD_ARG;
+    const bool dilate = d.rows_dilated != nullptr;
+    if (dilate != (d.counts_dilated != nullptr) || dilate != (d.flag_dilated != nullptr) || d.max_rows_dilated < 0 || (!dilate && d.max_rows_dilated != 0))
+        return GPP_ERR_BAD_ARG;
+    for (int l = 0; l < GPP_MAX_GROUPS; ++l) {
+        const bool live = dilate && l < d.n_levels;
+        if (live ? (d.level_widths[l] <= 0 || d.level_pixels[l] <= 0 || d.level_pixels[l] % d.level_widths[l] != 0) : d.level_widths[l] != 0) return GPP_ERR_BAD_ARG;
+    }
     if (d.B == 0) return GPP_OK;
     if (!d.workspace || !d.bitmap || !d.rows || !d.counts || !d.flag) return GPP_ERR_BAD_ARG;
     if (((uintptr_t)d.workspace & 15) || (((uintptr_t)d.bitmap | (uintptr_t)d.rows | (uintptr_t)d.counts | (uintptr_t)d.flag) & 3)) return GPP_ERR_ALIGN;
+    if (((uintptr_t)d.rows_dilated | (uintptr_t)d.counts_dilated | (uintptr_t)d.flag_dilated) & 3) return GPP_ERR_ALIGN;
     const int lists = d.B * d.lists_per_image;
     if (lists > 64) return GPP_ERR_UNSUPPORTED;
     LevelTable T;
@@ -771,6 +794,7 @@
         T.pix_begin[l] = (int)pixels;
         T.word_begin[l] = (int)words;
         T.list_begin[l] = (int)((int64_t)d.B * pixels);
+        T.width[l] = d.level_widths[l];
         pixels += pix;
         words += ((int64_t)d.B * pix + 31) / 32;
     }
@@ -780,8 +804,10 @@
     const int32_t* cnt = (const int32_t*)ws;
     const unsigned long long* keys = (const unsigned long long*)(ws + kHeaderBytes);
     mark_pixels_kernel<<<dim3(16, (unsigned)lists), 256, 0, st>>>(keys, cnt, pow2_ceil(d.n_anchors), d.n_anchors, d.num_base_anchors,
-                                                                   d.lists_per_image, T, d.bitmap);
-    compact_pixels_kernel<<<1, kCompactThreads, 0, st>>>(d.bitmap, T, d.B, d.max_rows, d.rows, d.counts, d.flag);
+                                                                   d.lists_per_image, T, d.bitmap, dilate ? d.bitmap + words : nullptr);
+    const PlaneOut first = {d.bitmap, d.rows, d.counts, d.flag, d.max_rows};
+    const PlaneOut second = {d.bitmap + words, d.rows_dilated, d.counts_dilated, d.flag_dilated, d.max_rows_dilated};
+    compact_pixels_kernel<<<dilate ? 2 : 1, kCompactThreads, 0, st>>>(first, second, T, d.B);
     const hipError_t e = hipGetLastError();
     return e == hipSuccess ? GPP_OK : (int)e;
 }
diff --git a/ground-plane-polling_amd/csrc/stem.hip b/ground-plane-polling_amd/csrc/stem.hip
--- a/ground-plane-polling_amd/csrc/stem.hip
+++ b/ground-plane-polling_amd/csrc/stem.hip
@@ -397,6 +397,7 @@
     const int Ho = (H + 1) / 2, Wo = (W + 1) / 2;
     const int pt = ((Ho - 1) * 2 + 3 - H > 0 ? (Ho - 1) * 2 + 3 - H : 0) / 2;
     const int pl = ((Wo - 1) * 2 + 3 - W > 0 ? (Wo - 1) * 2 + 3 - W : 0) / 2;
+    if ((double)B * Ho * Wo * (C / 8) >= 4.0e18) return GPP_ERR_UNSUPPORTED;
     const int64_t total = (int64_t)B * Ho * Wo * (C / 8);
     const unsigned blocks = (unsigned)((total + 255) / 256 < 8192 ? (total + 255) / 256 : 8192);
     hipStream_t st = (hipStream_t)stream;
diff --git a/ground-plane-polling_amd/keras_retinanet_3D/backend/hip.py b/ground-plane-polling_amd/keras_retinanet_3D/backend/hip.py
--- a/ground-plane-polling_amd/keras_retinanet_3D/backend/hip.py
+++ b/ground-plane-polling_amd/keras_retinanet_3D/backend/hip.py
@@ -74,7 +74,9 @@
     _fields_ = [('workspace', c_void_p), ('bitmap', c_void_p), ('rows', c_void_p), ('counts', c_void_p), ('flag', c_void_p),
                 ('n_anchors', c_int64)] + \
                [(n, ctypes.c_int32) for n in ('B', 'num_base_anchors', 'lists_per_image', 'n_levels', 'max_rows', 'reserved')] + \
-               [('level_pixels', ctypes.c_int32 * GPP_MAX_GROUPS), ('reserved2', ctypes.c_int32)]
+               [('level_pixels', ctypes.c_int32 * GPP_MAX_GROUPS), ('reserved2', ctypes.c_int32),
+                ('level_widths', ctypes.c_int32 * GPP_MAX_GROUPS), ('max_rows_dilated', ctypes.c_int32),
+                ('rows_dilated', c_void_p), ('counts_dilated', c_void_p), ('flag_dilated', c_void_p)]
 
 
 class MobileNetBlockDesc(ctypes.Structure):
diff --git a/ground-plane-polling_amd/keras_retinanet_3D/models/plan.py b/ground-plane-polling_amd/keras_retinanet_3D/models/plan.py
--- a/ground-plane-polling_amd/keras_retinanet_3D/models/plan.py
+++ b/ground-plane-polling_amd/keras_retinanet_3D/models/plan.py
@@ -93,7 +93,8 @@
 
 
 PlanOptions = collections.namedtuple('PlanOptions', 'x3_level fuse_stem_pool stage_chunks half_stages fuse_tail fuse_block fuse_block_proj '
-                                                    'br1_lane fpn_lanes p4_lane head_lanes decode_overlap cls_lane autotune tune_key sparse_heads')
+                                                    'br1_lane fpn_lanes p4_lane head_lanes decode_overlap cls_lane autotune tune_key sparse_heads '
+                                                    'sparse_tower sparse_tower_force')
 
 
 def block_form(opts, width, projection, split_input, halves, join):
@@ -115,6 +116,13 @@
 RANGE_AUDIT_THRESHOLD = 2.0 ** -9
 X3_QUANTUM = 2.0 ** -24
 SPARSE_HEADS_MAX_SHARE = '0.5'
+SPARSE_TOWER_MAX_SHARE = '0.5'
+SPARSE_TOWER_DEFAULT = '0'
+SPARSE_TOWER_HEIGHTS = (256, 224, 192, 160, 128)
+
+
+def sparse_tower_applies(B, level_pixels, c_out):
+    return sum((B * p + 255) // 256 for p in level_pixels) * ((c_out + 255) // 256) > 256
 
 
 def audit_report(maps, table, threshold=RANGE_AUDIT_THRESHOLD):
@@ -140,12 +148,21 @@
 
 class SparseHeads(object):
 
-    def __init__(self, torch, device, B, level_pixels, max_share):
+    def __init__(self, torch, device, B, level_pixels, max_share, level_widths=None, max_share_dilated=None):
         i32 = torch.int32
         self.B, self.level_pixels = B, [int(p) for p in level_pixels]
         total = B * sum(self.level_pixels)
         self.max_rows = max(0, min(total, int(max_share * total)))
-        self.bitmap = torch.zeros((sum((B * p + 31) // 32 for p in self.level_pixels),), dtype=i32, device=device)
+        self.dilated = max_share_dilated is not None
+        self.level_widths = [int(w) for w in level_widths] if self.dilated else []
+        self.max_rows_d = max(0, min(total, int(max_share_dilated * total))) if self.dilated else 0
+        words = sum((B * p + 31) // 32 for p in self.level_pixels)
+        self.bitmap = torch.zeros((words * (2 if self.dilated else 1),), dtype=i32, device=device)
+        self.rows_d = torch.zeros((total,), dtype=i32, device=device) if self.dilated else None
+        self.counts_d = torch.zeros((hip.GPP_MAX_GROUPS + 1,), dtype=i32, device=device) if self.dilated else None
+        self.flag_d = torch.ones((1,), dtype=i32, device=device) if self.dilated else None
+        self.tower_name = None
+        self.tower_dense, self.tower_gathered = [], []
         self.rows = torch.zeros((total,), dtype=i32, device=device)
         self.counts = torch.zeros((hip.GPP_MAX_GROUPS + 1,), dtype=i32, device=device)
         self.flag = torch.ones((1,), dtype=i32, device=device)
@@ -153,28 +170,45 @@
         self.lists_joined = False
 
     def tensors(self):
-        return [self.bitmap, self.rows, self.counts, self.flag]
-
-    def put_every_nth(self, torch, n=8):
+        return [self.bitmap, self.rows, self.counts, self.flag] + ([self.rows_d, self.counts_d, self.flag_d] if self.dilated else [])
+
+    def put_every_nth(self, torch, n=8, dilated=False):
+        rows, cnt = (self.rows_d, self.counts_d) if dilated else (self.rows, self.counts)
         begin, counts = 0, []
         for p in self.level_pixels:
-            idx = torch.arange(0, self.B * p, n, dtype=torch.int32, device=self.rows.device)
-            self.rows[begin:begin + idx.numel()] = idx
+            idx = torch.arange(0, self.B * p, n, dtype=torch.int32, device=rows.device)
+            rows[begin:begin + idx.numel()] = idx
             counts.append(int(idx.numel()))
             begin += self.B * p
         counts += [0] * (hip.GPP_MAX_GROUPS - len(counts)) + [sum(counts)]
-        self.counts.copy_(torch.as_tensor(counts, dtype=torch.int32))
+        cnt.copy_(torch.as_tensor(counts, dtype=torch.int32))
 
     def reset(self, torch):
         self.counts.zero_()
         self.flag.fill_(1)
+        if self.dilated:
+            self.counts_d.zero_()
+            self.flag_d.fill_(1)
+
+
+class _HeadsIO(dict):
+
+    def __init__(self, plan):
+        dict.__init__(self)
+        self.plan = plan
+
+    def __getitem__(self, name):
+        sp = self.plan.sparse
+        if sp is not None and sp.tower_dense and name == sp.tower_name:
+            self.plan.complete_heads()
+        return dict.__getitem__(self, name)
 
 
 class Plan(object):
 
     def __init__(self):
         self.keep = []
-        self.io = {}
+        self.io = _HeadsIO(self)
         self.io_parts = {}
         self.tuning_parts = {}
         self.ops = []
@@ -220,9 +254,11 @@
         if self.sparse is None or not self.heads_stale:
             return
         self.heads_stale = False
-        for guarded in self.sparse.dense:
+        for guarded in self.sparse.tower_dense + self.sparse.dense:
             d = type(guarded).from_buffer_copy(guarded)
             d.guard, d.guard_value = None, 0
+            if any(guarded is t for t in self.sparse.tower_dense) and d.range_counter:
+                d.range_counter = self.range_scratch.data_ptr()
             hip.check(hip.lib().gpp_conv2d_igemm(ctypes.byref(d), hip.stream_ptr()), 'gpp_conv2d_igemm (head tensors completed)')
 
     def emit(self, kind, desc, name, reads=(), writes=(), tag=0, flops=0.0, lane=0, join=False, sync=False, io=None, inner=(), atomic=()):
diff --git a/ground-plane-polling_amd/keras_retinanet_3D/models/retinanet.py b/ground-plane-polling_amd/keras_retinanet_3D/models/retinanet.py
--- a/ground-plane-polling_amd/keras_retinanet_3D/models/retinanet.py
+++ b/ground-plane-polling_amd/keras_retinanet_3D/models/retinanet.py
@@ -20,7 +20,8 @@
                    OP_ABSMAX, OP_ABSMAX_CLEAR, OP_STEM_RAGGED, OP_STEM_POOL_RAGGED, OP_MAXPOOL_RAGGED,
                    OP_DETECT_CANDIDATE_PIXELS, DETECT_OPS, OP_JOIN, OP_SYNC,
                    PlanOptions, block_form, part_of, TOWER_SLICES, RANGE_AUDIT_THRESHOLD, X3_QUANTUM,
-                   SPARSE_HEADS_MAX_SHARE, audit_report, SparseHeads, Plan)
+                   SPARSE_HEADS_MAX_SHARE, SPARSE_TOWER_DEFAULT, SPARSE_TOWER_HEIGHTS, SPARSE_TOWER_MAX_SHARE, audit_report, sparse_tower_applies,
+                   SparseHeads, Plan)
 
 
 class RetinaNet3D(object):
@@ -414,6 +415,10 @@
                 lists = hip.PixelListDesc(ws.data_ptr(), sp.bitmap.data_ptr(), sp.rows.data_ptr(), sp.counts.data_ptr(), sp.flag.data_ptr(),
                                           plan.n_anchors, B, anchor_utils.NUM_BASE_ANCHORS, 4 if self.osf else 1, len(sp.level_pixels),
                                           sp.max_rows, 0, (ctypes.c_int32 * hip.GPP_MAX_GROUPS)(*sp.level_pixels), 0)
+                if sp.dilated:
+                    lists.level_widths = (ctypes.c_int32 * hip.GPP_MAX_GROUPS)(*sp.level_widths)
+                    lists.max_rows_dilated = sp.max_rows_d
+                    lists.rows_dilated, lists.counts_dilated, lists.flag_dilated = sp.rows_d.data_ptr(), sp.counts_d.data_ptr(), sp.flag_d.data_ptr()
                 reads, writes = access[OP_DETECT_CANDIDATES]
                 plan.emit(kind, CandidatePixelsDesc(ctypes.addressof(dd), lists), name, reads, writes + sp.tensors(), inner=(dd,), **flags)
                 return
@@ -430,9 +435,28 @@
                    for m in wide]
             for i in range(1, 4):
                 _, dst = pyramid(width)
-                self._conv(plan, '{}_{}'.format(prefix, i), src, dst, 3, pad=(1, 1), relu=True, tag=tag, lane=lane)
+                if i == 3 and prefix == 'pyramid_regression' and plan.sparse is not None and plan.sparse.dilated:
+                    last_tower_layer('{}_{}'.format(prefix, i), src, dst)
+                else:
+                    self._conv(plan, '{}_{}'.format(prefix, i), src, dst, 3, pad=(1, 1), relu=True, tag=tag, lane=lane)
                 src = dst
             out_layer(out_name, src, out, lane, join)
+
+        def last_tower_layer(name, src, dst):
+            sp = plan.sparse
+            dense = self._desc(plan, name, src, dst, 3, pad=(1, 1), relu=True)
+            dense.guard, dense.guard_value = sp.flag_d.data_ptr(), 1
+            plan.emit(OP_CONV, dense, name, list(src) + [sp.flag_d], dst, flops=C.conv_flops(dense), join=not sp.lists_joined, io=(src, dst, None))
+            sp.lists_joined = True
+            sp.tower_dense.append(dense)
+            sp.tower_name = name
+            for height in SPARSE_TOWER_HEIGHTS:
+                rows = self._desc(plan, name, src, dst, 3, pad=(1, 1), relu=True)
+                rows.gather_rows, rows.gather_counts, rows.split_k = sp.rows_d.data_ptr(), sp.counts_d.data_ptr(), 1
+                rows.guard, rows.guard_value = sp.flag_d.data_ptr(), 0
+                rows.tile_hint = 9000256 + 1000 * height
+                plan.emit(OP_CONV, rows, name, list(src) + [sp.rows_d, sp.counts_d, sp.flag_d], dst, io=(src, dst, None))
+                sp.tower_gathered.append(rows)
 
         def out_layer(name, src, out, lane, join):
             sp = plan.sparse
@@ -461,7 +485,12 @@
                   'reg': ('pyramid_regression', 512, 0, 'pyramid_regression_ops', reg_o, 1, 0, bool(opts.cls_lane)),
                   'dim': ('pyramid_regression_dim', 128, 768, 'pyramid_regression_dim', dim_o, 0, l_dim)}
         if opts.sparse_heads:
-            plan.sparse = SparseHeads(self.torch, self.device, P[0].B, [m.H * m.W for m in P], opts.sparse_heads)
+            level_pixels = [m.H * m.W for m in P]
+            use_tower = (opts.sparse_tower >= 0.0 and self.dtype in C.X3_TYPES and opts.x3_level >= 1 and opts.decode_overlap and not opts.cls_lane and
+                     not plan.ragged and not self.audit and self.plan_mode != 'latency' and
+                     (opts.sparse_tower_force or sparse_tower_applies(P[0].B, level_pixels, 512)))
+            plan.sparse = SparseHeads(self.torch, self.device, P[0].B, level_pixels, opts.sparse_heads,
+                                      *(([m.W for m in P], opts.sparse_tower) if use_tower else ()))
             plan.keep += plan.sparse.tensors()
         if opts.decode_overlap:
             tower(*towers['cls'])
@@ -621,6 +650,8 @@
             autotune=env('GPP_AUTOTUNE', '1') != '0',
             sparse_heads=(max(1e-9, float(env('GPP_SPARSE_HEADS_MAX_SHARE', SPARSE_HEADS_MAX_SHARE)))
                           if (overlap and not self.audit and env('GPP_SPARSE_HEADS', '1') != '0') else 0.0),
+            sparse_tower=float(env('GPP_SPARSE_TOWER_MAX_SHARE', SPARSE_TOWER_MAX_SHARE)) if env('GPP_SPARSE_TOWER', SPARSE_TOWER_DEFAULT) != '0' else -1.0,
+            sparse_tower_force=env('GPP_SPARSE_TOWER', SPARSE_TOWER_DEFAULT) == 'force',
             tune_key='x3split={};fuse={}/{};plan={}{}'.format(env('GPP_X3_SPLIT', '2'), env('GPP_FUSE_TAIL', '64,128'), env('GPP_FUSE_BLOCK', '64,128'),
                                                               self.plan_mode, C.latency_split_config() if self.plan_mode == 'latency' else '') +
                      (';audit' if self.audit else ''))
@@ -648,6 +679,7 @@
         plan.decode_overlap = opts.decode_overlap
         plan.range_slot = torch.zeros((1,), dtype=torch.int64, device=dev)
         plan.range_seen = 0
+        plan.range_scratch = torch.zeros((1,), dtype=torch.int64, device=dev)
         plan.images = torch.empty((B, H, Wd, 3), dtype=torch.float32, device=dev)
         plan.P_inv = torch.empty((B, 4, 3), dtype=torch.float32, device=dev)
         plan.planes = torch.empty((B, n_planes, 4) if planes_batched else (n_planes, 4), dtype=torch.float32, device=dev)
@@ -729,10 +761,16 @@
                 continue
             gathered = kind == OP_CONV and bool(desc.gather_rows)
             if kind == OP_CONV and desc.guard:
-                plan.sparse.flag.fill_(0 if gathered else 1)
+                sp = plan.sparse
+                tower = sp.dilated and desc.guard == sp.flag_d.data_ptr()
+                (sp.flag_d if tower else sp.flag).fill_(0 if gathered else 1)
                 if gathered:
-                    plan.sparse.put_every_nth(self.torch)
+                    sp.put_every_nth(self.torch, 3 if tower else 8, dilated=tower)
                     name = name + '@rows'
+                if gathered and tower:
+                    self.run_op(plan, index)
+                    plan.tuning_parts.setdefault(name, []).append((int(desc.tile_hint), 0.0))
+                    continue
             self.run_op(plan, index)
             if kind not in (OP_CONV, OP_TAIL, OP_CONV_PREACT, OP_MOBILENET_BLOCK):
                 continue
diff --git a/include/gpp.h b/include/gpp.h
--- a/include/gpp.h
+++ b/include/gpp.h
@@ -181,6 +181,8 @@
     int64_t n_anchors;
     int32_t B, num_base_anchors, lists_per_image, n_levels, max_rows, reserved;
     int32_t level_pixels[GPP_MAX_GROUPS]; int32_t reserved2;
+    int32_t level_widths[GPP_MAX_GROUPS]; int32_t max_rows_dilated;
+    int32_t* rows_dilated; int32_t* counts_dilated; int32_t* flag_dilated;
 } gpp_pixel_list_desc;
 int gpp_detect_pixel_lists(const gpp_pixel_list_desc* host_desc, void* stream);
 
```

Measured after the change: 834.1. Within noise of the previous version (-0.4%).
